# BerserkerMother/Video-Summarization

Hardware: AMD Instinct MI355X
Metric: frames/sec scored (whole node), synthetic [B,T=1024,D=1024] (higher is better)
Workload: dtype f32; 1 GPU; configs[2]: B=64 videos x T=1024 frames x D=1024 per GPU, scorer cfg M-A (heads 4, d_model 256, layers 4), logits + hidden state; global_batch=64, parallelism=videos sharded over 1 GPU(s), no all_gather of scores

## Files before the change

video-summarization_amd/_lib.py:

```python
from __future__ import annotations

import concurrent.futures
import ctypes as C
import os
import subprocess
import threading
from typing import NamedTuple

HERE = os.path.dirname(os.path.abspath(__file__))
ROOT = os.path.dirname(HERE)
CSRC = os.path.join(HERE, "csrc")
INCLUDE = os.path.join(ROOT, "include")
LIB_PATH = os.path.join(HERE, "libvsscore.so")
DIAG_LIB_PATH = os.path.join(HERE, "libvsscore_diag.so")
SOURCES = ("vs_kernels.hip", "vs_attention.hip", "vs_attention_w64.hip", "vs_mlp_fused.hip", "vs_gemm_ring.hip", "vs_scorer.cpp", "vs_eval.cpp",
           "vs_train_kernels.hip", "vs_train_attention.hip", "vs_train_attention_bf16.hip", "vs_train_gemm_rows.hip", "vs_pretrain_kernels.hip",
           "vs_train.cpp", "vs_segment.hip", "vs_segment_gram.hip", "vs_segment.cpp", "vs_optim.hip", "vs_attention_maps.hip",
           "vs_eval_device.hip", "vs_eval_device.cpp", "vs_summary.hip", "vs_summary.cpp", "vs_batch.hip", "vs_cnn.hip", "vs_cnn.cpp",
           "vs_resize.hip", "vs_resize.cpp", "vs_cnn3d.hip", "vs_cnn3d.cpp", "vs_weights.cpp", "vs_error.cpp")
EXTRA_FLAGS = {"vs_resize.cpp": ("-ffp-contract=off",)}
ABI_VERSION = 3

VS_OK, VS_ERR_INVALID, VS_ERR_WORKSPACE, VS_ERR_HIP = 0, 1, 2, 3
VS_FLAG_SIGMOID = 1
VS_FLAG_BF16_ATTENTION = 2
VS_FLAG_BF16_LINEAR = 4
VS_FLAG_F16X3_LINEAR = 8
VS_FLAG_F16X3_ATTENTION = 16
VS_FLAG_SPLITK = 32
VS_TRAIN_FLAG_BF16_LINEAR = 1
VS_TRAIN_FLAG_BF16_ATTENTION = 2
VS_TRAIN_FLAG_FP16 = 4
VS_TRAIN_FLAG_PACKED_LP_ATTENTION = 8

VS_ADAM_MAX_TENSORS = 64
VS_GRAD_NORM_L2, VS_GRAD_NORM_MAX = 0, 1
VS_KTS_FEATURES_F32, VS_KTS_KERNEL_F32, VS_KTS_KERNEL_F64 = 0, 1, 2
VS_KTS_SCORES, VS_KTS_BACKTRACK, VS_KTS_AUTO = 0, 1, 2
VS_KTS_GRAM_DOT, VS_KTS_GRAM_COSINE, VS_KTS_GRAM_RBF = 0, 1, 2
VS_CNN_INPUT_F32_NCHW, VS_CNN_INPUT_U8_NHWC, VS_CNN_INPUT_F32_NHWC = 0, 1, 2
VS_CNN_NUM_CONVS, VS_CNN_FEATURES = 57, 1024
VS_CNN3D_INPUT_F32_NCDHW, VS_CNN3D_INPUT_U8_NDHWC, VS_CNN3D_INPUT_F32_NDHWC = 0, 1, 2
VS_R3D_NUM_CONVS, VS_R3D_FEATURES = 20, 512
VS_RESIZE_SWAP_RB = 1
VS_RESIZE_PATH_FUSED, VS_RESIZE_PATH_SMALL_TILE = 0, 1
NUM_STAGES = 6


class ModelDesc(C.Structure):
    _fields_ = [("d_model", C.c_int32), ("num_heads", C.c_int32), ("num_layers", C.c_int32),
                ("in_features", C.c_int32), ("max_len", C.c_int32), ("num_classes", C.c_int32)]


_LAYER_FIELDS = ("wq", "bq", "wk", "bk", "wv", "bv", "wo", "bo", "ln1_g", "ln1_b",
                 "w1", "b1", "w2", "b2", "ln2_g", "ln2_b")


class LayerParams(C.Structure):
    _fields_ = [(n, C.c_void_p) for n in _LAYER_FIELDS]


class ModelParams(C.Structure):
    _fields_ = [("embed_w", C.c_void_p), ("embed_b", C.c_void_p), ("pos_embedding", C.c_void_p),
                ("layers", C.POINTER(LayerParams)), ("final_w", C.c_void_p), ("final_b", C.c_void_p)]


class DropoutCfg(C.Structure):
    _fields_ = [("p_embed", C.c_float), ("p", C.c_float), ("seed", C.c_uint64), ("flags", C.c_uint32), ("reserved", C.c_uint32)]


class EvalVideo(C.Structure):
    _fields_ = [("scores", C.c_void_p), ("positions", C.c_void_p), ("change_points", C.c_void_p), ("user_summary", C.c_void_p),
                ("user_scores", C.c_void_p)] + [(n, C.c_int32) for n in ("n_scores", "n_positions", "n_frames", "n_shots", "n_users",
                                                                        "user_len", "n_score_users", "use_max", "user_scores_f32")]


LayerGrads = LayerParams


class ModelGrads(C.Structure):
    _fields_ = [("embed_w", C.c_void_p), ("embed_b", C.c_void_p), ("layers", C.POINTER(LayerParams)),
                ("final_w", C.c_void_p), ("final_b", C.c_void_p)]


class AdamCfg(C.Structure):
    _fields_ = [("lr", C.c_double), ("beta1", C.c_double), ("beta2", C.c_double), ("eps", C.c_double),
                ("weight_decay", C.c_double), ("decoupled", C.c_int32), ("reserved", C.c_int32)]


class AdamTensor(C.Structure):
    _fields_ = [("p", C.c_void_p), ("g", C.c_void_p), ("m", C.c_void_p), ("v", C.c_void_p), ("mirror", C.c_void_p),
                ("step", C.c_void_p), ("n", C.c_size_t)]


class KtsKernel(C.Structure):
    _fields_ = [("kind", C.c_int32), ("reserved", C.c_int32), ("gamma", C.c_double)]


class GradTensor(C.Structure):
    _fields_ = [("g", C.c_void_p), ("n", C.c_size_t)]


class CnnConvParams(C.Structure):
    _fields_ = [(n, C.c_void_p) for n in ("weight", "gamma", "beta", "running_mean", "running_var")]


class CnnParams(C.Structure):
    _fields_ = [("conv", CnnConvParams * VS_CNN_NUM_CONVS)]


class Cnn3dConvParams(C.Structure):
    _fields_ = [(n, C.c_void_p) for n in ("weight", "gamma", "beta", "running_mean", "running_var")]


class R3dParams(C.Structure):
    _fields_ = [("conv", Cnn3dConvParams * VS_R3D_NUM_CONVS)]


_P, _I, _Z, _F, _D, _U32, _U64, _RC = C.c_void_p, C.c_int32, C.c_size_t, C.c_float, C.c_double, C.c_uint32, C.c_uint64, C.c_int
_ref = C.POINTER
_LINEAR = [_P] * 4 + [_I] * 4 + [_P, _I, _P]
_LINEAR_OPERANDS = [_P] * 4 + [_I] * 5 + [_P]
_LINEAR_LN = [_P] * 7 + [_I] * 3 + [_P] * 2 + [_I] * 2 + [_P] * 2
_ATTENTION = [_P] * 5 + [_I] * 4 + [_F, _P]
_BYTES_BT = (_Z, [_P, _I, _I])
_DROPOUT_MASK = [_P, _I, _I, _I, _U64, _U32, _F, _P]
_KTS_SIZES = [_P, _I, _I, _I, _P, _I]
_BINDINGS = {
    "vs_scorer.h": {
        "vs_abi_version": (_RC, []),
        "vs_last_error": (C.c_char_p, []),
        "vs_weights_pack": (_RC, [_ref(ModelDesc), _ref(ModelParams), _P, _ref(_P)]),
        "vs_weights_free": (None, [_P]),
        "vs_weights_update": (_RC, [_P, _ref(ModelParams), _P]),
        "vs_weights_set_norm_width": (_RC, [_P, _I]),
        "vs_set_option": (_RC, [C.c_char_p, _I]),
        "vs_scorer_workspace_bytes": _BYTES_BT,
        "vs_scorer_forward": (_RC, [_P, _P, _P, _I, _I, _U32, _P, _P, _P, _Z, _P]),
        "vs_scorer_workspace_bytes_packed": (_Z, [_P, _P, _I]),
        "vs_scorer_forward_packed": (_RC, [_P, _P, _P, _P, _I, _U32, _P, _P, _P, _Z, _P]),
        "vs_scorer_workspace_bytes_cls": _BYTES_BT,
        "vs_scorer_forward_cls": (_RC, [_P, _P, _P, _P, _I, _I, _U32, _P, _P, _P, _Z, _P]),
        "vs_linear_f32": (_RC, _LINEAR),
        "vs_qkv_proj_f32": (_RC, [_P] * 4 + [_I] * 4 + [_P]),
        "vs_attention_f32": (_RC, _ATTENTION),
        "vs_attention_bf16": (_RC, _ATTENTION),
        "vs_attention_bf16_stored": (_RC, [_P] * 5 + [_I] * 4 + [_P]),
        "vs_attention_qscale": (_F, [_F]),
        "vs_attention_f16x3": (_RC, _ATTENTION),
        "vs_linear_residual_layernorm_f32": (_RC, _LINEAR_LN),
        "vs_linear_bf16": (_RC, _LINEAR),
        "vs_linear_residual_layernorm_bf16": (_RC, _LINEAR_LN),
        "vs_linear_f16x3": (_RC, _LINEAR),
        "vs_linear_residual_layernorm_f16x3": (_RC, _LINEAR_LN),
        "vs_mlp_block_bf16": (_RC, [_P, _I, _P, _P, _I, _I, _I, _P, _P]),
        "vs_linear_bf16_operands": (_RC, _LINEAR_OPERANDS),
        "vs_qkv_proj_bf16_operands": (_RC, _LINEAR_OPERANDS),
        "vs_to_bf16": (_RC, [_P, _P, _Z, _P]),
        "vs_linear_bf16_a16": (_RC, [_P] * 4 + [_I] * 3 + [_P, _P]),
        "vs_profile_enable": (_RC, [_I]),
        "vs_profile_collect": (_RC, [_ref(_D), _ref(C.c_int64)]),
        "vs_stage_name": (C.c_char_p, [_I]),
    },
    "vs_eval.h": {
        "vs_eval_upsample": (_RC, [_P, _I, _P, _I, _I, _P]),
        "vs_eval_knapsack": (_RC, [_I, _P, _P, _I, _P, _ref(_I)]),
        "vs_eval_generate_summary": (_RC, [_P, _I, _P, _I, _I, _P, _I, _P, _I]),
        "vs_eval_fscore": (_RC, [_P, _I, _P, _I, _I, _I, _ref(_D)]),
        "vs_eval_rank_correlation": (_RC, [_P, _I, _P, _I, _ref(_D), _ref(_D)]),
        "vs_eval_corpus": (_RC, [_ref(EvalVideo), _I, _I, _P, _P, _P]),
    },
    "vs_eval_device.h": {
        "vs_eval_set_create": (_RC, [_ref(EvalVideo), _I, _P, _ref(_P)]),
        "vs_eval_set_free": (None, [_P]),
        "vs_eval_set_workspace_bytes": (_Z, [_P, _P, _I]),
        "vs_eval_set_run": (_RC, [_P, _P, _P, _I] + [_P] * 5 + [_Z, _P]),
    },
    "vs_summary.h": {
        "vs_summarize_workspace_bytes": (_Z, [_I] + [_P] * 4 + [_D]),
        "vs_summarize": (_RC, [_I] + [_P] * 6 + [_D] + [_P] * 7 + [_Z, _P]),
    },
    "vs_batch.h": {
        "vs_batch_gather_packed": (_RC, [_P] * 3 + [_I] + [_P] * 2 + [_I, C.c_int64, _I] + [_P] * 3),
        "vs_batch_gather_padded": (_RC, [_P] * 3 + [_I] + [_P] * 2 + [_I] * 3 + [_F, _I] + [_P] * 4),
        "vs_batch_gather_rows": (_RC, [_P, _I, _P, _I, _I, _P, _P]),
    },
    "vs_train.h": {
        "vs_train_prepare": (_RC, [_P, _P]),
        "vs_train_saved_bytes": _BYTES_BT,
        "vs_train_workspace_bytes": _BYTES_BT,
        "vs_train_forward": (_RC, [_P, _P, _P, _I, _I, _ref(DropoutCfg), _P, _P, _P, _Z, _P, _Z, _P]),
        "vs_train_backward": (_RC, [_P, _P, _P, _I, _I, _ref(DropoutCfg), _P, _P, _P, _Z, _ref(ModelGrads), _P, _P, _Z, _P]),
        "vs_mse_mask_loss_forward": (_RC, [_P, _P, _P, _I, _I, _P, _P, _P]),
        "vs_mse_mask_loss_backward": (_RC, [_P, _P, _P, _P, _I, _I, _P, _P]),
        "vs_train_attention_forward": (_RC, [_P] * 6 + [_I] * 4 + [_F, _U64, _U32, _F, _P]),
        "vs_train_attention_backward": (_RC, [_P] * 9 + [_I] * 4 + [_F, _U64, _U32, _F, _P]),
        "vs_train_attention_dropout_bits_bytes": (_Z, [_I] * 3),
        "vs_train_attention_dropout_bits": (_RC, _DROPOUT_MASK),
        "vs_train_attention_forward_bf16": (_RC, [_P] * 6 + [_I] * 4 + [_F, _F, _P, _I, _P]),
        "vs_train_attention_backward_bf16": (_RC, [_P] * 9 + [_I] * 4 + [_F, _F, _P, _I, _P]),
        "vs_train_wgrad_scratch_floats": (_Z, [_I] * 3),
        "vs_train_wgrad": (_RC, [_P, _P, _I, _I, _I, _P, _P, _P, _P]),
        "vs_train_wgrad_bf16": (_RC, [_P, _P, _I, _I, _I, _P, _P, _P, _P]),
        "vs_train_dropout_mask_attention": (_RC, _DROPOUT_MASK),
        "vs_train_dropout_mask_rows": (_RC, [_P, _I, _I, _U64, _U32, _F, _P]),
        "vs_train_dropout_site": (_U32, [_I, _I]),
        "vs_train_saved_field": (_RC, [_P, _I, _I, _I, _I, _ref(_Z), _ref(_Z)]),
        "vs_train_last_format": (_U32, []),
        "vs_pretrain_head_state_bytes": (_Z, [_I] * 3),
        "vs_pretrain_head_workspace_bytes": (_Z, [_I] * 4),
        "vs_pretrain_head_forward": (_RC, [_P] * 6 + [_I] * 4 + [_F, _I] + [_P] * 4),
        "vs_pretrain_head_backward": (_RC, [_P] * 8 + [_I] * 4 + [_F, _I] + [_P] * 5 + [_Z, _P]),
        "vs_train_check_packed": (_RC, [_ref(ModelDesc), _P, _I]),
        "vs_train_saved_bytes_desc": (_Z, [_ref(ModelDesc), _P, _I, _I]),
        "vs_train_saved_bytes_packed": (_Z, [_P, _P, _I]),
        "vs_train_workspace_bytes_packed": (_Z, [_P, _P, _I]),
        "vs_train_forward_packed": (_RC, [_P, _P, _P, _P, _I, _ref(DropoutCfg), _P, _P, _P, _Z, _P, _Z, _P]),
        "vs_train_backward_packed": (_RC, [_P, _P, _P, _P, _I, _ref(DropoutCfg), _P, _P, _P, _Z, _ref(ModelGrads), _P, _P, _Z, _P]),
        "vs_mse_packed_loss_forward": (_RC, [_P, _P, _I, _D, _P, _P, _P]),
        "vs_mse_packed_loss_backward": (_RC, [_P, _P, _P, _I, _D, _P, _P]),
        "vs_train_attention_packed_scratch_bytes": _BYTES_BT,
        "vs_train_attention_forward_packed": (_RC, [_P] * 7 + [_I] * 3 + [_F, _U64, _U32, _F, _P, _Z, _P]),
        "vs_train_attention_backward_packed": (_RC, [_P] * 9 + [_I] * 3 + [_F, _U64, _U32, _F, _P, _Z, _P]),
        "vs_train_dropout_mask_attention_packed": (_RC, [_P, _P, _I, _I, _U64, _U32, _F, _P]),
        "vs_train_saved_field_packed": (_RC, [_P, _P, _I, _I, _I, _ref(_Z), _ref(_Z)]),
        "vs_train_attention_packed_lp_scratch_bytes": _BYTES_BT,
        "vs_train_attention_forward_packed_lp": (_RC, [_P] * 7 + [_I] * 3 + [_F, _U64, _U32, _F, _I, _P, _Z, _P]),
        "vs_train_attention_backward_packed_lp": (_RC, [_P] * 9 + [_I] * 3 + [_F, _U64, _U32, _F, _I, _P, _Z, _P]),
        "vs_pretrain_head_state_bytes_packed": _BYTES_BT,
        "vs_pretrain_head_workspace_bytes_packed": (_Z, [_P, _I, _I, _I]),
        "vs_pretrain_head_forward_packed": (_RC, [_P] * 4 + [_I] * 2 + [_P] * 3 + [_I] * 2 + [_F, _I] + [_P] * 4),
        "vs_pretrain_head_backward_packed": (_RC, [_P] * 4 + [_I] * 2 + [_P] * 5 + [_I] * 2 + [_F, _I] + [_P] * 5 + [_Z, _P]),
    },
    "vs_segment.h": {
        "vs_kts_workspace_bytes": (_Z, _KTS_SIZES),
        "vs_kts_segment": (_RC, [_P, _I, _I, _P, _I] + [_P] * 5 + [_I] + [_P] * 4 + [_Z, _P]),
        "vs_kts_scatters": (_RC, [_P, _I, _I, _I, _P, _P, _Z, _P]),
        "vs_kts_gram_workspace_bytes": _BYTES_BT,
        "vs_kts_gram": (_RC, [_P, _I, _P, _I, _ref(KtsKernel), _P, _P, _Z, _P]),
        "vs_kts_workspace_bytes_k": (_Z, _KTS_SIZES + [_ref(KtsKernel)]),
        "vs_kts_segment_k": (_RC, [_P, _I, _I, _P, _I] + [_P] * 5 + [_I, _ref(KtsKernel)] + [_P] * 4 + [_Z, _P]),
        "vs_kts_eval_score": (_RC, [_P, _I, _I, _ref(KtsKernel), _P, _I] + [_P] * 4 + [_Z, _P]),
    },
    "vs_optim.h": {
        "vs_adam_step_tensors": (_RC, [_ref(AdamTensor), _I, _ref(AdamCfg), _P, _P, _P, _P]),
        "vs_adam_state_bytes": (_Z, [_P]),
        "vs_adam_state_init": (_RC, [_P, _P, _P]),
        "vs_adam_state_field": (_RC, [_P, _I, _I, _ref(_Z), _ref(_Z)]),
        "vs_adam_step": (_RC, [_P, _ref(ModelParams), _ref(ModelGrads), _P, _ref(AdamCfg), _P, _P, _P]),
        "vs_grad_norm_workspace_bytes": (_Z, [_ref(GradTensor), _I]),
        "vs_grad_norm_tensors": (_RC, [_ref(GradTensor), _I, _I, _D, _P, _P, _P, _Z, _P]),
        "vs_grad_norm": (_RC, [_P, _ref(ModelGrads), _I, _D, _P, _P, _P, _Z, _P]),
        "vs_grad_scale_tensors": (_RC, [_ref(GradTensor), _I, _P, _P]),
    },
    "vs_inspect.h": {
        "vs_inspect_workspace_bytes": (_Z, [_P, _I, _I, _I]),
        "vs_inspect_forward": (_RC, [_P] * 4 + [_I] * 2 + [_ref(_I), _I] + [_P] * 6 + [_Z, _P]),
        "vs_attention_probs_workspace_bytes": (_Z, [_I] * 3),
        "vs_attention_probs_f32": (_RC, [_P] * 6 + [_I] * 4 + [_F, _P, _Z, _P]),
    },
}
(EXPORTS, EVAL_EXPORTS, EVAL_DEVICE_EXPORTS, SUMMARY_EXPORTS, BATCH_EXPORTS, TRAIN_EXPORTS, SEGMENT_EXPORTS, OPTIM_EXPORTS,
 INSPECT_EXPORTS) = (tuple(_BINDINGS["vs_%s.h" % h]) for h in ("scorer", "eval", "eval_device", "summary", "batch", "train", "segment",
                                                                "optim", "inspect"))

PACKED_INSPECT_HEADER = os.path.join("packed", "vs_inspect_packed.h")
_PACKED_INSPECT_BINDINGS = {
    "vs_inspect_workspace_bytes_packed": (_Z, [_P, _P, _I]),
    "vs_inspect_forward_packed": (_RC, [_P] * 4 + [_I, _ref(_I), _I] + [_P] * 6 + [_Z, _P]),
    "vs_attention_probs_packed_workspace_bytes": (_Z, [_P, _I, _I]),
    "vs_attention_probs_packed_f32": (_RC, [_P] * 4 + [_I] * 3 + [_F] + [_P] * 4 + [_Z, _P]),
}
PACKED_INSPECT_EXPORTS = tuple(_PACKED_INSPECT_BINDINGS)

FEATURES_HEADER = os.path.join("features", "vs_features.h")
_FEATURES_BINDINGS = {
    "vs_cnn_pack": (_RC, [_ref(CnnParams), _P, _ref(_P)]),
    "vs_cnn_free": (None, [_P]),
    "vs_cnn_min_side": (_I, []),
    "vs_cnn_workspace_bytes": (_Z, [_I] * 3),
    "vs_cnn_forward": (_RC, [_P, _P] + [_I] * 4 + [_P, _P, _Z, _P]),
    "vs_cnn_packed_floats": (_Z, [_I] * 3),
    "vs_cnn_pack_conv": (_RC, [_ref(CnnConvParams)] + [_I] * 3 + [_P, _P]),
    "vs_cnn_conv": (_RC, [_P] + [_I] * 5 + [_P] + [_I] * 4 + [_P, _I, _I, _P]),
    "vs_cnn_maxpool": (_RC, [_P] + [_I] * 8 + [_P, _P]),
}
FEATURES_EXPORTS = tuple(_FEATURES_BINDINGS)

RESIZE_HEADER = os.path.join("features", "vs_resize.h")
_RESIZE_BINDINGS = {
    "vs_resize_output_size": (_RC, [_I] * 3 + [_ref(_I)] * 2),
    "vs_resize_plan_create": (_RC, [_I] * 4 + [_P, _ref(_P)]),
    "vs_resize_plan_free": (None, [_P]),
    "vs_resize_plan_describe": (_RC, [_P] + [_ref(_I)] * 3),
    "vs_resize_workspace_bytes": (_Z, [_P, _I]),
    "vs_resize_run": (_RC, [_P, _P, _I, _U32, _P, _P, _Z, _P]),
}
RESIZE_EXPORTS = tuple(_RESIZE_BINDINGS)

VIDEO_FEATURES_HEADER = os.path.join("features", "vs_video_features.h")
_VIDEO_FEATURES_BINDINGS = {
    "vs_r3d_pack": (_RC, [_ref(R3dParams), _P, _ref(_P)]),
    "vs_r3d_free": (None, [_P]),
    "vs_r3d_workspace_bytes": (_Z, [_I] * 4),
    "vs_r3d_flops": (_D, [_I] * 4),
    "vs_r3d_normalisation": (_RC, [_ref(_F)]),
    "vs_r3d_forward": (_RC, [_P, _P] + [_I] * 5 + [_P, _P, _Z, _P]),
    "vs_cnn3d_packed_floats": (_Z, [_I] * 4),
    "vs_cnn3d_pack_conv": (_RC, [_ref(Cnn3dConvParams)] + [_I] * 4 + [_P, _P]),
    "vs_cnn3d_conv": (_RC, [_P] + [_I] * 6 + [_P] + [_I] * 7 + [_P, _I, _P, _P]),
}
VIDEO_FEATURES_EXPORTS = tuple(_VIDEO_FEATURES_BINDINGS)


def hipcc_path() -> str:
    for p in (os.environ.get("HIPCC"), "/opt/rocm/bin/hipcc"):
        if p and os.path.exists(p):
            return p
# ... 152 lines not shown
```

video-summarization_amd/csrc/vs_forward_plan.h:

```cpp
#pragma once
#include <stddef.h>

#include <cstdio>
#include <string>

#include "vs_scorer.h"

struct VskOptions {
    int skinny_rows;
    int lp_min_rows;
    int train_lp_min_rows;
    int lp_min_rows_fused;
    int attn_w64;
    int lp_store32;
    int lp_mlp_unfused;
    int lp_tail_unfused;
    int lp_qkv_unfused;
    int lp_tile256;
    int lp_embed_unfused;
    int exact_unfused;
    int layer_tail_min_rows;
    int mlp_abl;
    int attn_w64_checked;
    int attn_w64_abl;
};

enum { VSK_STORE16 = 16, VSK_A16 = 32, VSK_F16 = 64 };

enum { VSW_FRAGMENTS = 1, VSW_F16X3 = 2, VSW_BF16 = 4, VSW_ROWS16 = 8,
       VSW_TRANSPOSED = 16, VSW_TRANSPOSED_FRAGMENTS = 32, VSW_TRANSPOSED_W2_16 = 64,
       VSW_NUM_FAMILIES = 7 };

inline bool vsk_mlp_bf16_supported(int d) { return d == 256; }
inline bool vsk_gemm16_supported(int M, int N, int K) { return M > 0 && N > 0 && N % 32 == 0 && K >= 32 && K % 32 == 0; }
inline bool vsk_layer_fused_supported(int M, int d, int skinny_rows) { return d == 256 && M > skinny_rows && M <= (1 << 20); }

enum VsArith { VS_ARITH_EXACT = 0, VS_ARITH_BF16 = 1, VS_ARITH_F16X3 = 2 };
enum VsEmbedForm {
    VS_EMBED_CLS,
    VS_EMBED_BF16_QKV,
    VS_EMBED_SPLITK,
    VS_EMBED_GEMM,
};
enum VsAttentionKernel {
    VS_ATT_PACKED,
    VS_ATT_DH256,
    VS_ATT_SPLITKV,
    VS_ATT_LOWPREC,
    VS_ATT_EXACT,
};
enum VsLayerForm {
    VS_LAYER_RING,
    VS_LAYER_BF16_TAIL,
    VS_LAYER_BF16_MLP,
    VS_LAYER_EXACT_PAIR,
    VS_LAYER_STAGES,
};
enum VsLnForm {
    VS_LN_NONE,
    VS_LN_SPLITK_ROWS,
    VS_LN_GEMM_ROWS,
    VS_LN_FUSED,
};

struct VsForwardIn {
    int d_model, num_heads, num_layers, in_features, max_len;
    int norm_width;
    bool has_pe, has_b_embed;
    int B, T;
    unsigned flags;
    bool cls, packed;
};

struct VsForwardPlan {
    int T, M;
    VsArith linear, attention_arith;
    unsigned families;
    VsEmbedForm embed;
    VsAttentionKernel attention;
    VsLayerForm layer;
    VsLnForm ln1, ln2;
    bool qkv16, ffn16;
    bool next_qkv;
    size_t kv_stride;
    int mode_linear;
    int mode_qkv;
    int mode_ffn;
    int mode_attention;

    bool tail_writes_qkv() const { return next_qkv || layer == VS_LAYER_EXACT_PAIR; }
};

inline int vs_attention_prec(unsigned flags) { return (flags & VS_FLAG_F16X3_ATTENTION) ? 2 : (flags & VS_FLAG_BF16_ATTENTION) ? 1 : 0; }

inline int vs_forward_plan(const VsForwardIn &in, const VskOptions &opt, VsForwardPlan *plan, std::string *err) {
    char msg[192];
    auto fail = [&](int code) { *err = msg; return code; };
    const int d = in.d_model, H = in.num_heads, dh = d / H;
    const unsigned flags = in.flags;
    if (!in.packed && in.has_pe && in.T > in.max_len) {
        snprintf(msg, sizeof msg, "T=%d exceeds the positional table (max_len=%d)", in.T, in.max_len);
        return fail(VS_ERR_INVALID);
    }
    if (in.cls && in.packed) { snprintf(msg, sizeof msg, "packed batches have no class-token form"); return fail(VS_ERR_INVALID); }
    const int T = in.T + (in.cls ? 1 : 0);
    if ((long long)in.B * T > (1ll << 30)) { snprintf(msg, sizeof msg, "B*T too large"); return fail(VS_ERR_INVALID); }
    if ((flags & VS_FLAG_BF16_LINEAR) && (flags & VS_FLAG_F16X3_LINEAR)) {
        snprintf(msg, sizeof msg, "VS_FLAG_BF16_LINEAR and VS_FLAG_F16X3_LINEAR are exclusive");
        return fail(VS_ERR_INVALID);
    }
    if ((flags & (VS_FLAG_BF16_ATTENTION | VS_FLAG_F16X3_ATTENTION)) && dh != 32 && dh != 64 && !((flags & VS_FLAG_BF16_ATTENTION) && dh == 128)) {
        snprintf(msg, sizeof msg, "VS_FLAG_BF16_ATTENTION needs head_dim 32, 64 or 128, VS_FLAG_F16X3_ATTENTION 32 or 64 (got %d)", dh);
        return fail(VS_ERR_INVALID);
    }
    if ((flags & VS_FLAG_BF16_ATTENTION) && (flags & VS_FLAG_F16X3_ATTENTION)) {
        snprintf(msg, sizeof msg, "VS_FLAG_BF16_ATTENTION and VS_FLAG_F16X3_ATTENTION are exclusive");
        return fail(VS_ERR_INVALID);
    }

    VsForwardPlan p{};
    p.T = T;
    p.M = in.B * T;
    const int M = p.M;
    const bool embedded = in.norm_width != d;
    const int aprec = vs_attention_prec(flags);
    p.attention_arith = (VsArith)aprec;
    const bool fused_ok = !embedded && vsk_mlp_bf16_supported(d) && aprec == 1 && !opt.lp_store32 && !opt.lp_mlp_unfused;
    const int lp_min_rows = fused_ok && opt.lp_min_rows_fused < opt.lp_min_rows ? opt.lp_min_rows_fused
                                                                               : opt.lp_min_rows;
    p.linear = (flags & VS_FLAG_F16X3_LINEAR) ? VS_ARITH_F16X3 : ((flags & VS_FLAG_BF16_LINEAR) && M > lp_min_rows) ? VS_ARITH_BF16 : VS_ARITH_EXACT;
    const bool bf16 = p.linear == VS_ARITH_BF16;
    const bool splitk = (flags & VS_FLAG_SPLITK) && !bf16 && !in.packed && !in.cls && M <= opt.skinny_rows && (d == 128 || d == 256 || d == 512);
    const int rows_min = in.cls ? in.B * in.T : M;
    p.families = 0;
    if (bf16) p.families = VSW_BF16;
    else if (rows_min <= opt.skinny_rows) p.families = p.linear == VS_ARITH_F16X3 ? VSW_F16X3 : VSW_FRAGMENTS;
    if (bf16 && d > 256) p.families |= VSW_ROWS16;
    p.ffn16 = bf16 && d <= 256 && !embedded && !opt.lp_store32;
    p.qkv16 = p.ffn16 && aprec == 1;
    const bool mlp16 = bf16 && !embedded && vsk_mlp_bf16_supported(d) && !opt.lp_mlp_unfused && !opt.lp_store32;
    const bool ring = bf16 && aprec == 1 && !in.packed && d > 256 && !opt.lp_store32 && vsk_gemm16_supported(M, d, d);
    p.kv_stride = (p.qkv16 || ring) ? (size_t)M * d / 2 : (size_t)M * d;
    p.next_qkv = mlp16 && p.qkv16 && !opt.lp_qkv_unfused;
    const bool exact_fused = p.linear == VS_ARITH_EXACT && aprec == 0 && !embedded && !splitk && !opt.exact_unfused &&
                             vsk_layer_fused_supported(M, d, opt.skinny_rows) && d % H == 0 && dh % 32 == 0;

    p.embed = in.cls ? VS_EMBED_CLS
            : bf16 && in.has_b_embed && p.next_qkv && in.num_layers > 0 && !opt.lp_embed_unfused ? VS_EMBED_BF16_QKV
            : splitk && in.in_features % 1024 == 0 ? VS_EMBED_SPLITK
            : VS_EMBED_GEMM;
    p.attention = in.packed ? VS_ATT_PACKED
                : dh == 256 ? VS_ATT_DH256
                : splitk && aprec != 1 && (dh == 32 || dh == 64 || dh == 128) ? VS_ATT_SPLITKV
                : aprec ? VS_ATT_LOWPREC
                : VS_ATT_EXACT;
    const VsLnForm ln = (d > 256 || embedded) ? VS_LN_GEMM_ROWS : VS_LN_FUSED;
    p.ln1 = p.ln2 = VS_LN_NONE;
    if (ring) p.layer = VS_LAYER_RING;
    else if (mlp16 && p.qkv16 && !opt.lp_tail_unfused) p.layer = VS_LAYER_BF16_TAIL;
    else if (exact_fused) p.layer = VS_LAYER_EXACT_PAIR;
    else {
        p.layer = mlp16 ? VS_LAYER_BF16_MLP : VS_LAYER_STAGES;
        p.ln1 = splitk && d >= 256 ? VS_LN_SPLITK_ROWS : ln;
        if (!mlp16) p.ln2 = splitk ? VS_LN_SPLITK_ROWS : ln;
    }
    p.mode_linear = p.linear;
    p.mode_qkv = p.qkv16 ? (1 | VSK_STORE16) : p.linear;
    p.mode_ffn = p.ffn16 ? (1 | VSK_STORE16) : p.linear;
    p.mode_attention = (p.qkv16 || ring) ? (1 | VSK_STORE16) : aprec;
    *plan = p;
    return VS_OK;
}

inline int vs_packed_waves(int dh, int aprec, long long r8, long long r4) {
    if (dh == 128) return aprec == 1 ? 8 : 4;
    return (!(aprec != 0 && dh == 32) && r8 * 100 <= r4 * 105) ? 8 : 4;
}
```

video-summarization_amd/csrc/vs_kernels.h:

```cpp
#pragma once
#include <hip/hip_runtime.h>
#include <stdint.h>

#include "vs_forward_plan.h"

int vsk_linear(const float *A, const float *W, const float *Wf, const float *bias, float *C, int M, int N, int K,
               int relu, const float *pe, int T, int mode, hipStream_t st);
int vsk_linear_gate(const float *A, const float *W, const float *Wf, const float *bias, const float *gate, float scale,
                    float *C, int M, int N, int K, hipStream_t st, int mode = 0);
int vsk_linear_relu_dropout(const float *A, const float *W, const float *Wf, const float *bias, float *C, int M, int N,
                            int K, unsigned long long seed, unsigned site, float p, hipStream_t st, int mode = 0);
int vsk_pack_fragments(const float *W, float *Wf, int N, int K, hipStream_t st);
int vsk_pack_fragments_f16x3(const float *W, float *Wh, int N, int K, hipStream_t st);
int vsk_qkv(const float *h, const float *Wqkv, const float *Wf, const float *bqkv, float *qkv, int B, int T, int d,
            int H, int mode, hipStream_t st, float qscale = 1.0f);
int vsk_attention(const float *q, const float *k, const float *v, const uint8_t *mask, float *out,
                  int B, int H, int T, int dh, float scale, hipStream_t st);
int vsk_attention_packed(const float *q, const float *k, const float *v, float *out, int H, int Mtot, int dh,
                         float scale, const int *cu, const int *work, int nwork, int nw, int prec, hipStream_t st);
float vsk_attention_qscale(float scale);
int vsk_attention_bf16(const float *q, const float *k, const float *v, const uint8_t *mask, float *out,
                       int B, int H, int T, int dh, float scale, int prec, hipStream_t st);
int vsk_attention_bf16_w64(const void *q, const void *k, const void *v, const uint8_t *mask, void *out, int B, int H, int T,
                           hipStream_t st);
int vsk_attention_bf16_w64_packed(const void *q, const void *k, const void *v, void *out, int H, int Mtot, const int *cu,
                                  const int *work, int nwork, hipStream_t st);
size_t vsk_attention_probs_workspace_bytes(int B, int H, int T);
int vsk_attention_probs(const float *q, const float *k, const uint8_t *mask, float *maps, float *received, float *entropy,
                        int B, int H, int T, int dh, float scale, void *workspace, hipStream_t st);
size_t vsk_attention_probs_packed_workspace_bytes(int B, int H, int M, int tiles);
int vsk_attention_probs_packed_plan(const int *lengths_dev, int B, int H, int M, int tiles, void *workspace, hipStream_t st);
int vsk_attention_probs_packed(const float *q, const float *k, const int *cu, float *maps, float *received, float *entropy, int B,
                               int H, int M, int tiles, int dh, float scale, void *workspace, hipStream_t st);
int vsk_linear_res_ln(const float *A, const float *W, const float *Wf, const float *bias, const float *res,
                      const float *gamma, const float *beta, float *out, int M, int N, int K,
                      const float *score_w, const float *score_b, int num_classes, int sigmoid,
                      float *scores, int mode, hipStream_t st);
int vsk_outproj_ln_fc1(const float *att, const float *Wo, const float *bo, const float *res, const float *gamma, const float *beta,
                       float *h1, const float *W1, const float *b1, float *hidden, int M, int d, hipStream_t st);
int vsk_fc2_ln_qkv(const float *hidden, const float *W2, const float *b2, const float *res, const float *gamma, const float *beta,
                   float *out, const float *Wqkv, const float *bqkv, float *qkv, int B, int T, int d, int H, hipStream_t st);
int vsk_layer_tail(const float *att, const float *Wo, const float *bo, const float *res, const float *g1, const float *be1,
                   const float *W1, const float *b1, float *hidden, const float *W2, const float *b2, const float *g2, const float *be2,
                   float *out, const float *Wqkv, const float *bqkv, float *qkv, const float *score_w, const float *score_b,
                   int num_classes, int sigmoid, float *scores, int B, int T, int d, int H, hipStream_t st);
int vsk_rows_res_ln(const float *a, const float *res, const float *gamma, const float *beta, float *out, int M, int d,
                    const float *score_w, const float *score_b, int num_classes, int sigmoid, float *scores,
                    hipStream_t st, void *out16 = nullptr, int dn = 0,
                    int nsplit = 0, const float *pbias = nullptr);
struct VskMatJobs {
    enum { MAX = 24 };
    const float *in[MAX];
    float *out[MAX];
    int rows[MAX], cols[MAX];
    int n;
};
int vsk_pack_fragments_batch(const VskMatJobs &jobs, hipStream_t st);
int vsk_attention_splitkv(const float *q, const float *k, const float *v, const uint8_t *mask, float *out,
                          int B, int H, int T, int dh, float scale, hipStream_t st);
int vsk_linear_parts(const float *A, const float *Wf, float *parts, int M, int N, int K, int nsplit, hipStream_t st,
                     int f16x3 = 0);
int vsk_sum_parts_pe(const float *parts, int nsplit, const float *bias, const float *pe, int T, float *out, int M, int N, hipStream_t st);
int vsk_diag_attention(const float *q, const float *k, const float *v, float *out, int B, int H, int T, float scale,
                       unsigned long long *diag, hipStream_t st);
int vsk_diag_attention_lp(const float *q, const float *k, const float *v, float *out, int B, int H, int T, float scale,
                          int prec, unsigned long long *diag, hipStream_t st);
int vsk_diag_gemm(const float *A, const float *W, const float *bias, float *C, int M, int N, int K,
                  int grid, unsigned long long *diag, hipStream_t st);
size_t vsk_mlp_bf16_image_bytes(int d);
int vsk_pack_mlp_bf16(const float *Wo, const float *W1, const float *W2, void *img, int d, hipStream_t st);
struct VskNextQkv {
    const void *img;
    const float *bqkv;
    void *qkv16;
    int T, H;
    float qscale;
};
size_t vsk_embed_bf16_image_bytes(int d, int K);
int vsk_pack_embed_bf16(const float *W, void *img, int d, int K, hipStream_t st);
int vsk_embed_bf16(const float *x, const void *img, const float *bias, const float *pe, int T, float *out, int M, int d, int K,
                   const VskNextQkv *next, hipStream_t st);
size_t vsk_qkv_bf16_image_bytes(int d);
int vsk_pack_qkv_bf16(const float *Wqkv, void *img, int d, hipStream_t st);
int vsk_mlp_bf16(const float *h, const void *att16, const float *bo, const float *gamma1, const float *beta1,
                 const void *img, const float *b1, const float *b2,
                 const float *gamma, const float *beta, float *out, int M, int d,
                 const float *score_w, const float *score_b, int num_classes, int sigmoid, float *scores,
                 const VskNextQkv *next, hipStream_t st);
int vsk_plan_packed(const int *lengths_dev, int B, int qb, int *cu, int *work, int work_cap, hipStream_t st);
int vsk_gather_rows(const float *pe, const int *cu, int B, int tmax, int d, float *rows, hipStream_t st);
enum { VSK_COPY_MAX_SEGS = 20 };
struct VskCopySegs {
    const float *src[VSK_COPY_MAX_SEGS];
    float *dst[VSK_COPY_MAX_SEGS];
    unsigned n[VSK_COPY_MAX_SEGS];
    int count;
};
int vsk_copy_segments(const VskCopySegs &segs, hipStream_t st);
int vsk_insert_cls(const float *e, const float *cls, const uint8_t *mask, float *h, uint8_t *mask1, int B, int T, int d,
                   hipStream_t st);
int vsk_skinny_max_rows();

VskOptions &vsk_options();
int vsk_device_cus();

int vsk_gemm16(const void *A16, const void *W16, const float *bias, void *C, int M, int N, int K, int epi, int c16,
               int T, int H, int dh, float qscale, hipStream_t st);
int vsk_to_bf16(const float *src, void *dst, size_t n, hipStream_t st);
```

video-summarization_amd/csrc/vs_kernels.hip:

```cpp
#include "vs_train_device.h"
#include "vs_kernels.h"
#include "vs_launch.h"
#include "vs_linear_pick.h"

namespace {

struct EpiArgs {
    unsigned long long seed;
    unsigned site;
    float p;
    float scale;
};

__device__ __forceinline__ unsigned long long stamp() { return vs_stamp(); }

template <int EPI, int NWM = 2, int DIAG = 0, int NJ = 2, int PREC = 0, int C16 = 0, int KW = 32, int A16 = 0>
__global__ __launch_bounds__(128 * NWM, 2) void gemm_nt_128(
    const float *__restrict__ A, const float *__restrict__ W, const float *__restrict__ bias,
    float *__restrict__ C, int M, int N, int K, const float *__restrict__ pe, int T, int H, int dh,
    unsigned long long *__restrict__ diag = nullptr, EpiArgs ea = EpiArgs{0ull, 0u, 0.f, 0.f}) {
    static_assert(KW == 32 || (KW == 64 && (PREC == 1 || PREC == 3)), "64-wide k-tiles exist for the 16-bit operands only");
    static_assert(A16 == 0 || PREC == 1 || PREC == 3, "16-bit-stored A belongs to the 16-bit operand modes");
    constexpr bool LP1 = PREC == 1 || PREC == 3;
    constexpr int F16 = PREC == 3 ? 1 : 0;
// ... 243 lines not shown
        } else
            __syncthreads();
        fpar ^= 1;
    };

    set_tile(0);
#pragma unroll
    for (int i = 0; i < LA; ++i) load_a(i, 0);
#pragma unroll
    for (int i = 0; i < LW; ++i) load_w(i, 0);
    stage(0);
    __syncthreads();
    if (DIAG != 0) ts0 = stamp();
    const unsigned long long tbegin = ts0;
    if (DIAG >= 2) dsum[3] = __builtin_amdgcn_s_memrealtime();

    for (int it = 0; it < my_tiles; ++it) {
        cu_m0 = nx_m0; cu_n0 = nx_n0;
#pragma unroll
        for (int jj = 0; jj < NJ; ++jj) cu_bias[jj] = nx_bias[jj];
        {
            const f32x16 zero = {0.f, 0.f, 0.f, 0.f, 0.f, 0.f, 0.f, 0.f, 0.f, 0.f, 0.f, 0.f, 0.f, 0.f, 0.f, 0.f};
#pragma unroll
            for (int i = 0; i < 2; ++i)
#pragma unroll
                for (int jj = 0; jj < NJ; ++jj) acc[i][jj] = MFMA32(cu_bias[jj], PREC == 2 ? F16X3_WS : 1.0f, zero);
        }
        for (int kt = 0; kt + 1 < nk; ++kt) ktile((kt + 1) * BK);
        if (it + 1 < my_tiles) set_tile(it + 1);
        ktile(0);

        if constexpr (DIAG == 2) {
            float keep = 0.f;
#pragma unroll
            for (int i = 0; i < 2; ++i)
#pragma unroll
                for (int jj = 0; jj < NJ; ++jj)
#pragma unroll
                    for (int t = 0; t < 16; ++t) keep += acc[i][jj][t];
            if (keep == 1.2345e-30f && diag != nullptr) diag[0] = 1;
            continue;
        }
        unsigned long long te = 0;
        if constexpr (DIAG != 0) te = stamp();
        const int m0 = cu_m0, n0 = cu_n0;
        float *tp = smem + (fpar ^ 1) * (BM + BN) * LD + wave * (32 * LD);
        const int trow = lane >> 3, tc4 = (lane & 7) * 4;
        int b0 = 0, t0 = 0;
        if (EPI == EPI_PE || EPI == EPI_QKV) { b0 = m0 / T; t0 = m0 - b0 * T; }
#pragma unroll
        for (int i = 0; i < 2; ++i) {
#pragma unroll
            for (int jj = 0; jj < NJ; ++jj) {
#pragma unroll
                for (int q = 0; q < 4; ++q) {
                    f32x4 v;
#pragma unroll
                    for (int e = 0; e < 4; ++e) {
                        v[e] = acc[i][jj][4 * q + e];
                        if (EPI == EPI_RELU || EPI == EPI_RELU_DROP) v[e] = relu1(v[e]);
                    }
                    *(f32x4 *)&tp[r * LD + 8 * q + 4 * h] = v;
                }
                const int c32 = n0 + 32 * NJ * wc + 32 * jj;
                int which = 0, head = 0, e0 = 0;
                if (EPI == EPI_QKV) { const int d = H * dh; which = c32 / d; const int c = c32 - which * d; head = c / dh; e0 = c - head * dh; }
#pragma unroll
                for (int p = 0; p < 4; ++p) {
                    const int ro = 64 * wr + 32 * i + trow + 8 * p;
                    f32x4 v = *(const f32x4 *)&tp[(trow + 8 * p) * LD + tc4];
                    if constexpr (PREC == 2) v *= 1.0f / F16X3_WS;
                    const int row = m0 + ro;
                    int bb = b0, tt = t0 + ro;
                    if (EPI == EPI_PE || EPI == EPI_QKV) { while (tt >= T) { tt -= T; ++bb; } }
                    if (row < M && c32 < N) {
                        if (EPI == EPI_PE) {
                            const f32x4 pv = *(const f32x4 *)(pe + (size_t)tt * N + c32 + tc4);
#pragma unroll
                            for (int e = 0; e < 4; ++e) v[e] += pv[e];
                        }
                        if (EPI == EPI_GATE) {
                            if constexpr (C16 != 0) {
                                const u32x2 g2 = *(const u32x2 *)((const a16_t *)pe + (size_t)row * N + c32 + tc4);
#pragma unroll
                                for (int e = 0; e < 4; ++e) v[e] = (short)(g2[e >> 1] >> (16 * (e & 1))) > 0 ? v[e] * ea.scale : 0.f;
                            } else {
                            const f32x4 gv = *(const f32x4 *)(pe + (size_t)row * N + c32 + tc4);
#pragma unroll
                            for (int e = 0; e < 4; ++e) v[e] = gv[e] > 0.f ? v[e] * ea.scale : 0.f;
                            }
                        }
                        if (EPI == EPI_RELU_DROP) {
                            const DropSite dsite = drop_site(ea.seed, ea.site, ea.p);
                            const unsigned rk = drop_rowkey(dsite, (unsigned)row);
#pragma unroll
                            for (int e = 0; e < 4; ++e) v[e] = drop_keep(dsite, rk, (unsigned)(c32 + tc4 + e)) ? v[e] * dsite.scale : 0.f;
                        }
                        if constexpr (C16 != 0) {
                            if (EPI == EPI_QKV && which == 0) v *= ea.scale;
                            u32x2 u; u[0] = pack_lp<F16>(v[0], v[1]); u[1] = pack_lp<F16>(v[2], v[3]);
                            unsigned short *C2 = (unsigned short *)C;
                            if (EPI == EPI_QKV)
                                *(u32x2 *)(C2 + (size_t)which * M * (H * dh) + (((size_t)bb * H + head) * T + tt) * dh + e0 + tc4) = u;
                            else
                                *(u32x2 *)(C2 + (size_t)row * N + c32 + tc4) = u;
                        } else if (EPI == EPI_QKV)
                            *(f32x4 *)(C + (size_t)which * M * (H * dh) + (((size_t)bb * H + head) * T + tt) * dh + e0 + tc4) = v;
                        else
                            *(f32x4 *)(C + (size_t)row * N + c32 + tc4) = v;
                    }
                }
            }
        }
        __syncthreads();
        if constexpr (DIAG != 0) dsum[1] += stamp() - te;
    }
    if (DIAG >= 2) { ts0 = stamp(); dsum[4] = __builtin_amdgcn_s_memrealtime(); }
    if (DIAG != 0 && diag != nullptr && lane == 0) {
        unsigned long long *o = diag + ((size_t)blockIdx.x * (2 * NWM) + wave) * 8;
#pragma unroll
        for (int i = 0; i < 5; ++i) o[i] = dsum[i];
        o[5] = ts0 - tbegin; o[6] = (unsigned long long)(my_tiles * nk); o[7] = tbegin;
    }
}

template <int NB, int PREC = 0>
__global__ __launch_bounds__(256) void gemm_res_ln(
    const float *__restrict__ A, const float *__restrict__ W, const float *__restrict__ bias,
    const float *__restrict__ res, const float *__restrict__ gamma, const float *__restrict__ beta,
    float *__restrict__ out, int M, int K,
    const float *__restrict__ score_w, const float *__restrict__ score_b, int num_classes,
    int sigmoid, float *__restrict__ scores) {
    constexpr int BM = 64, N = 64 * NB, BK = 16, LD = BK + 4;
    __shared__ __attribute__((aligned(16))) float smem[2 * (BM + N) * LD];

    const int m0 = blockIdx.x * BM;
    const int tid = threadIdx.x, lane = tid & 63, wave = tid >> 6;
    const int r = lane & 31, h = lane >> 5;
    const int wr = wave >> 1, wc = wave & 1;

    const int lrow = tid >> 2, lc4 = (tid & 3) * 4;
    int arow = m0 + lrow; arow = arow < M ? arow : M - 1;
    const float *ag = A + (size_t)arow * K + lc4;
    const float *wg = W + (size_t)lrow * K + lc4;
    f32x4 pa, pw[NB];
    pa = *(const f32x4 *)ag;
#pragma unroll
    for (int i = 0; i < NB; ++i) pw[i] = *(const f32x4 *)(wg + (size_t)64 * i * K);

    f32x16 acc[NB];
#pragma unroll
    for (int j = 0; j < NB; ++j)
#pragma unroll
        for (int t = 0; t < 16; ++t) acc[j][t] = 0.f;

    auto put = [&](float *rowp, f32x4 v, float scale) __attribute__((always_inline)) {
        if constexpr (PREC == 2) {
            v *= scale;
            u32x2 hi, lo;
            split_f16x4((const float *)&v, hi, lo);
            *(u32x2 *)&rowp[lc4 / 2] = hi;
            *(u32x2 *)&rowp[8 + lc4 / 2] = lo;
        } else {
            *(f32x4 *)&rowp[lc4] = v;
        }
    };
    {
        float *As = smem, *Ws = smem + BM * LD;
        put(&As[lrow * LD], pa, 1.0f);
#pragma unroll
        for (int i = 0; i < NB; ++i) put(&Ws[(lrow + 64 * i) * LD], pw[i], F16X3_WS);
    }
    __syncthreads();

    const int nk = K / BK;
    for (int kt = 0; kt < nk; ++kt) {
        const int cur = kt & 1;
        const float *As = smem + cur * (BM + N) * LD, *Ws = As + BM * LD;
        const bool more = kt + 1 < nk;
        if (more) {
            pa = *(const f32x4 *)(ag + (kt + 1) * BK);
#pragma unroll
            for (int i = 0; i < NB; ++i) pw[i] = *(const f32x4 *)(wg + (size_t)64 * i * K + (kt + 1) * BK);
        }
        const float *ap = As + (32 * wr + r) * LD + 4 * h;
        const float *wp = Ws + (32 * NB * wc + r) * LD + 4 * h;
        if constexpr (PREC == 2) {
            const f16x8 ah = __builtin_bit_cast(f16x8, *(const u32x4 *)ap), al = __builtin_bit_cast(f16x8, *(const u32x4 *)(ap + 8));
#pragma unroll
            for (int j = 0; j < NB; ++j) {
                const f16x8 bh = __builtin_bit_cast(f16x8, *(const u32x4 *)(wp + 32 * j * LD));
                const f16x8 bl = __builtin_bit_cast(f16x8, *(const u32x4 *)(wp + 32 * j * LD + 8));
                acc[j] = MFMA_F16(ah, bl, acc[j]);
                acc[j] = MFMA_F16(al, bh, acc[j]);
                acc[j] = MFMA_F16(ah, bh, acc[j]);
            }
        } else {
#pragma unroll
            for (int g = 0; g < BK / 8; ++g) {
                const f32x4 a = *(const f32x4 *)(ap + 8 * g);
                f32x4 b[NB];
#pragma unroll
                for (int j = 0; j < NB; ++j) b[j] = *(const f32x4 *)(wp + 32 * j * LD + 8 * g);
#pragma unroll
                for (int s = 0; s < 4; ++s)
#pragma unroll
                    for (int j = 0; j < NB; ++j) acc[j] = MFMA32(a[s], b[j][s], acc[j]);
            }
        }
        if (more) {
            float *An = smem + (cur ^ 1) * (BM + N) * LD, *Wn = An + BM * LD;
            put(&An[lrow * LD], pa, 1.0f);
#pragma unroll
            for (int i = 0; i < NB; ++i) put(&Wn[(lrow + 64 * i) * LD], pw[i], F16X3_WS);
        }
        __syncthreads();
    }

    float *red = smem;
    const int cbase = 32 * NB * wc + r;
    float bj[NB], gj[NB], bej[NB];
#pragma unroll
    for (int j = 0; j < NB; ++j) { bj[j] = bias[cbase + 32 * j]; gj[j] = gamma[cbase + 32 * j]; bej[j] = beta[cbase + 32 * j]; }

    float part[16];
#pragma unroll
    for (int t = 0; t < 16; ++t) {
        int row = m0 + 32 * wr + acc_row(t, h); row = row < M ? row : M - 1;
        float s = 0.f;
#pragma unroll
        for (int j = 0; j < NB; ++j) {
            const float v = (PREC == 2 ? acc[j][t] * (1.0f / F16X3_WS) : acc[j][t]) + bj[j] + res[(size_t)row * N + cbase + 32 * j];
            acc[j][t] = v;
            s += v;
        }
        part[t] = half_sum(s);
    }
    if (r == 0) {
#pragma unroll
        for (int t = 0; t < 16; ++t) red[wc * 64 + 32 * wr + acc_row(t, h)] = part[t];
    }
    __syncthreads();
    float mean[16];
#pragma unroll
    for (int t = 0; t < 16; ++t) {
        const int rl = 32 * wr + acc_row(t, h);
        mean[t] = (red[rl] + red[64 + rl]) * (1.0f / N);
    }
    __syncthreads();
#pragma unroll
    for (int t = 0; t < 16; ++t) {
        float s = 0.f;
#pragma unroll
        for (int j = 0; j < NB; ++j) { const float c = acc[j][t] - mean[t]; acc[j][t] = c; s += c * c; }
        part[t] = half_sum(s);
    }
    if (r == 0) {
#pragma unroll
        for (int t = 0; t < 16; ++t) red[wc * 64 + 32 * wr + acc_row(t, h)] = part[t];
    }
    __syncthreads();
#pragma unroll
    for (int t = 0; t < 16; ++t) {
        const int rl = 32 * wr + acc_row(t, h);
        const float rstd = 1.0f / sqrtf((red[rl] + red[64 + rl]) * (1.0f / N) + 1e-5f);
        const int row = m0 + rl;
#pragma unroll
        for (int j = 0; j < NB; ++j) {
            const float y = acc[j][t] * rstd * gj[j] + bej[j];
            acc[j][t] = y;
            if (row < M) out[(size_t)row * N + cbase + 32 * j] = y;
        }
    }
    if (score_w != nullptr) {
        for (int c = 0; c < num_classes; ++c) {
            __syncthreads();
            float wj[NB];
#pragma unroll
            for (int j = 0; j < NB; ++j) wj[j] = score_w[(size_t)c * N + cbase + 32 * j];
#pragma unroll
            for (int t = 0; t < 16; ++t) {
                float s = 0.f;
#pragma unroll
                for (int j = 0; j < NB; ++j) s += acc[j][t] * wj[j];
                part[t] = half_sum(s);
            }
            if (r == 0) {
#pragma unroll
                for (int t = 0; t < 16; ++t) red[wc * 64 + 32 * wr + acc_row(t, h)] = part[t];
            }
            __syncthreads();
            if (tid < 64) {
                const int row = m0 + tid;
                if (row < M) {
                    float s = red[tid] + red[64 + tid] + score_b[c];
                    if (sigmoid) s = 1.0f / (1.0f + expf(-s));
                    scores[(size_t)row * num_classes + c] = s;
                }
            }
        }
    }
}

struct LnTail {
    const float *W2, *b2;
    float *C2;
    int T, H, dhs;
};
struct LnPhase2 {
    const float *W, *bias, *gamma, *beta;
    float *out;
    LnTail tl;
};

template <int NT, int PREC, int A16, int DIAG, int TAIL>
__device__ __forceinline__ void ln_rows_tiles(
    const float *__restrict__ A, const float *__restrict__ W, const float *__restrict__ bias,
    const float *__restrict__ res, const float *__restrict__ gamma, const float *__restrict__ beta,
    float *__restrict__ out, int M, int K,
    const float *__restrict__ score_w, const float *__restrict__ score_b, int num_classes,
    int sigmoid, float *__restrict__ scores, unsigned long long *__restrict__ diag, const LnTail tl, const LnPhase2 p2) {
    static_assert(TAIL == 0 || (NT == 8 && PREC == 0 && DIAG == 0), "the register-fed tail exists for exact fp32 at d_model 256");
    constexpr int BM = 128, N = 32 * NT, BK = 16, LD = BK + 4;
    constexpr int WL = (N * BK / 4 + 255) / 256;
    constexpr bool TWO = TAIL >= 3;
    constexpr int NPH = TWO ? 2 : 1;
    constexpr int TN2 = TAIL == 2 ? 3 * N : 4 * N;
    constexpr int SMALL2 = TAIL == 3 ? 3 * N + 3 * N : TAIL == 4 ? 3 * N : 0;
    __shared__ __attribute__((aligned(16))) float smem[2 * (BM + N) * LD + 4 * N + (TAIL != 0 ? TN2 : 0) + SMALL2];
    float *gam_s = smem + 2 * (BM + N) * LD, *bet_s = gam_s + N, *sw_s = bet_s + N, *bias_s = sw_s + N;
    float *bias2_s = bias_s + N;
    float *small2_s = bias2_s + TN2;

    int tid = threadIdx.x, lane = tid & 63, wave = tid >> 6;
    int r = lane & 31, h = lane >> 5;
    const int ntiles = (M + BM - 1) / BM;
    const int nk = K / BK;

    constexpr float SC = PREC == 2 ? F16X3_WS : 1.0f;
    for (int i = tid; i < N; i += 256) { gam_s[i] = gamma[i]; bet_s[i] = beta[i]; bias_s[i] = bias[i] * SC; }
    if constexpr (TAIL != 0)
        for (int i = tid; i < TN2; i += 256) bias2_s[i] = tl.b2[i];
    if constexpr (TWO) {
        for (int i = tid; i < N; i += 256) { small2_s[i] = p2.gamma[i]; small2_s[N + i] = p2.beta[i]; small2_s[2 * N + i] = p2.bias[i]; }
        if constexpr (TAIL == 3)
            for (int i = tid; i < 3 * N; i += 256) small2_s[3 * N + i] = p2.tl.b2[i];
    }

    int lrow = tid >> 2, lc4 = (tid & 3) * 4;
    f32x4 pa[2], pw[WL];
    u32x2 pa16[2];
    const float *aptr[2], *wptr[WL];
    const unsigned short *aptr16[2];
#pragma unroll
    for (int i = 0; i < WL; ++i) {
        int wrow = lrow + 64 * i; wrow = wrow < N ? wrow : N - 1;
        wptr[i] = W + (size_t)wrow * K + lc4;
    }
    static_assert(PREC != 0 || N % 64 == 0, "the exact-fp32 staging map covers W without a guard");
    __amdgpu_buffer_rsrc_t ars = __builtin_amdgcn_make_buffer_rsrc(const_cast<float *>(A), 0, 0, 0x00020000);
    __amdgpu_buffer_rsrc_t wrs = __builtin_amdgcn_make_buffer_rsrc(const_cast<float *>(W), 0, N * K * 4, 0x00020000);
    int aoff[2], woff[WL];
#pragma unroll
    for (int i = 0; i < WL; ++i) woff[i] = ((lrow + 64 * i) * K + lc4) * 4;
    auto gload = [&](int i, int kb) __attribute__((always_inline)) {
        if (i < 2) pa[i] = __builtin_bit_cast(f32x4, __builtin_amdgcn_raw_buffer_load_b128(ars, aoff[i], kb, 0));
        else pw[i - 2] = __builtin_bit_cast(f32x4, __builtin_amdgcn_raw_buffer_load_b128(wrs, woff[i - 2], kb, 0));
    };
    constexpr int LDB = 12;
    auto stage = [&](int buf) __attribute__((always_inline)) {
        float *As = smem + buf * (BM + N) * LD, *Ws = As + BM * LD;
        if constexpr (PREC == 2) {
#pragma unroll
            for (int i = 0; i < 2; ++i) {
                u32x2 hi, lo;
                split_f16x4((const float *)&pa[i], hi, lo);
                *(u32x2 *)&As[(lrow + 64 * i) * LD + lc4 / 2] = hi;
                *(u32x2 *)&As[(lrow + 64 * i) * LD + 8 + lc4 / 2] = lo;
            }
#pragma unroll
            for (int i = 0; i < WL; ++i)
                if (lrow + 64 * i < N) {
                    u32x2 hi, lo;
                    const f32x4 ws = pw[i] * F16X3_WS;
                    split_f16x4((const float *)&ws, hi, lo);
                    *(u32x2 *)&Ws[(lrow + 64 * i) * LD + lc4 / 2] = hi;
                    *(u32x2 *)&Ws[(lrow + 64 * i) * LD + 8 + lc4 / 2] = lo;
                }
        } else if constexpr (PREC == 1) {
#pragma unroll
            for (int i = 0; i < 2; ++i) {
                u32x2 u;
                if constexpr (A16 != 0) u = pa16[i];
                else { u[0] = pack_bf16(pa[i][0], pa[i][1]); u[1] = pack_bf16(pa[i][2], pa[i][3]); }
                *(u32x2 *)&As[(lrow + 64 * i) * LDB + lc4 / 2] = u;
            }
#pragma unroll
            for (int i = 0; i < WL; ++i)
                if (lrow + 64 * i < N) {
                    u32x2 u; u[0] = pack_bf16(pw[i][0], pw[i][1]); u[1] = pack_bf16(pw[i][2], pw[i][3]);
                    *(u32x2 *)&Ws[(lrow + 64 * i) * LDB + lc4 / 2] = u;
                }
        } else {
#pragma unroll
            for (int i = 0; i < 2; ++i) *(f32x4 *)&As[(lrow + 64 * i) * LD + lc4] = pa[i];
#pragma unroll
            for (int i = 0; i < WL; ++i) *(f32x4 *)&Ws[(lrow + 64 * i) * LD + lc4] = pw[i];
        }
    };

    f32x16 acc[NT];

    constexpr int TCH = 128, TWB = 4 * 32 * 36, TBUF = TCH * 36;
    static_assert(TAIL == 0 || TWB + 2 * TBUF <= 2 * (BM + N) * LD, "corners and weight tiles fit the staging area");
    int r2 = tid >> 3, c2 = (tid & 7) * 4;
    __amdgpu_buffer_rsrc_t wrs2 = __builtin_amdgcn_make_buffer_rsrc(const_cast<float *>(tl.W2), 0, TN2 * N * 4, 0x00020000);
    const float *tbias_s = bias2_s;
    int woff2 = (r2 * N + c2) * 4;
    f32x4 pw2[4];
    f32x16 U[4];
    auto tail_soff = [&](int c, int kt) __attribute__((always_inline)) { return (TCH * c * N + 32 * kt) * 4; };
    auto tail_load = [&](int i, int soff) __attribute__((always_inline)) {
        pw2[i] = __builtin_bit_cast(f32x4, __builtin_amdgcn_raw_buffer_load_b128(wrs2, woff2, soff + 32 * i * N * 4, 0));
    };
    auto tail_stage = [&](int buf) __attribute__((always_inline)) {
#pragma unroll
        for (int i = 0; i < 4; ++i) *(f32x4 *)&smem[TWB + buf * TBUF + (r2 + 32 * i) * 36 + c2] = pw2[i];
    };
    auto bias_mfma = [&](int c) __attribute__((always_inline)) {
        const f32x16 zero = {0.f, 0.f, 0.f, 0.f, 0.f, 0.f, 0.f, 0.f, 0.f, 0.f, 0.f, 0.f, 0.f, 0.f, 0.f, 0.f};
#pragma unroll
        for (int jj = 0; jj < 4; ++jj) {
            const float bv = tbias_s[TCH * c + 32 * jj + r];
            U[jj] = MFMA32(h == 0 ? bv : 0.f, 1.0f, zero);
        }
    };
    auto tail_step = [&](auto ktc, int nsoff) __attribute__((always_inline)) {
        constexpr int kt = decltype(ktc)::value;
        const float *wp = smem + TWB + (kt & 1) * TBUF + r * 36 + 4 * h;
        float *wd = smem + TWB + ((kt + 1) & 1) * TBUF + r2 * 36 + c2;
        f32x4 fw[3];
        fw[0] = *(const f32x4 *)wp;
        fw[1] = *(const f32x4 *)(wp + 32 * 36);
        __builtin_amdgcn_sched_barrier(0);
#pragma unroll
        for (int t = 0; t < 16; ++t) {
            const int g = t / 4, jj = t % 4;
            if (t + 2 < 16) fw[(t + 2) % 3] = *(const f32x4 *)(wp + 32 * ((t + 2) % 4) * 36 + 8 * ((t + 2) / 4));
            if (t < 4) tail_load(t, nsoff);
            if (t >= 12) *(f32x4 *)(wd + 32 * (t - 12) * 36) = pw2[t - 12];
#pragma unroll
            for (int s2 = 0; s2 < 4; ++s2) U[jj] = MFMA32(fw[t % 3][s2], acc[kt][4 * g + s2], U[jj]);
            __builtin_amdgcn_sched_group_barrier(0x008, 1, 0);
            if (t + 2 < 16) __builtin_amdgcn_sched_group_barrier(0x100, 1, 0);
            if (t < 4) __builtin_amdgcn_sched_group_barrier(0x020, 1, 0);
            __builtin_amdgcn_sched_group_barrier(0x008, 3, 0);
            if (t >= 12) __builtin_amdgcn_sched_group_barrier(0x200, 1, 0);
            __builtin_amdgcn_sched_barrier(0);
        }
        __syncthreads();
    };

    unsigned long long dsum[3] = {0, 0, 0}, tbegin = 0, tq = 0, ktiles = 0;
    if constexpr (DIAG != 0) tbegin = stamp();
    for (int tile = blockIdx.x; tile < ntiles; tile += gridDim.x) {
        if constexpr (DIAG != 0) tq = stamp();
        const int m0 = tile * BM;
      static_for<NPH>([&](auto phc) __attribute__((always_inline)) {
        constexpr int PH = decltype(phc)::value;
        constexpr bool P1 = TWO && PH == 1;
        constexpr int PT = !TWO ? TAIL : PH == 0 ? 1 : TAIL == 3 ? 2 : 0;
        constexpr int PTN2 = PT == 2 ? 3 * N : 4 * N, TNC = PTN2 / TCH;
        const LnTail ptl = P1 ? p2.tl : tl;
        const float *pA = P1 ? tl.C2 : A;
        const int pK = P1 ? 4 * N : K, pnk = P1 ? 4 * N / BK : nk;
        const float *pgam_s = P1 ? small2_s : gam_s, *pbet_s = P1 ? small2_s + N : bet_s, *pbias_s = P1 ? small2_s + 2 * N : bias_s;
        float *pout = P1 ? p2.out : out;
        if constexpr (TWO) {
            asm volatile("" : "+v"(tid));
            lane = tid & 63; wave = tid >> 6; r = lane & 31; h = lane >> 5;
            lrow = tid >> 2; lc4 = (tid & 3) * 4; r2 = tid >> 3; c2 = (tid & 7) * 4; woff2 = (r2 * N + c2) * 4;
            wrs = __builtin_amdgcn_make_buffer_rsrc(const_cast<float *>(P1 ? p2.W : W), 0, N * pK * 4, 0x00020000);
#pragma unroll
            for (int i = 0; i < WL; ++i) woff[i] = ((lrow + 64 * i) * pK + lc4) * 4;
            if constexpr (PT != 0) {
                wrs2 = __builtin_amdgcn_make_buffer_rsrc(const_cast<float *>(ptl.W2), 0, PTN2 * N * 4, 0x00020000);
                tbias_s = P1 ? small2_s + 3 * N : bias2_s;
            }
        }
        int row = m0 + 32 * wave + r;
        const bool row_ok = row < M;
        row = row_ok ? row : M - 1;
#pragma unroll
        for (int i = 0; i < 2; ++i) {
            int ar = m0 + lrow + 64 * i; ar = ar < M ? ar : M - 1;
            if constexpr (A16 != 0) {
                aptr16[i] = (const unsigned short *)A + (size_t)ar * K + lc4;
                pa16[i] = *(const u32x2 *)aptr16[i];
            } else if constexpr (PREC == 0) {
                aoff[i] = ((ar - m0) * pK + lc4) * 4;
            } else {
                aptr[i] = A + (size_t)ar * K + lc4;
                pa[i] = *(const f32x4 *)aptr[i];
            }
        }
        if constexpr (PREC == 0) {
            ars = __builtin_amdgcn_make_buffer_rsrc(const_cast<float *>(pA + (size_t)m0 * pK), 0, (M - m0 < BM ? M - m0 : BM) * pK * 4, 0x00020000);
            if constexpr (P1) {
#pragma unroll
                for (int i = 2; i < 2 + WL; ++i) gload(i, 0);
                asm volatile("s_waitcnt vmcnt(0)" ::: "memory");
                __builtin_amdgcn_fence(__ATOMIC_RELEASE, "workgroup");
                __syncthreads();
                __builtin_amdgcn_fence(__ATOMIC_ACQUIRE, "workgroup");
#pragma unroll
                for (int i = 0; i < 2; ++i) gload(i, 0);
            } else {
#pragma unroll
                for (int i = 0; i < 2 + WL; ++i) gload(i, 0);
            }
        } else {
#pragma unroll
            for (int i = 0; i < WL; ++i) pw[i] = *(const f32x4 *)wptr[i];
        }
        if constexpr (!P1) {
            const float *rp = res + (size_t)row * N + 4 * h;
#pragma unroll
            for (int j = 0; j < NT; ++j)
#pragma unroll
                for (int q = 0; q < 4; ++q) {
                    f32x4 rv = *(const f32x4 *)(rp + 32 * j + 8 * q);
                    if constexpr (PREC == 2) rv *= SC;
#pragma unroll
                    for (int e = 0; e < 4; ++e) acc[j][4 * q + e] = rv[e];
                }
        }
        if constexpr (!P1) __syncthreads();
        stage(0);
        __syncthreads();
        if constexpr (DIAG != 0) { dsum[2] += stamp() - tq; ktiles += nk; }

        for (int kt = 0; kt < pnk; ++kt) {
            const int kn = kt + 1 < pnk ? kt + 1 : kt;
            const float *As = smem + (kt & 1) * (BM + N) * LD, *Ws = As + BM * LD;
            if constexpr (PREC == 2) {
                const float *arow = As + (32 * wave + r) * LD + 4 * h;
                const f16x8 ah = __builtin_bit_cast(f16x8, *(const u32x4 *)arow);
                const f16x8 al = __builtin_bit_cast(f16x8, *(const u32x4 *)(arow + 8));
#pragma unroll
                for (int i = 0; i < 2; ++i) pa[i] = *(const f32x4 *)(aptr[i] + kn * BK);
#pragma unroll
                for (int i = 0; i < WL; ++i) pw[i] = *(const f32x4 *)(wptr[i] + kn * BK);
#pragma unroll
                for (int j = 0; j < NT; ++j) {
                    const float *wrow = Ws + (32 * j + r) * LD + 4 * h;
                    const f16x8 wh = __builtin_bit_cast(f16x8, *(const u32x4 *)wrow);
                    const f16x8 wl = __builtin_bit_cast(f16x8, *(const u32x4 *)(wrow + 8));
                    acc[j] = MFMA_F16(wl, ah, acc[j]);
                    acc[j] = MFMA_F16(wh, al, acc[j]);
                    acc[j] = MFMA_F16(wh, ah, acc[j]);
                }
                stage((kt + 1) & 1);
                __syncthreads();
                continue;
            }
            if constexpr (PREC == 1) {
                const bf16x8 fa = __builtin_bit_cast(bf16x8, *(const u32x4 *)(As + (32 * wave + r) * LDB + 4 * h));
#pragma unroll
                for (int i = 0; i < 2; ++i) {
                    if constexpr (A16 != 0) pa16[i] = *(const u32x2 *)(aptr16[i] + kn * BK);
                    else pa[i] = *(const f32x4 *)(aptr[i] + kn * BK);
                }
#pragma unroll
                for (int i = 0; i < WL; ++i) pw[i] = *(const f32x4 *)(wptr[i] + kn * BK);
#pragma unroll
                for (int j = 0; j < NT; ++j) {
                    const bf16x8 fw = __builtin_bit_cast(bf16x8, *(const u32x4 *)(Ws + (32 * j + r) * LDB + 4 * h));
                    acc[j] = MFMA_BF16(fw, fa, acc[j]);
                }
                stage((kt + 1) & 1);
                __syncthreads();
                continue;
            }
            const float *ap = As + (32 * wave + r) * LD + 4 * h;
            const float *wp = Ws + r * LD + 4 * h;
            constexpr int NS = 2 * NT, NL = 2 + WL;
            constexpr int LPS = (NL + NT - 1) / NT;
            constexpr int WB = NS - (NL + LPS - 1) / LPS;
            static_assert(BK == 16 && (NL + LPS - 1) / LPS <= NT, "loads and LDS writes of a k-tile occupy distinct steps");
            f32x4 fa[2], fw[3];
            fa[0] = *(const f32x4 *)ap;
            fw[0] = *(const f32x4 *)wp;
            fw[1] = *(const f32x4 *)(wp + 32 * LD);
            fa[1] = *(const f32x4 *)(ap + 8);
            __builtin_amdgcn_sched_barrier(0);
#pragma unroll
            for (int t = 0; t < NS; ++t) {
                const int g = t / NT, j = t % NT;
                if (t + 2 < NS) fw[(t + 2) % 3] = *(const f32x4 *)(wp + 32 * ((t + 2) % NT) * LD + 8 * ((t + 2) / NT));
                int nld = 0, nwr = 0;
#pragma unroll
                for (int q = 0; q < LPS; ++q) {
                    const int il = t * LPS + q, iw = (t - WB) * LPS + q;
                    if (il < NL) { gload(il, kn * (BK * 4)); ++nld; }
                    if (t >= WB && iw < NL) {
                        float *Ad = smem + ((kt + 1) & 1) * (BM + N) * LD, *Wd = Ad + BM * LD;
                        if (iw < 2) *(f32x4 *)&Ad[(lrow + 64 * iw) * LD + lc4] = pa[iw];
                        else *(f32x4 *)&Wd[(lrow + 64 * (iw - 2)) * LD + lc4] = pw[iw - 2];
                        ++nwr;
                    }
                }
#pragma unroll
                for (int s2 = 0; s2 < 4; ++s2) acc[j] = MFMA32(fw[t % 3][s2], fa[g][s2], acc[j]);
                __builtin_amdgcn_sched_group_barrier(0x008, 1, 0);
                if (t + 2 < NS) __builtin_amdgcn_sched_group_barrier(0x100, 1, 0);
#pragma unroll
                for (int q = 0; q < LPS; ++q)
                    if (q < nld) __builtin_amdgcn_sched_group_barrier(0x020, 1, 0);
                __builtin_amdgcn_sched_group_barrier(0x008, 3, 0);
#pragma unroll
                for (int q = 0; q < LPS; ++q)
                    if (q < nwr) __builtin_amdgcn_sched_group_barrier(0x200, 1, 0);
                __builtin_amdgcn_sched_barrier(0);
            }
            if constexpr (DIAG != 0) {
                const unsigned long long tb = stamp();
                __syncthreads();
                dsum[0] += stamp() - tb;
            } else
                __syncthreads();
        }
        if constexpr (DIAG != 0) tq = stamp();
        if constexpr (PT != 0) {
#pragma unroll
            for (int i = 0; i < 4; ++i) tail_load(i, tail_soff(0, 0));
        }

        float sum = 0.f;
#pragma unroll
        for (int j = 0; j < NT; ++j) {
            float pj = 0.f;
#pragma unroll
            for (int q = 0; q < 4; ++q) {
                const f32x4 bv = *(const f32x4 *)&pbias_s[32 * j + 8 * q + 4 * h];
#pragma unroll
                for (int e = 0; e < 4; ++e) { acc[j][4 * q + e] += bv[e]; pj += acc[j][4 * q + e]; }
            }
            sum += pj;
        }
        sum = pair_sum(sum);
        const float mean = sum * (1.0f / N);
        float sq = 0.f;
#pragma unroll
        for (int j = 0; j < NT; ++j) {
            float pj = 0.f;
#pragma unroll
            for (int t = 0; t < 16; ++t) { const float c = acc[j][t] - mean; acc[j][t] = c; pj += c * c; }
            sq += pj;
        }
        sq = pair_sum(sq);
        const float rstd = 1.0f / sqrtf(sq * (1.0f / N) + 1e-5f * (SC * SC));
        float *tp = smem + wave * (32 * 36);
        const int trow = lane >> 3, tc4 = (lane & 7) * 4;
#pragma unroll
        for (int j = 0; j < NT; ++j) {
#pragma unroll
            for (int q = 0; q < 4; ++q) {
                const f32x4 gv = *(const f32x4 *)&pgam_s[32 * j + 8 * q + 4 * h];
                const f32x4 bv = *(const f32x4 *)&pbet_s[32 * j + 8 * q + 4 * h];
                f32x4 y;
#pragma unroll
                for (int e = 0; e < 4; ++e) { y[e] = acc[j][4 * q + e] * rstd * gv[e] + bv[e]; acc[j][4 * q + e] = y[e]; }
                if constexpr (!TWO || P1) *(f32x4 *)&tp[r * 36 + 8 * q + 4 * h] = y;
            }
            if constexpr (TWO && !P1) __builtin_amdgcn_sched_barrier(0);
            if constexpr (!TWO || P1) {
#pragma unroll
                for (int pq = 0; pq < 4; ++pq) {
                    const f32x4 v = *(const f32x4 *)&tp[(trow + 8 * pq) * 36 + tc4];
                    const int orow = m0 + 32 * wave + trow + 8 * pq;
                    if (orow < M) *(f32x4 *)(pout + (size_t)orow * N + 32 * j + tc4) = v;
                }
            }
        }
        if constexpr (!TWO || (P1 && TAIL == 4))
        if (score_w != nullptr) {
            for (int c = 0; c < num_classes; ++c) {
                __syncthreads();
                for (int i = tid; i < N; i += 256) sw_s[i] = score_w[(size_t)c * N + i];
                __syncthreads();
                float dot = 0.f;
#pragma unroll
                for (int j = 0; j < NT; ++j) {
                    float pj = 0.f;
#pragma unroll
                    for (int q = 0; q < 4; ++q) {
                        const f32x4 wv = *(const f32x4 *)&sw_s[32 * j + 8 * q + 4 * h];
#pragma unroll
                        for (int e = 0; e < 4; ++e) pj += acc[j][4 * q + e] * wv[e];
                    }
                    dot += pj;
                }
                dot = pair_sum(dot);
                if (h == 0 && row_ok) {
                    float sc = dot + score_b[c];
                    if (sigmoid) sc = 1.0f / (1.0f + expf(-sc));
                    scores[(size_t)row * num_classes + c] = sc;
                }
            }
        }
        if constexpr (DIAG != 0) dsum[1] += stamp() - tq;
        if constexpr (PT != 0) {
            tail_stage(0);
            int rowoff[4];
            __amdgpu_buffer_rsrc_t crs;
            if constexpr (PT == 1) {
                crs = __builtin_amdgcn_make_buffer_rsrc(ptl.C2 + (size_t)m0 * PTN2, 0, (M - m0 < BM ? M - m0 : BM) * PTN2 * 4, 0x00020000);
#pragma unroll
                for (int p = 0; p < 4; ++p) rowoff[p] = ((32 * wave + trow + 8 * p) * PTN2 + tc4) * 4;
            } else {
                crs = __builtin_amdgcn_make_buffer_rsrc(ptl.C2, 0, 0, 0x00020000);
#pragma unroll
                for (int p = 0; p < 4; ++p) {
                    const int orow = m0 + 32 * wave + trow + 8 * p;
                    const int bb = orow / ptl.T, tt = orow - bb * ptl.T;
                    rowoff[p] = orow < M ? (((bb * ptl.H * ptl.T + tt) << ptl.dhs) + tc4) * 4 : (int)0x80000000;
                }
            }
            bias_mfma(0);
            __syncthreads();
            for (int c = 0; c < TNC; ++c) {
                const int cn = c + 1 < TNC ? c + 1 : c;
                static_for<8>([&](auto ktc) __attribute__((always_inline)) {
                    constexpr int kt = decltype(ktc)::value;
                    tail_step(ktc, kt < 7 ? tail_soff(c, kt + 1) : tail_soff(cn, 0));
                });
                if constexpr (PT == 2) {
                    const int which = c >> 1;
                    crs = __builtin_amdgcn_make_buffer_rsrc(ptl.C2 + (size_t)which * M * N, 0, M * N * 4, 0x00020000);
                }
#pragma unroll
                for (int jj = 0; jj < 4; ++jj) {
                    __builtin_amdgcn_sched_barrier(0);
#pragma unroll
                    for (int q = 0; q < 4; ++q) {
                        f32x4 v;
#pragma unroll
                        for (int e = 0; e < 4; ++e) v[e] = PT == 1 ? relu1(U[jj][4 * q + e]) : U[jj][4 * q + e];
                        *(f32x4 *)&tp[r * 36 + 8 * q + 4 * h] = v;
                    }
                    int soff;
                    if constexpr (PT == 1) soff = (TCH * c + 32 * jj) * 4;
                    else {
                        const int cc = (TCH * c + 32 * jj) & (N - 1), head = cc >> ptl.dhs, e0 = cc - (head << ptl.dhs);
                        soff = (((head * ptl.T) << ptl.dhs) + e0) * 4;
                    }
#pragma unroll
                    for (int p = 0; p < 4; ++p) {
                        const f32x4 v = *(const f32x4 *)&tp[(trow + 8 * p) * 36 + tc4];
                        __builtin_amdgcn_raw_buffer_store_b128(__builtin_bit_cast(u32x4, v), crs, rowoff[p], soff, 0);
                    }
                }
                __builtin_amdgcn_sched_barrier(0);
                bias_mfma(cn);
            }
        }
      });
    }
    if constexpr (DIAG != 0) {
        if (diag != nullptr && lane == 0) {
            unsigned long long *o = diag + ((size_t)blockIdx.x * 4 + wave) * 8;
            o[0] = dsum[0]; o[1] = dsum[1]; o[2] = dsum[2]; o[3] = 0; o[4] = 0;
            o[5] = stamp() - tbegin; o[6] = ktiles; o[7] = tbegin;
        }
    }
}

template <int NT, int PREC = 0, int A16 = 0, int DIAG = 0>
__global__ __launch_bounds__(256, 2) void gemm_ln_rows(
    const float *__restrict__ A, const float *__restrict__ W, const float *__restrict__ bias,
    const float *__restrict__ res, const float *__restrict__ gamma, const float *__restrict__ beta,
    float *__restrict__ out, int M, int K,
    const float *__restrict__ score_w, const float *__restrict__ score_b, int num_classes,
    int sigmoid, float *__restrict__ scores, unsigned long long *__restrict__ diag = nullptr) {
    ln_rows_tiles<NT, PREC, A16, DIAG, 0>(A, W, bias, res, gamma, beta, out, M, K, score_w, score_b, num_classes, sigmoid, scores, diag,
                                          LnTail{nullptr, nullptr, nullptr, 0, 0, 0}, LnPhase2{});
}

__global__ __launch_bounds__(256, 2) void layer_outproj_ln_fc1(
    const float *__restrict__ A, const float *__restrict__ W, const float *__restrict__ bias,
    const float *__restrict__ res, const float *__restrict__ gamma, const float *__restrict__ beta,
    float *__restrict__ out, int M, int K, const float *__restrict__ W1, const float *__restrict__ b1, float *__restrict__ hidden) {
    ln_rows_tiles<8, 0, 0, 0, 1>(A, W, bias, res, gamma, beta, out, M, K, nullptr, nullptr, 0, 0, nullptr, nullptr,
                                 LnTail{W1, b1, hidden, 0, 0, 0}, LnPhase2{});
}
__global__ __launch_bounds__(256, 2) void layer_fc2_ln_qkv(
    const float *__restrict__ A, const float *__restrict__ W, const float *__restrict__ bias,
    const float *__restrict__ res, const float *__restrict__ gamma, const float *__restrict__ beta,
    float *__restrict__ out, int M, int K, const float *__restrict__ Wqkv, const float *__restrict__ bqkv, float *__restrict__ qkv,
    int T, int H, int dhs) {
    ln_rows_tiles<8, 0, 0, 0, 2>(A, W, bias, res, gamma, beta, out, M, K, nullptr, nullptr, 0, 0, nullptr, nullptr,
                                 LnTail{Wqkv, bqkv, qkv, T, H, dhs}, LnPhase2{});
}
struct LayerTailArgs {
    const float *att, *Wo, *bo, *res, *g1, *be1;
    const float *W1, *b1;
    float *hidden;
    const float *W2, *b2, *g2, *be2;
    float *out;
    int M;
};
__global__ __launch_bounds__(256, 2) void gemm_ln_rows_tail_qkv(const LayerTailArgs a, const float *__restrict__ Wqkv,
                                                         const float *__restrict__ bqkv, float *__restrict__ qkv, int T, int H, int dhs) {
    ln_rows_tiles<8, 0, 0, 0, 3>(a.att, a.Wo, a.bo, a.res, a.g1, a.be1, nullptr, a.M, 256, nullptr, nullptr, 0, 0, nullptr, nullptr,
                                 LnTail{a.W1, a.b1, a.hidden, 0, 0, 0}, LnPhase2{a.W2, a.b2, a.g2, a.be2, a.out, LnTail{Wqkv, bqkv, qkv, T, H, dhs}});
}
__global__ __launch_bounds__(256, 2) void gemm_ln_rows_tail_score(const LayerTailArgs a, const float *__restrict__ score_w,
                                                           const float *__restrict__ score_b, int num_classes, int sigmoid,
                                                           float *__restrict__ scores) {
    ln_rows_tiles<8, 0, 0, 0, 4>(a.att, a.Wo, a.bo, a.res, a.g1, a.be1, nullptr, a.M, 256, score_w, score_b, num_classes, sigmoid, scores, nullptr,
                                 LnTail{a.W1, a.b1, a.hidden, 0, 0, 0}, LnPhase2{a.W2, a.b2, a.g2, a.be2, a.out, LnTail{nullptr, nullptr, nullptr, 0, 0, 0}});
}

__device__ __forceinline__ void skinny_mainloop(f32x16 &acc, const float *__restrict__ ap,
                                                const float *__restrict__ wp, int K) {
    f32x4 a[4][4], w[4][4];
    auto load = [&](int set, int off) __attribute__((always_inline)) {
#pragma unroll
        for (int g = 0; g < 4; ++g) {
            a[set][g] = *(const f32x4 *)(ap + off + 8 * g);
            w[set][g] = *(const f32x4 *)(wp + off + 8 * g);
        }
    };
    auto mma = [&](int set) __attribute__((always_inline)) {
#pragma unroll
        for (int g = 0; g < 4; ++g)
#pragma unroll
            for (int st = 0; st < 4; ++st) acc = MFMA32(w[set][g][st], a[set][g][st], acc);
    };
    const int nc = K / 32;
    load(0, 0); load(1, 32); load(2, 64);
    for (int c = 0; c < nc - 4; c += 4) {
        load(3, 96);  mma(0);
        load(0, 128); mma(1);
        load(1, 160); mma(2);
        load(2, 192); mma(3);
        ap += 128; wp += 128;
    }
    load(3, 96);
    mma(0); mma(1); mma(2); mma(3);
}

template <int EPI>
__global__ __launch_bounds__(256) void skinny_gemm(
    const float *__restrict__ A, const float *__restrict__ W, const float *__restrict__ bias,
    float *__restrict__ C, int M, int N, int K, const float *__restrict__ pe, int T, int H, int dh, EpiArgs ea) {
    const int lane = threadIdx.x & 63, wave = threadIdx.x >> 6, r = lane & 31, h = lane >> 5;
    const int m0 = blockIdx.x * 32, n0 = blockIdx.y * 128 + 32 * wave;
    if (n0 >= N) return;
    const int row = m0 + r;
    const int arow = row < M ? row : M - 1;
    const float *ap = A + (size_t)arow * K + 4 * h, *wp = W + (size_t)(n0 + r) * K + 4 * h;
    const f32x16 zero = {0.f, 0.f, 0.f, 0.f, 0.f, 0.f, 0.f, 0.f, 0.f, 0.f, 0.f, 0.f, 0.f, 0.f, 0.f, 0.f};
    f32x16 acc = MFMA32(h == 0 ? bias[n0 + r] : 0.f, 1.0f, zero);
    skinny_mainloop(acc, ap, wp, K);
    if (row >= M) return;
    int bb = 0, tt = 0;
    if (EPI == EPI_PE || EPI == EPI_QKV) { bb = row / T; tt = row - bb * T; }
    int which = 0, head = 0, e0 = 0;
    if (EPI == EPI_QKV) { const int d = H * dh; which = n0 / d; const int c = n0 - which * d; head = c / dh; e0 = c - head * dh; }
#pragma unroll
    for (int q = 0; q < 4; ++q) {
        const int co = 8 * q + 4 * h;
        f32x4 v;
#pragma unroll
        for (int e = 0; e < 4; ++e) v[e] = acc[4 * q + e];
        if (EPI == EPI_RELU || EPI == EPI_RELU_DROP) {
#pragma unroll
            for (int e = 0; e < 4; ++e) v[e] = relu1(v[e]);
        }
        if (EPI == EPI_PE) {
            const f32x4 pv = *(const f32x4 *)(pe + (size_t)tt * N + n0 + co);
#pragma unroll
            for (int e = 0; e < 4; ++e) v[e] += pv[e];
        }
        if (EPI == EPI_GATE) {
            const f32x4 gv = *(const f32x4 *)(pe + (size_t)row * N + n0 + co);
#pragma unroll
            for (int e = 0; e < 4; ++e) v[e] = gv[e] > 0.f ? v[e] * ea.scale : 0.f;
        }
        if (EPI == EPI_RELU_DROP) {
            const DropSite dsite = drop_site(ea.seed, ea.site, ea.p);
            const unsigned rk = drop_rowkey(dsite, (unsigned)row);
#pragma unroll
            for (int e = 0; e < 4; ++e) v[e] = drop_keep(dsite, rk, (unsigned)(n0 + co + e)) ? v[e] * dsite.scale : 0.f;
        }
        if (EPI == EPI_QKV)
            *(f32x4 *)(C + (size_t)which * M * (H * dh) + (((size_t)bb * H + head) * T + tt) * dh + e0 + co) = v;
        else
            *(f32x4 *)(C + (size_t)row * N + n0 + co) = v;
    }
}

template <int NW>
__global__ __launch_bounds__(64 * NW) void skinny_ln(
    const float *__restrict__ A, const float *__restrict__ W, const float *__restrict__ bias,
    const float *__restrict__ res, const float *__restrict__ gamma, const float *__restrict__ beta,
    float *__restrict__ out, int M, int K,
    const float *__restrict__ score_w, const float *__restrict__ score_b, int num_classes,
    int sigmoid, float *__restrict__ scores) {
    constexpr int N = 32 * NW;
    __shared__ float red[NW * 64];
    const int lane = threadIdx.x & 63, wave = threadIdx.x >> 6, r = lane & 31, h = lane >> 5;
    const int m0 = blockIdx.x * 32, n0 = 32 * wave;
    const int row = m0 + r;
    const bool row_ok = row < M;
    const int arow = row_ok ? row : M - 1;
    const float *ap = A + (size_t)arow * K + 4 * h, *wp = W + (size_t)(n0 + r) * K + 4 * h;
    f32x16 acc;
#pragma unroll
    for (int q = 0; q < 4; ++q) {
        const f32x4 rv = *(const f32x4 *)(res + (size_t)arow * N + n0 + 8 * q + 4 * h);
#pragma unroll
        for (int e = 0; e < 4; ++e) acc[4 * q + e] = rv[e];
    }
    skinny_mainloop(acc, ap, wp, K);

    auto row_total = [&](float v) __attribute__((always_inline)) {
        __syncthreads();
        red[wave * 64 + lane] = v;
        __syncthreads();
        float t = 0.f;
#pragma unroll
        for (int w = 0; w < NW; ++w) t += red[w * 64 + lane];
        return pair_sum(t);
    };
    float s1 = 0.f;
#pragma unroll
    for (int q = 0; q < 4; ++q) {
        const f32x4 bv = *(const f32x4 *)(bias + n0 + 8 * q + 4 * h);
#pragma unroll
        for (int e = 0; e < 4; ++e) { acc[4 * q + e] += bv[e]; s1 += acc[4 * q + e]; }
    }
    const float mean = row_total(s1) * (1.0f / N);
    float s2 = 0.f;
#pragma unroll
    for (int t = 0; t < 16; ++t) { const float c = acc[t] - mean; acc[t] = c; s2 += c * c; }
    const float rstd = 1.0f / sqrtf(row_total(s2) * (1.0f / N) + 1e-5f);
#pragma unroll
    for (int q = 0; q < 4; ++q) {
        const int co = n0 + 8 * q + 4 * h;
        const f32x4 gv = *(const f32x4 *)(gamma + co), bv = *(const f32x4 *)(beta + co);
        f32x4 y;
#pragma unroll
        for (int e = 0; e < 4; ++e) { y[e] = acc[4 * q + e] * rstd * gv[e] + bv[e]; acc[4 * q + e] = y[e]; }
        if (row_ok) *(f32x4 *)(out + (size_t)row * N + co) = y;
    }
    if (score_w != nullptr) {
        for (int c = 0; c < num_classes; ++c) {
            float dot = 0.f;
#pragma unroll
            for (int q = 0; q < 4; ++q) {
                const f32x4 wv = *(const f32x4 *)(score_w + (size_t)c * N + n0 + 8 * q + 4 * h);
#pragma unroll
                for (int e = 0; e < 4; ++e) dot += acc[4 * q + e] * wv[e];
            }
            const float tot = row_total(dot);
            if (wave == 0 && h == 0 && row_ok) {
                float sc = tot + score_b[c];
                if (sigmoid) sc = 1.0f / (1.0f + expf(-sc));
                scores[(size_t)row * num_classes + c] = sc;
            }
        }
    }
}

__global__ void pack_fragments(const float *__restrict__ W, float *__restrict__ Wf, int N, int K) {
    const size_t total = (size_t)N * K / 4;
    for (size_t idx = (size_t)blockIdx.x * blockDim.x + threadIdx.x; idx < total; idx += (size_t)gridDim.x * blockDim.x) {
        const int lane = (int)(idx & 63);
        const size_t gi = idx >> 6;
        const int g = (int)(gi % (K / 8)), nb = (int)(gi / (K / 8));
        const int row = 32 * nb + (lane & 31), col = 8 * g + 4 * (lane >> 5);
        *(f32x4 *)(Wf + idx * 4) = *(const f32x4 *)(W + (size_t)row * K + col);
    }
}

__device__ __forceinline__ void skinny2_phase(f32x16 &acc, const float *__restrict__ As_row,
                                              const float *__restrict__ wf, int kp) {
    f32x4 w[4][4];
    auto load = [&](int set, int chunk) __attribute__((always_inline)) {
#pragma unroll
        for (int g = 0; g < 4; ++g) w[set][g] = *(const f32x4 *)(wf + (size_t)(4 * chunk + g) * 256);
    };
    auto mma = [&](int set, int chunk) __attribute__((always_inline)) {
#pragma unroll
        for (int g = 0; g < 4; ++g) {
            const f32x4 a = *(const f32x4 *)(As_row + 32 * chunk + 8 * g);
#pragma unroll
            for (int st = 0; st < 4; ++st) acc = MFMA32(w[set][g][st], a[st], acc);
        }
    };
    const int nc = kp / 32;
    load(0, 0); load(1, 1); load(2, 2);
    int c = 0;
    for (; c < nc - 4; c += 4) {
        load(3, c + 3); mma(0, c);
        load(0, c + 4); mma(1, c + 1);
        load(1, c + 5); mma(2, c + 2);
        load(2, c + 6); mma(3, c + 3);
    }
    load(3, c + 3);
    mma(0, c); mma(1, c + 1); mma(2, c + 2); mma(3, c + 3);
}

template <int NT>
__device__ __forceinline__ void skinny2_stage(float *As, const float *__restrict__ A, int M, int K, int m0, int k0, int kp) {
    const int f4row = kp / 4, total = 32 * f4row;
    for (int idx = threadIdx.x; idx < total; idx += NT) {
        const int row = idx / f4row, c4 = idx - row * f4row;
        int ar = m0 + row; ar = ar < M ? ar : M - 1;
        *(f32x4 *)&As[row * (kp + 4) + 4 * c4] = *(const f32x4 *)(A + (size_t)ar * K + k0 + 4 * c4);
    }
}

__global__ void pack_fragments_f16x3(const float *__restrict__ W, unsigned *__restrict__ Wh, int N, int K) {
    const size_t total = (size_t)N * K / 8;
    for (size_t idx = (size_t)blockIdx.x * blockDim.x + threadIdx.x; idx < total; idx += (size_t)gridDim.x * blockDim.x) {
        const int lane = (int)(idx & 63);
        const size_t gi = idx >> 6;
        const int g = (int)(gi % (K / 16)), nb = (int)(gi / (K / 16));
        const int row = 32 * nb + (lane & 31), col = 16 * g + 8 * (lane >> 5);
        const f32x4 v0 = *(const f32x4 *)(W + (size_t)row * K + col) * F16X3_WS;
        const f32x4 v1 = *(const f32x4 *)(W + (size_t)row * K + col + 4) * F16X3_WS;
        u32x2 h0, l0, h1, l1;
        split_f16x4((const float *)&v0, h0, l0);
        split_f16x4((const float *)&v1, h1, l1);
        u32x4 hi, lo;
        hi[0] = h0[0]; hi[1] = h0[1]; hi[2] = h1[0]; hi[3] = h1[1];
        lo[0] = l0[0]; lo[1] = l0[1]; lo[2] = l1[0]; lo[3] = l1[1];
        *(u32x4 *)(Wh + idx * 8) = hi;
        *(u32x4 *)(Wh + idx * 8 + 4) = lo;
    }
}

__device__ __forceinline__ void skinny3_phase(f32x16 &acc, const unsigned char *__restrict__ as_row,
                                              const unsigned *__restrict__ wh, int kp) {
    u32x4 w[4][2][2];
    auto load = [&](int set, int chunk) __attribute__((always_inline)) {
#pragma unroll
        for (int g = 0; g < 2; ++g) {
            w[set][g][0] = *(const u32x4 *)(wh + (size_t)(2 * chunk + g) * 512);
            w[set][g][1] = *(const u32x4 *)(wh + (size_t)(2 * chunk + g) * 512 + 4);
        }
    };
    auto mma = [&](int set, int chunk) __attribute__((always_inline)) {
#pragma unroll
        for (int g = 0; g < 2; ++g) {
            const f16x8 ah = __builtin_bit_cast(f16x8, *(const u32x4 *)(as_row + 64 * chunk + 32 * g));
            const f16x8 al = __builtin_bit_cast(f16x8, *(const u32x4 *)(as_row + 2 * kp + 64 * chunk + 32 * g));
            const f16x8 wh8 = __builtin_bit_cast(f16x8, w[set][g][0]), wl8 = __builtin_bit_cast(f16x8, w[set][g][1]);
            acc = MFMA_F16(wl8, ah, acc);
            acc = MFMA_F16(wh8, al, acc);
            acc = MFMA_F16(wh8, ah, acc);
        }
    };
    const int nc = kp / 32;
    load(0, 0); load(1, 1); load(2, 2);
    int c = 0;
    for (; c < nc - 4; c += 4) {
        load(3, c + 3); mma(0, c);
        load(0, c + 4); mma(1, c + 1);
        load(1, c + 5); mma(2, c + 2);
        load(2, c + 6); mma(3, c + 3);
    }
    load(3, c + 3);
    mma(0, c); mma(1, c + 1); mma(2, c + 2); mma(3, c + 3);
}

// ... 731 lines not shown
```

video-summarization_amd/csrc/vs_scorer.cpp:

```cpp
#include "vs_scorer.h"
#include "vs_inspect.h"

#include <hip/hip_runtime.h>

#include <atomic>
#include <cmath>
#include <cstdio>
#include <cstdlib>
#include <cstring>
#include <mutex>
#include <string>
#include <vector>

#include "vs_error.h"
#include "vs_kernels.h"
#include "vs_train_kernels.h"
#include "vs_weights_impl.h"

namespace {

size_t align_up(size_t v, size_t a) { return (v + a - 1) / a * a; }

const char *const kStageNames[VS_NUM_STAGES] = {"embed_pe", "qkv_proj", "attention", "outproj_ln", "fc1_relu", "fc2_ln_score"};
struct StageRec { int stage; hipEvent_t a, b; };
std::mutex g_prof_mu;
std::atomic<bool> g_prof_on{false};
std::vector<StageRec> g_prof;
std::vector<hipEvent_t> g_event_pool;

hipEvent_t take_event() {
    {
        std::lock_guard<std::mutex> lk(g_prof_mu);
        if (!g_event_pool.empty()) { hipEvent_t e = g_event_pool.back(); g_event_pool.pop_back(); return e; }
    }
    hipEvent_t e = nullptr;
    return hipEventCreate(&e) == hipSuccess ? e : nullptr;
}

struct StageScope {
    hipStream_t st; int stage; hipEvent_t a = nullptr, b = nullptr; bool on;
    StageScope(int stage_, hipStream_t st_) : st(st_), stage(stage_), on(g_prof_on.load(std::memory_order_relaxed)) {
        if (!on) return;
        a = take_event(); b = take_event();
        if (!a || !b) { on = false; return; }
        (void)hipEventRecord(a, st);
    }
    ~StageScope() {
        if (!on) return;
        (void)hipEventRecord(b, st);
        std::lock_guard<std::mutex> lk(g_prof_mu);
        g_prof.push_back({stage, a, b});
    }
};

}

namespace {
struct OptionName { const char *name; int VskOptions::*field; int dflt; };
const OptionName kOptions[] = {
    {"VS_SKINNY_ROWS", &VskOptions::skinny_rows, 16384}, {"VS_LP_MIN_ROWS", &VskOptions::lp_min_rows, 8192},
    {"VS_MLP_ABL", &VskOptions::mlp_abl, 0},             {"VS_EXACT_UNFUSED", &VskOptions::exact_unfused, 0},
    {"VS_LP_STORE32", &VskOptions::lp_store32, 0},
    {"VS_LP_MLP_UNFUSED", &VskOptions::lp_mlp_unfused, 0}, {"VS_LP_TAIL_UNFUSED", &VskOptions::lp_tail_unfused, 0},
    {"VS_LP_QKV_UNFUSED", &VskOptions::lp_qkv_unfused, 0}, {"VS_LP_EMBED_UNFUSED", &VskOptions::lp_embed_unfused, 0},
    {"VS_LP_MIN_ROWS_FUSED", &VskOptions::lp_min_rows_fused, 256}, {"VS_LP_TILE256", &VskOptions::lp_tile256, 0},
    {"VS_ATTN_W64_CHECKED", &VskOptions::attn_w64_checked, 0}, {"VS_TRAIN_LP_MIN_ROWS", &VskOptions::train_lp_min_rows, 1024},
    {"VS_ATTN_W64", &VskOptions::attn_w64, 1},           {"VS_ATTN_W64_ABL", &VskOptions::attn_w64_abl, 0},
    {"VS_LAYER_TAIL_MIN_ROWS", &VskOptions::layer_tail_min_rows, 1024},
};
int option_from_env(const OptionName &o) {
    const char *e = getenv(o.name);
    if (!e) return o.dflt;
    return *e ? atoi(e) : 1;
}
}

VskOptions &vsk_options() {
    static VskOptions opts = [] {
        VskOptions o{};
        for (const auto &k : kOptions) o.*(k.field) = option_from_env(k);
        return o;
    }();
    return opts;
}

int vsk_device_cus() {
    static std::atomic<int> cus[64];
    int dev = 0;
    if (hipGetDevice(&dev) != hipSuccess) return -1;
    if (dev >= 0 && dev < 64) { const int c = cus[dev].load(std::memory_order_relaxed); if (c > 0) return c; }
    int n = 0;
    if (hipDeviceGetAttribute(&n, hipDeviceAttributeMultiprocessorCount, dev) != hipSuccess || n <= 0) return -1;
    if (dev >= 0 && dev < 64) cus[dev].store(n, std::memory_order_relaxed);
    return n;
}

extern "C" {

int vs_abi_version(void) { return VS_ABI_VERSION; }

size_t vs_scorer_workspace_bytes(const vs_weights *w, int32_t B, int32_t T) {
    if (!w || B <= 0 || T <= 0) return 0;
    const size_t md = align_up((size_t)B * T * w->desc.d_model * sizeof(float), 256);
    return 10 * md;
}

}

namespace {
struct PackedInfo {
    const float *pe_rows;
    const int *cu;
    const int *work;
    int nwork, nw;
};

struct InspectHook {
    const int32_t *layers;
    int n_layers;
    float *maps, *received, *entropy;
    void *workspace;
    int videos = 0, tiles = 0;
    size_t map_stride = 0;
};

int forward_core(const vs_weights *w, const float *x, const uint8_t *key_pad_mask, int32_t B,
                 int32_t T, uint32_t flags, float *scores, float *hidden, void *workspace,
                 size_t workspace_bytes, void *stream, const PackedInfo *pk, const float *cls = nullptr,
                 const InspectHook *ins = nullptr) {
    if (!w || !x || !scores) return vs_failf(VS_ERR_INVALID, "weights/x/scores is NULL");
    if (B <= 0 || T <= 0) return vs_failf(VS_ERR_INVALID, "B=%d T=%d", B, T);
    const vs_model_desc &D = w->desc;
    const int Tf = T;
    const int sig = (flags & VS_FLAG_SIGMOID) ? 1 : 0;
    const VsForwardIn in{D.d_model, D.num_heads, D.num_layers, D.in_features, D.max_len, w->dn(), w->has_pe, w->has_b_embed,
                         B, Tf, flags, cls != nullptr, pk != nullptr};
    VsForwardPlan plan;
    std::string err;
    if (int rc = vs_forward_plan(in, vsk_options(), &plan, &err)) return vs_fail_msg(rc, err.c_str());
    T = plan.T;
    const size_t need_core = vs_scorer_workspace_bytes(w, B, T);
    const size_t need = need_core + (cls ? align_up((size_t)B * T, 256) : 0);
    if (!workspace || workspace_bytes < need)
        return vs_failf(VS_ERR_WORKSPACE, "workspace %zu bytes < %zu needed", workspace_bytes, need);
    if (((uintptr_t)workspace & 255) || ((uintptr_t)x & 15) || (hidden && ((uintptr_t)hidden & 15)) || (cls && ((uintptr_t)cls & 15)))
        return vs_failf(VS_ERR_INVALID, "workspace must be 256-byte, x/hidden/cls_token 16-byte aligned");
    vsw_order(w, stream);
    if (plan.families) if (int rc = vsw_ensure(w, plan.families, stream)) return rc;

    hipStream_t st = (hipStream_t)stream;
    const int d = D.d_model, H = D.num_heads, L = D.num_layers, M = plan.M;
    const size_t md = align_up((size_t)M * d * sizeof(float), 256) / sizeof(float);
    float *ws = (float *)workspace;
    float *h0 = ws, *h1 = ws + md, *qkv = ws + 2 * md, *att = ws + 5 * md, *ffn = ws + 6 * md;
    void *h16 = ffn + 2 * md;
    const size_t kv = plan.kv_stride;
    const int dn = w->dn();
    const float scale = 1.0f / sqrtf((float)dn);
    const float qs = vsk_attention_qscale(scale);
    const bool f16x3 = plan.linear == VS_ARITH_F16X3;
    auto frag = [&](size_t f, size_t h) { return w->p(f16x3 ? h : f); };
    const float *pe_rows = pk ? pk->pe_rows : (w->has_pe ? w->p(w->pe) : nullptr);
    {
        StageScope ps(VS_STAGE_EMBED, st);
        switch (plan.embed) {
        case VS_EMBED_CLS: {
            VS_LAUNCH(vsk_linear(x, w->p(w->embed_w), frag(w->f_embed_w, w->h_embed_w), w->p(w->embed_b), h1, B * Tf, d,
                                 D.in_features, 0, pe_rows, Tf, plan.mode_linear, st));
            uint8_t *mask1 = key_pad_mask ? (uint8_t *)workspace + need_core : nullptr;
            VS_LAUNCH(vsk_insert_cls(h1, cls, key_pad_mask, h0, mask1, B, Tf, d, st));
            key_pad_mask = mask1;
        } break;
        case VS_EMBED_BF16_QKV: {
            const LayerOff &N = w->layers[0];
            const VskNextQkv nq{w->p(N.b_qkv), w->p(N.bqkv), qkv, T, H, qs};
            VS_LAUNCH(vsk_embed_bf16(x, w->p(w->b_embed), w->p(w->embed_b), pe_rows, T, h0, M, d, D.in_features, &nq, st));
        } break;
        case VS_EMBED_SPLITK:
            VS_LAUNCH(vsk_linear_parts(x, frag(w->f_embed_w, w->h_embed_w), qkv, M, d, D.in_features, 8, st, f16x3));
            VS_LAUNCH(vsk_sum_parts_pe(qkv, 8, w->p(w->embed_b), pe_rows, T, h0, M, d, st));
            break;
        case VS_EMBED_GEMM:
            VS_LAUNCH(vsk_linear(x, w->p(w->embed_w), frag(w->f_embed_w, w->h_embed_w), w->p(w->embed_b), h0, M, d, D.in_features, 0,
                                 pe_rows, T, plan.mode_linear, st));
            break;
        }
    }
    if (plan.layer == VS_LAYER_RING) VS_LAUNCH(vsk_to_bf16(h0, h16, (size_t)M * d, st));
    for (int l = 0; l < L; ++l) {
        const LayerOff &P = w->layers[l];
        const bool last = l == L - 1;
        float *dst = (last && hidden) ? hidden : h0;
        const float *head_w = last ? w->p(w->final_w) : nullptr, *head_b = last ? w->p(w->final_b) : nullptr;
        float *head_out = last ? scores : nullptr;
        VskNextQkv nq{}, *next = nullptr;
        if (plan.next_qkv && !last) {
            const LayerOff &N = w->layers[l + 1];
            nq = VskNextQkv{w->p(N.b_qkv), w->p(N.bqkv), qkv, T, H, qs};
            next = &nq;
        }
        if (plan.layer == VS_LAYER_RING) {
            StageScope ps(VS_STAGE_QKV, st);
            VS_LAUNCH(vsk_gemm16(h16, w->p(P.r_wqkv), w->p(P.bqkv), qkv, M, 3 * d, d, 3, 1, T, H, d / H, qs, st));
        } else if (l == 0 ? plan.embed != VS_EMBED_BF16_QKV : !plan.tail_writes_qkv()) {
            StageScope ps(VS_STAGE_QKV, st);
            VS_LAUNCH(vsk_qkv(h0, w->p(P.wqkv), frag(P.f_wqkv, P.h_wqkv), w->p(P.bqkv), qkv, B, T, d, H, plan.mode_qkv, st,
                              plan.qkv16 ? qs : 1.0f));
        }
        if (ins) {
            for (int i = 0; i < ins->n_layers; ++i) {
                if (ins->layers[i] != l) continue;
                const size_t rows = (size_t)B * H * T;
                if (pk) {
                    VS_LAUNCH(vsk_attention_probs_packed(qkv, qkv + kv, pk->cu, ins->maps ? ins->maps + i * ins->map_stride : nullptr,
                                                         ins->received ? ins->received + i * rows : nullptr,
                                                         ins->entropy ? ins->entropy + i * rows : nullptr, ins->videos, H, M, ins->tiles,
                                                         d / H, scale, ins->workspace, st));
                    continue;
                }
                VS_LAUNCH(vsk_attention_probs(qkv, qkv + kv, key_pad_mask, ins->maps ? ins->maps + i * rows * T : nullptr,
                                              ins->received ? ins->received + i * rows : nullptr,
                                              ins->entropy ? ins->entropy + i * rows : nullptr, B, H, T, d / H, scale, ins->workspace, st));
            }
        }
        {
            StageScope ps(VS_STAGE_ATTENTION, st);
            switch (plan.attention) {
            case VS_ATT_PACKED:
                VS_LAUNCH(vsk_attention_packed(qkv, qkv + kv, qkv + 2 * kv, att, H, M, d / H, scale, pk->cu, pk->work, pk->nwork, pk->nw,
                                               plan.mode_attention, st));
                break;
            case VS_ATT_DH256:
                VS_LAUNCH(vst_attention_fwd(qkv, qkv + kv, qkv + 2 * kv, key_pad_mask, att, ffn, B, H, T, 256, scale, 0ull, 0u, 0.f, st, nullptr));
                break;
            case VS_ATT_SPLITKV:
                VS_LAUNCH(vsk_attention_splitkv(qkv, qkv + kv, qkv + 2 * kv, key_pad_mask, att, B, H, T, d / H, scale, st));
                break;
            case VS_ATT_LOWPREC:
                VS_LAUNCH(vsk_attention_bf16(qkv, qkv + kv, qkv + 2 * kv, key_pad_mask, att, B, H, T, d / H, scale, plan.mode_attention, st));
                break;
            case VS_ATT_EXACT:
                VS_LAUNCH(vsk_attention(qkv, qkv + kv, qkv + 2 * kv, key_pad_mask, att, B, H, T, d / H, scale, st));
                break;
            }
        }
        if (plan.ln1 != VS_LN_NONE) {
            StageScope ps(VS_STAGE_OUTPROJ_LN, st);
            switch (plan.ln1) {
            case VS_LN_SPLITK_ROWS:
                VS_LAUNCH(vsk_linear_parts(att, frag(P.f_wo, P.h_wo), qkv, M, d, d, 2, st, f16x3));
                VS_LAUNCH(vsk_rows_res_ln(qkv, h0, w->p(P.ln1g), w->p(P.ln1b), h1, M, d, nullptr, nullptr, 0, 0, nullptr, st, nullptr, dn,
                                          2, w->p(P.bo)));
                break;
            case VS_LN_GEMM_ROWS:
                VS_LAUNCH(vsk_linear(att, w->p(P.wo), frag(P.f_wo, P.h_wo), w->p(P.bo), qkv, M, d, d, 0, nullptr, 1, plan.mode_linear, st));
                VS_LAUNCH(vsk_rows_res_ln(qkv, h0, w->p(P.ln1g), w->p(P.ln1b), h1, M, d, nullptr, nullptr, 0, 0, nullptr, st, nullptr, dn));
                break;
            default:
                VS_LAUNCH(vsk_linear_res_ln(att, w->p(P.wo), frag(P.f_wo, P.h_wo), w->p(P.bo), h0, w->p(P.ln1g), w->p(P.ln1b), h1, M, d, d,
                                            nullptr, nullptr, 0, 0, nullptr, plan.mode_qkv, st));
            }
        }
        switch (plan.layer) {
        case VS_LAYER_RING: {
            {
                StageScope ps(VS_STAGE_OUTPROJ_LN, st);
                VS_LAUNCH(vsk_gemm16(att, w->p(P.r_wo), w->p(P.bo), qkv, M, d, d, 0, 0, 1, 0, 0, 1.0f, st));
                VS_LAUNCH(vsk_rows_res_ln(qkv, h0, w->p(P.ln1g), w->p(P.ln1b), h1, M, d, nullptr, nullptr, 0, 0, nullptr, st, h16, dn));
            }
            {
                StageScope ps(VS_STAGE_FC1, st);
                VS_LAUNCH(vsk_gemm16(h16, w->p(P.r_w1), w->p(P.b1), ffn, M, 4 * d, d, 1, 1, 1, 0, 0, 1.0f, st));
            }
            StageScope ps(VS_STAGE_FC2_LN, st);
            VS_LAUNCH(vsk_gemm16(ffn, w->p(P.r_w2), w->p(P.b2), att, M, d, 4 * d, 0, 0, 1, 0, 0, 1.0f, st));
            VS_LAUNCH(vsk_rows_res_ln(att, h1, w->p(P.ln2g), w->p(P.ln2b), dst, M, d, head_w, head_b, D.num_classes, sig, head_out, st,
                                      last ? nullptr : h16, dn));
        } break;
        case VS_LAYER_BF16_TAIL: {
            StageScope ps(VS_STAGE_FC2_LN, st);
            VS_LAUNCH(vsk_mlp_bf16(h0, att, w->p(P.bo), w->p(P.ln1g), w->p(P.ln1b), w->p(P.b_mlp), w->p(P.b1), w->p(P.b2),
                                   w->p(P.ln2g), w->p(P.ln2b), dst, M, d, head_w, head_b, D.num_classes, sig, head_out, next, st));
        } break;
        case VS_LAYER_BF16_MLP: {
            StageScope ps(VS_STAGE_FC2_LN, st);
            VS_LAUNCH(vsk_mlp_bf16(h1, nullptr, nullptr, nullptr, nullptr, w->p(P.b_mlp), w->p(P.b1), w->p(P.b2), w->p(P.ln2g), w->p(P.ln2b), dst, M, d,
                                   head_w, head_b, D.num_classes, sig, head_out, next, st));
        } break;
        case VS_LAYER_EXACT_PAIR: {
            if (M >= vsk_options().layer_tail_min_rows) {
                StageScope ps(VS_STAGE_FC2_LN, st);
                const LayerOff *N = last ? nullptr : &w->layers[l + 1];
                VS_LAUNCH(vsk_layer_tail(att, w->p(P.wo), w->p(P.bo), h0, w->p(P.ln1g), w->p(P.ln1b), w->p(P.w1), w->p(P.b1), ffn, w->p(P.w2),
                                         w->p(P.b2), w->p(P.ln2g), w->p(P.ln2b), dst, N ? w->p(N->wqkv) : nullptr, N ? w->p(N->bqkv) : nullptr,
                                         qkv, head_w, head_b, D.num_classes, sig, head_out, B, T, d, H, st));
                break;
            }
            {
                StageScope ps(VS_STAGE_FC1, st);
                VS_LAUNCH(vsk_outproj_ln_fc1(att, w->p(P.wo), w->p(P.bo), h0, w->p(P.ln1g), w->p(P.ln1b), h1, w->p(P.w1), w->p(P.b1), ffn, M, d, st));
            }
            StageScope ps(VS_STAGE_FC2_LN, st);
            if (last) {
                VS_LAUNCH(vsk_linear_res_ln(ffn, w->p(P.w2), w->p(P.f_w2), w->p(P.b2), h1, w->p(P.ln2g), w->p(P.ln2b), dst, M, d, 4 * d,
                                            head_w, head_b, D.num_classes, sig, head_out, 0, st));
            } else {
                const LayerOff &N = w->layers[l + 1];
                VS_LAUNCH(vsk_fc2_ln_qkv(ffn, w->p(P.w2), w->p(P.b2), h1, w->p(P.ln2g), w->p(P.ln2b), dst, w->p(N.wqkv), w->p(N.bqkv), qkv,
                                         B, T, d, H, st));
            }
        } break;
        case VS_LAYER_STAGES: {
            {
                StageScope ps(VS_STAGE_FC1, st);
                VS_LAUNCH(vsk_linear(h1, w->p(P.w1), frag(P.f_w1, P.h_w1), w->p(P.b1), ffn, M, 4 * d, d, 1, nullptr, 1, plan.mode_ffn, st));
            }
            StageScope ps(VS_STAGE_FC2_LN, st);
            switch (plan.ln2) {
            case VS_LN_SPLITK_ROWS:
                VS_LAUNCH(vsk_linear_parts(ffn, frag(P.f_w2, P.h_w2), qkv, M, d, 4 * d, 4, st, f16x3));
                VS_LAUNCH(vsk_rows_res_ln(qkv, h1, w->p(P.ln2g), w->p(P.ln2b), dst, M, d, head_w, head_b, D.num_classes, sig, head_out, st, nullptr, dn,
                                          4, w->p(P.b2)));
                break;
            case VS_LN_GEMM_ROWS:
                VS_LAUNCH(vsk_linear(ffn, w->p(P.w2), frag(P.f_w2, P.h_w2), w->p(P.b2), att, M, d, 4 * d, 0, nullptr, 1, plan.mode_linear, st));
                VS_LAUNCH(vsk_rows_res_ln(att, h1, w->p(P.ln2g), w->p(P.ln2b), dst, M, d, head_w, head_b, D.num_classes, sig, head_out, st, nullptr, dn));
                break;
            default:
                VS_LAUNCH(vsk_linear_res_ln(ffn, w->p(P.w2), frag(P.f_w2, P.h_w2), w->p(P.b2), h1, w->p(P.ln2g), w->p(P.ln2b), dst, M, d,
                                            4 * d, head_w, head_b, D.num_classes, sig, head_out, plan.mode_ffn, st));
            }
        } break;
        }
    }
    return VS_OK;
}
}

extern "C" {

int vs_scorer_forward(const vs_weights *w, const float *x, const uint8_t *key_pad_mask, int32_t B,
                      int32_t T, uint32_t flags, float *scores, float *hidden, void *workspace,
                      size_t workspace_bytes, void *stream) {
    return forward_core(w, x, key_pad_mask, B, T, flags, scores, hidden, workspace, workspace_bytes, stream, nullptr);
}

size_t vs_scorer_workspace_bytes_cls(const vs_weights *w, int32_t B, int32_t T) {
    if (!w || B <= 0 || T <= 0) return 0;
    return vs_scorer_workspace_bytes(w, B, T + 1) + align_up((size_t)B * (T + 1), 256);
}

int vs_scorer_forward_cls(const vs_weights *w, const float *x, const uint8_t *key_pad_mask, const float *cls_token,
                          int32_t B, int32_t T, uint32_t flags, float *scores, float *hidden, void *workspace,
                          size_t workspace_bytes, void *stream) {
    if (!cls_token) return vs_failf(VS_ERR_INVALID, "cls_token is NULL");
    return forward_core(w, x, key_pad_mask, B, T, flags, scores, hidden, workspace, workspace_bytes, stream, nullptr, cls_token);
}

size_t vs_inspect_workspace_bytes(const vs_weights *w, int32_t B, int32_t T, int32_t with_cls) {
    if (!w || B <= 0 || T <= 0) return 0;
    const size_t core = with_cls ? vs_scorer_workspace_bytes_cls(w, B, T) : vs_scorer_workspace_bytes(w, B, T);
    return align_up(core, 256) + vsk_attention_probs_workspace_bytes(B, w->desc.num_heads, T + (with_cls ? 1 : 0));
}

int vs_inspect_forward(const vs_weights *w, const float *x, const uint8_t *key_pad_mask, const float *cls_token,
                       int32_t B, int32_t T, const int32_t *layers, int32_t n_layers,
                       float *scores, float *hidden, float *maps, float *received, float *entropy,
                       void *workspace, size_t workspace_bytes, void *stream) {
    if (!w) return vs_failf(VS_ERR_INVALID, "weights is NULL");
    if (!layers || n_layers <= 0) return vs_failf(VS_ERR_INVALID, "layers is NULL or n_layers=%d", n_layers);
    for (int i = 0; i < n_layers; ++i) {
        if (layers[i] < 0 || layers[i] >= w->desc.num_layers)
            return vs_failf(VS_ERR_INVALID, "layers[%d]=%d out of range (num_layers=%d)", i, layers[i], w->desc.num_layers);
        if (i && layers[i] <= layers[i - 1]) return vs_failf(VS_ERR_INVALID, "layers must be strictly ascending (layers[%d]=%d after %d)", i, layers[i], layers[i - 1]);
    }
    if (!maps && !received && !entropy) return vs_failf(VS_ERR_INVALID, "maps, received and entropy are all NULL");
    if (((uintptr_t)maps | (uintptr_t)received | (uintptr_t)entropy) & 15)
        return vs_failf(VS_ERR_INVALID, "maps / received / entropy must be 16-byte aligned");
    if (B <= 0 || T <= 0) return vs_failf(VS_ERR_INVALID, "B=%d T=%d", B, T);
    const size_t core = align_up(cls_token ? vs_scorer_workspace_bytes_cls(w, B, T) : vs_scorer_workspace_bytes(w, B, T), 256);
    const size_t need = vs_inspect_workspace_bytes(w, B, T, cls_token != nullptr);
    if (!workspace || workspace_bytes < need)
        return vs_failf(VS_ERR_WORKSPACE, "workspace %zu bytes < %zu needed", workspace_bytes, need);
    const InspectHook ins{layers, n_layers, maps, received, entropy, (char *)workspace + core};
    return forward_core(w, x, key_pad_mask, B, T, 0u, scores, hidden, workspace, core, stream, nullptr, cls_token, &ins);
}

size_t vs_attention_probs_workspace_bytes(int32_t B, int32_t H, int32_t T) {
    if (B <= 0 || H <= 0 || T <= 0) return 0;
    return vsk_attention_probs_workspace_bytes(B, H, T);
}

int vs_attention_probs_f32(const float *q, const float *k, const uint8_t *key_pad_mask, float *maps, float *received,
                           float *entropy, int32_t B, int32_t H, int32_t T, int32_t dh, float scale, void *workspace,
                           size_t workspace_bytes, void *stream) {
    if (!q || !k) return vs_failf(VS_ERR_INVALID, "q / k is NULL");
    if (!maps && !received && !entropy) return vs_failf(VS_ERR_INVALID, "maps, received and entropy are all NULL");
    if (B <= 0 || H <= 0 || T <= 0) return vs_failf(VS_ERR_INVALID, "B=%d H=%d T=%d", B, H, T);
    if (dh != 32 && dh != 64 && dh != 128 && dh != 256) return vs_failf(VS_ERR_INVALID, "head_dim=%d unsupported (32, 64, 128 or 256)", dh);
    if (((uintptr_t)q | (uintptr_t)k | (uintptr_t)maps | (uintptr_t)received | (uintptr_t)entropy) & 15)
        return vs_failf(VS_ERR_INVALID, "q / k / maps / received / entropy must be 16-byte aligned");
    const size_t need = vsk_attention_probs_workspace_bytes(B, H, T);
    if (!workspace || workspace_bytes < need)
        return vs_failf(VS_ERR_WORKSPACE, "workspace %zu bytes < %zu needed", workspace_bytes, need);
    if ((uintptr_t)workspace & 255) return vs_failf(VS_ERR_INVALID, "workspace must be 256-byte aligned");
    VS_LAUNCH(vsk_attention_probs(q, k, key_pad_mask, maps, received, entropy, B, H, T, dh, scale, workspace, (hipStream_t)stream));
    return VS_OK;
}

static int packed_plan(const vs_weights *w, const int32_t *lengths, int32_t B, std::vector<int> &cu,
                       std::vector<int> &work, int &nw, int aprec = 0) {
    if (!w || !lengths || B <= 0) return vs_failf(VS_ERR_INVALID, "weights/lengths is NULL or B=%d", B);
    const vs_model_desc &D = w->desc;
    const int dh = D.d_model / D.num_heads;
    if (dh != 32 && dh != 64 && dh != 128) return vs_failf(VS_ERR_INVALID, "packed batches need head_dim 32, 64 or 128 (got %d)", dh);
    cu.assign(B + 1, 0);
    long long r8 = 0, r4 = 0;
    for (int b = 0; b < B; ++b) {
        const int t = lengths[b];
        if (t <= 0) return vs_failf(VS_ERR_INVALID, "lengths[%d]=%d", b, t);
        if (w->has_pe && t > D.max_len)
            return vs_failf(VS_ERR_INVALID, "T=%d exceeds the positional table (max_len=%d)", t, D.max_len);
        if ((long long)cu[b] + t > (1ll << 30)) return vs_failf(VS_ERR_INVALID, "too many frames");
        cu[b + 1] = cu[b] + t;
        r8 += (t + 255) / 256 * 256;
        r4 += (t + 127) / 128 * 128;
    }
    nw = vs_packed_waves(dh, aprec, r8, r4);
    const int qb = 32 * nw;
    work.clear();
    for (int b = 0; b < B; ++b)
        for (int q = 0; q < (lengths[b] + qb - 1) / qb; ++q) { work.push_back(b); work.push_back(q); }
    return VS_OK;
}

static size_t packed_plan_capacity(const int32_t *lengths, int32_t B) {
    size_t n = 0;
    for (int b = 0; b < B; ++b) n += (size_t)(lengths[b] + 127) / 128;
    return n;
}

size_t vs_scorer_workspace_bytes_packed(const vs_weights *w, const int32_t *lengths, int32_t B) {
    std::vector<int> cu, work;
    int nw = 0;
    if (packed_plan(w, lengths, B, cu, work, nw) != VS_OK) return 0;
    const size_t md = align_up((size_t)cu[B] * w->desc.d_model * sizeof(float), 256);
    return 11 * md + align_up((cu.size() + 2 * packed_plan_capacity(lengths, B)) * sizeof(int), 256);
}

static int forward_packed(const vs_weights *w, const float *x, const int32_t *lengths, const int32_t *lengths_dev,
                          int32_t B, uint32_t flags, float *scores, float *hidden, void *workspace,
                          size_t workspace_bytes, void *stream, const InspectHook *ins) {
    if (!lengths_dev) return vs_failf(VS_ERR_INVALID, "lengths_dev is NULL");
    if (!w) return vs_failf(VS_ERR_INVALID, "weights is NULL");
    if ((flags & VS_FLAG_BF16_ATTENTION) && (flags & VS_FLAG_F16X3_ATTENTION))
        return vs_failf(VS_ERR_INVALID, "VS_FLAG_BF16_ATTENTION and VS_FLAG_F16X3_ATTENTION are exclusive");
    const int aprec = vs_attention_prec(flags);
    std::vector<int> cu, work;
    int nw = 0;
    if (aprec == 2 && w->desc.d_model / w->desc.num_heads == 128)
        return vs_failf(VS_ERR_INVALID, "VS_FLAG_F16X3_ATTENTION needs head_dim 32 or 64 (got 128)");
    if (int rc = packed_plan(w, lengths, B, cu, work, nw, aprec)) return rc;
    const size_t need = vs_scorer_workspace_bytes_packed(w, lengths, B);
    if (!workspace || workspace_bytes < need)
        return vs_failf(VS_ERR_WORKSPACE, "workspace %zu bytes < %zu needed", workspace_bytes, need);
    if ((uintptr_t)workspace & 255) return vs_failf(VS_ERR_INVALID, "workspace must be 256-byte aligned");
    const int M = cu[B], d = w->desc.d_model;
    const size_t md = align_up((size_t)M * d * sizeof(float), 256);
    hipStream_t st = (hipStream_t)stream;
    float *pe_rows = (float *)((char *)workspace + 10 * md);
    int *plan = (int *)((char *)workspace + 11 * md);
    const size_t cap = packed_plan_capacity(lengths, B);
    if (work.size() / 2 > cap) return vs_failf(VS_ERR_INVALID, "internal: packed plan %zu > capacity %zu", work.size() / 2, cap);
    VS_LAUNCH(vsk_plan_packed(lengths_dev, B, 32 * nw, plan, plan + cu.size(), (int)cap, st));
    PackedInfo pk{nullptr, plan, plan + cu.size(), (int)(work.size() / 2), nw};
    if (w->has_pe) {
        int tmax = 0;
        for (int b = 0; b < B; ++b) tmax = lengths[b] > tmax ? lengths[b] : tmax;
        VS_LAUNCH(vsk_gather_rows(w->p(w->pe), pk.cu, B, tmax, d, pe_rows, st));
        pk.pe_rows = pe_rows;
    }
    return forward_core(w, x, nullptr, 1, M, flags, scores, hidden, workspace, 10 * md, stream, &pk, nullptr, ins);
}

int vs_scorer_forward_packed(const vs_weights *w, const float *x, const int32_t *lengths, const int32_t *lengths_dev,
                             int32_t B, uint32_t flags, float *scores, float *hidden, void *workspace,
                             size_t workspace_bytes, void *stream) {
    return forward_packed(w, x, lengths, lengths_dev, B, flags, scores, hidden, workspace, workspace_bytes, stream, nullptr);
}

static int probs_packed_sizes(const int32_t *lengths, int32_t B, int &M, int &tiles, size_t &sumsq) {
    if (!lengths || B <= 0) return vs_failf(VS_ERR_INVALID, "lengths is NULL or B=%d", B);
    long long m = 0, n = 0;
    sumsq = 0;
    for (int b = 0; b < B; ++b) {
        const int t = lengths[b];
        if (t <= 0) return vs_failf(VS_ERR_INVALID, "lengths[%d]=%d", b, t);
        m += t;
        n += (t + 31) / 32;
        sumsq += (size_t)t * (size_t)t;
        if (m > (1ll << 30)) return vs_failf(VS_ERR_INVALID, "too many frames");
    }
    M = (int)m;
    tiles = (int)n;
    return VS_OK;
}

// ... 302 lines not shown
```

Before: 12.35 million frames/s.

## Fuse embedding GEMM with first-layer QKV projection in exact fp32 path

Adds a kernel that computes the input embedding (with bias and positional rows) and then, from the register-resident result, produces layer 0's QKV projection in head-split layout. This replaces separate embed and QKV launches for large exact-fp32 batches. It saves one launch and a full re-read of the embedded activations from memory. The shared row-tile device routine moves into an include file with a new tail mode. It is gated by a row-count threshold and shape checks.

Result: no change. 12.40 million frames/s (median of 6 runs) (+0.4%).

```diff
diff --git a/video-summarization_amd/_lib.py b/video-summarization_amd/_lib.py
--- a/video-summarization_amd/_lib.py
+++ b/video-summarization_amd/_lib.py
@@ -13,7 +13,7 @@
 INCLUDE = os.path.join(ROOT, "include")
 LIB_PATH = os.path.join(HERE, "libvsscore.so")
 DIAG_LIB_PATH = os.path.join(HERE, "libvsscore_diag.so")
-SOURCES = ("vs_kernels.hip", "vs_attention.hip", "vs_attention_w64.hip", "vs_mlp_fused.hip", "vs_gemm_ring.hip", "vs_scorer.cpp", "vs_eval.cpp",
+SOURCES = ("vs_kernels.hip", "vs_embed_qkv.hip", "vs_attention.hip", "vs_attention_w64.hip", "vs_mlp_fused.hip", "vs_gemm_ring.hip", "vs_scorer.cpp", "vs_eval.cpp",
            "vs_train_kernels.hip", "vs_train_attention.hip", "vs_train_attention_bf16.hip", "vs_train_gemm_rows.hip", "vs_pretrain_kernels.hip",
            "vs_train.cpp", "vs_segment.hip", "vs_segment_gram.hip", "vs_segment.cpp", "vs_optim.hip", "vs_attention_maps.hip",
            "vs_eval_device.hip", "vs_eval_device.cpp", "vs_summary.hip", "vs_summary.cpp", "vs_batch.hip", "vs_cnn.hip", "vs_cnn.cpp",
diff --git a/video-summarization_amd/csrc/vs_embed_qkv.hip b/video-summarization_amd/csrc/vs_embed_qkv.hip
--- /dev/null
+++ b/video-summarization_amd/csrc/vs_embed_qkv.hip
@@ -0,0 +1,36 @@
+#include "vs_device.h"
+#include "vs_kernels.h"
+#include "vs_linear_pick.h"
+
+namespace {
+
+__device__ __forceinline__ unsigned long long stamp() { return vs_stamp(); }
+
+#include "vs_ln_rows_tiles.inc"
+
+template <bool PE>
+__global__ __launch_bounds__(256, 2) void gemm_rows_embed_qkv(
+    const float *__restrict__ x, const float *__restrict__ We, const float *__restrict__ be, const float *__restrict__ pe,
+    float *__restrict__ h0, int M, int K, const float *__restrict__ Wqkv, const float *__restrict__ bqkv, float *__restrict__ qkv,
+    int T, int H, int dhs) {
+    ln_rows_tiles<8, 0, 0, 0, PE ? 5 : 6>(x, We, be, pe, nullptr, nullptr, h0, M, K, nullptr, nullptr, 0, 0, nullptr, nullptr,
+                                          LnTail{Wqkv, bqkv, qkv, T, H, dhs}, LnPhase2{});
+}
+
+}
+
+int vsk_embed_qkv(const float *x, const float *We, const float *be, const float *pe_rows, float *h0, const float *Wqkv,
+                  const float *bqkv, float *qkv, int B, int T, int d, int H, int in_features, hipStream_t st) {
+    const int M = B * T;
+    if (!vsk_embed_qkv_shape_ok(M, d, H, in_features)) return -1;
+    const int cus = vsk_device_cus();
+    if (cus <= 0) return (int)hipErrorInvalidDevice;
+    const int blocks = vsk_row_tile_grid(M, cus);
+    const int dhs = vsk_head_dim_shift(d / H);
+    if (pe_rows != nullptr)
+        hipLaunchKernelGGL(gemm_rows_embed_qkv<true>, dim3(blocks), dim3(256), 0, st, x, We, be, pe_rows, h0, M, in_features, Wqkv, bqkv, qkv, T, H, dhs);
+    else
+        hipLaunchKernelGGL(gemm_rows_embed_qkv<false>, dim3(blocks), dim3(256), 0, st, x, We, be, pe_rows, h0, M, in_features, Wqkv, bqkv, qkv, T, H, dhs);
+    VSK_CHECK_LAUNCH();
+    return 0;
+}
diff --git a/video-summarization_amd/csrc/vs_forward_plan.h b/video-summarization_amd/csrc/vs_forward_plan.h
--- a/video-summarization_amd/csrc/vs_forward_plan.h
+++ b/video-summarization_amd/csrc/vs_forward_plan.h
@@ -20,6 +20,7 @@
     int lp_embed_unfused;
     int exact_unfused;
     int layer_tail_min_rows;
+    int embed_qkv_min_rows;
     int mlp_abl;
     int attn_w64_checked;
     int attn_w64_abl;
@@ -34,6 +35,10 @@
 inline bool vsk_mlp_bf16_supported(int d) { return d == 256; }
 inline bool vsk_gemm16_supported(int M, int N, int K) { return M > 0 && N > 0 && N % 32 == 0 && K >= 32 && K % 32 == 0; }
 inline bool vsk_layer_fused_supported(int M, int d, int skinny_rows) { return d == 256 && M > skinny_rows && M <= (1 << 20); }
+inline bool vsk_embed_qkv_shape_ok(int M, int d, int H, int in_features) {
+    if (d != 256 || M <= 0 || M > (1 << 20) || in_features < 16 || in_features % 16 || H <= 0 || d % H) return false;
+    return d / H == 32 || d / H == 64 || d / H == 128;
+}
 
 enum VsArith { VS_ARITH_EXACT = 0, VS_ARITH_BF16 = 1, VS_ARITH_F16X3 = 2 };
 enum VsEmbedForm {
@@ -172,6 +177,12 @@
     return VS_OK;
 }
 
+inline bool vsk_embed_qkv_applies(const VsForwardIn &in, const VsForwardPlan &p, const VskOptions &opt) {
+    return p.embed == VS_EMBED_GEMM && p.linear == VS_ARITH_EXACT && p.attention_arith == VS_ARITH_EXACT &&
+           in.norm_width == in.d_model && !in.cls && !(in.flags & VS_FLAG_SPLITK) && in.num_layers > 0 &&
+           vsk_embed_qkv_shape_ok(p.M, in.d_model, in.num_heads, in.in_features) && p.M >= opt.embed_qkv_min_rows;
+}
+
 inline int vs_packed_waves(int dh, int aprec, long long r8, long long r4) {
     if (dh == 128) return aprec == 1 ? 8 : 4;
     return (!(aprec != 0 && dh == 32) && r8 * 100 <= r4 * 105) ? 8 : 4;
diff --git a/video-summarization_amd/csrc/vs_kernels.h b/video-summarization_amd/csrc/vs_kernels.h
--- a/video-summarization_amd/csrc/vs_kernels.h
+++ b/video-summarization_amd/csrc/vs_kernels.h
@@ -44,6 +44,8 @@
                    const float *W1, const float *b1, float *hidden, const float *W2, const float *b2, const float *g2, const float *be2,
                    float *out, const float *Wqkv, const float *bqkv, float *qkv, const float *score_w, const float *score_b,
                    int num_classes, int sigmoid, float *scores, int B, int T, int d, int H, hipStream_t st);
+int vsk_embed_qkv(const float *x, const float *We, const float *be, const float *pe_rows, float *h0, const float *Wqkv,
+                  const float *bqkv, float *qkv, int B, int T, int d, int H, int in_features, hipStream_t st);
 int vsk_rows_res_ln(const float *a, const float *res, const float *gamma, const float *beta, float *out, int M, int d,
                     const float *score_w, const float *score_b, int num_classes, int sigmoid, float *scores,
                     hipStream_t st, void *out16 = nullptr, int dn = 0,
diff --git a/video-summarization_amd/csrc/vs_kernels.hip b/video-summarization_amd/csrc/vs_kernels.hip
--- a/video-summarization_amd/csrc/vs_kernels.hip
+++ b/video-summarization_amd/csrc/vs_kernels.hip
@@ -569,479 +569,7 @@
     }
 }
 
-struct LnTail {
-    const float *W2, *b2;
-    float *C2;
-    int T, H, dhs;
-};
-struct LnPhase2 {
-    const float *W, *bias, *gamma, *beta;
-    float *out;
-    LnTail tl;
-};
-
-template <int NT, int PREC, int A16, int DIAG, int TAIL>
-__device__ __forceinline__ void ln_rows_tiles(
-    const float *__restrict__ A, const float *__restrict__ W, const float *__restrict__ bias,
-    const float *__restrict__ res, const float *__restrict__ gamma, const float *__restrict__ beta,
-    float *__restrict__ out, int M, int K,
-    const float *__restrict__ score_w, const float *__restrict__ score_b, int num_classes,
-    int sigmoid, float *__restrict__ scores, unsigned long long *__restrict__ diag, const LnTail tl, const LnPhase2 p2) {
-    static_assert(TAIL == 0 || (NT == 8 && PREC == 0 && DIAG == 0), "the register-fed tail exists for exact fp32 at d_model 256");
-    constexpr int BM = 128, N = 32 * NT, BK = 16, LD = BK + 4;
-    constexpr int WL = (N * BK / 4 + 255) / 256;
-    constexpr bool TWO = TAIL >= 3;
-    constexpr int NPH = TWO ? 2 : 1;
-    constexpr int TN2 = TAIL == 2 ? 3 * N : 4 * N;
-    constexpr int SMALL2 = TAIL == 3 ? 3 * N + 3 * N : TAIL == 4 ? 3 * N : 0;
-    __shared__ __attribute__((aligned(16))) float smem[2 * (BM + N) * LD + 4 * N + (TAIL != 0 ? TN2 : 0) + SMALL2];
-    float *gam_s = smem + 2 * (BM + N) * LD, *bet_s = gam_s + N, *sw_s = bet_s + N, *bias_s = sw_s + N;
-    float *bias2_s = bias_s + N;
-    float *small2_s = bias2_s + TN2;
-
-    int tid = threadIdx.x, lane = tid & 63, wave = tid >> 6;
-    int r = lane & 31, h = lane >> 5;
-    const int ntiles = (M + BM - 1) / BM;
-    const int nk = K / BK;
-
-    constexpr float SC = PREC == 2 ? F16X3_WS : 1.0f;
-    for (int i = tid; i < N; i += 256) { gam_s[i] = gamma[i]; bet_s[i] = beta[i]; bias_s[i] = bias[i] * SC; }
-    if constexpr (TAIL != 0)
-        for (int i = tid; i < TN2; i += 256) bias2_s[i] = tl.b2[i];
-    if constexpr (TWO) {
-        for (int i = tid; i < N; i += 256) { small2_s[i] = p2.gamma[i]; small2_s[N + i] = p2.beta[i]; small2_s[2 * N + i] = p2.bias[i]; }
-        if constexpr (TAIL == 3)
-            for (int i = tid; i < 3 * N; i += 256) small2_s[3 * N + i] = p2.tl.b2[i];
-    }
-
-    int lrow = tid >> 2, lc4 = (tid & 3) * 4;
-    f32x4 pa[2], pw[WL];
-    u32x2 pa16[2];
-    const float *aptr[2], *wptr[WL];
-    const unsigned short *aptr16[2];
-#pragma unroll
-    for (int i = 0; i < WL; ++i) {
-        int wrow = lrow + 64 * i; wrow = wrow < N ? wrow : N - 1;
-        wptr[i] = W + (size_t)wrow * K + lc4;
-    }
-    static_assert(PREC != 0 || N % 64 == 0, "the exact-fp32 staging map covers W without a guard");
-    __amdgpu_buffer_rsrc_t ars = __builtin_amdgcn_make_buffer_rsrc(const_cast<float *>(A), 0, 0, 0x00020000);
-    __amdgpu_buffer_rsrc_t wrs = __builtin_amdgcn_make_buffer_rsrc(const_cast<float *>(W), 0, N * K * 4, 0x00020000);
-    int aoff[2], woff[WL];
-#pragma unroll
-    for (int i = 0; i < WL; ++i) woff[i] = ((lrow + 64 * i) * K + lc4) * 4;
-    auto gload = [&](int i, int kb) __attribute__((always_inline)) {
-        if (i < 2) pa[i] = __builtin_bit_cast(f32x4, __builtin_amdgcn_raw_buffer_load_b128(ars, aoff[i], kb, 0));
-        else pw[i - 2] = __builtin_bit_cast(f32x4, __builtin_amdgcn_raw_buffer_load_b128(wrs, woff[i - 2], kb, 0));
-    };
-    constexpr int LDB = 12;
-    auto stage = [&](int buf) __attribute__((always_inline)) {
-        float *As = smem + buf * (BM + N) * LD, *Ws = As + BM * LD;
-        if constexpr (PREC == 2) {
-#pragma unroll
-            for (int i = 0; i < 2; ++i) {
-                u32x2 hi, lo;
-                split_f16x4((const float *)&pa[i], hi, lo);
-                *(u32x2 *)&As[(lrow + 64 * i) * LD + lc4 / 2] = hi;
-                *(u32x2 *)&As[(lrow + 64 * i) * LD + 8 + lc4 / 2] = lo;
-            }
-#pragma unroll
-            for (int i = 0; i < WL; ++i)
-                if (lrow + 64 * i < N) {
-                    u32x2 hi, lo;
-                    const f32x4 ws = pw[i] * F16X3_WS;
-                    split_f16x4((const float *)&ws, hi, lo);
-                    *(u32x2 *)&Ws[(lrow + 64 * i) * LD + lc4 / 2] = hi;
-                    *(u32x2 *)&Ws[(lrow + 64 * i) * LD + 8 + lc4 / 2] = lo;
-                }
-        } else if constexpr (PREC == 1) {
-#pragma unroll
-            for (int i = 0; i < 2; ++i) {
-                u32x2 u;
-                if constexpr (A16 != 0) u = pa16[i];
-                else { u[0] = pack_bf16(pa[i][0], pa[i][1]); u[1] = pack_bf16(pa[i][2], pa[i][3]); }
-                *(u32x2 *)&As[(lrow + 64 * i) * LDB + lc4 / 2] = u;
-            }
-#pragma unroll
-            for (int i = 0; i < WL; ++i)
-                if (lrow + 64 * i < N) {
-                    u32x2 u; u[0] = pack_bf16(pw[i][0], pw[i][1]); u[1] = pack_bf16(pw[i][2], pw[i][3]);
-                    *(u32x2 *)&Ws[(lrow + 64 * i) * LDB + lc4 / 2] = u;
-                }
-        } else {
-#pragma unroll
-            for (int i = 0; i < 2; ++i) *(f32x4 *)&As[(lrow + 64 * i) * LD + lc4] = pa[i];
-#pragma unroll
-            for (int i = 0; i < WL; ++i) *(f32x4 *)&Ws[(lrow + 64 * i) * LD + lc4] = pw[i];
-        }
-    };
-
-    f32x16 acc[NT];
-
-    constexpr int TCH = 128, TWB = 4 * 32 * 36, TBUF = TCH * 36;
-    static_assert(TAIL == 0 || TWB + 2 * TBUF <= 2 * (BM + N) * LD, "corners and weight tiles fit the staging area");
-    int r2 = tid >> 3, c2 = (tid & 7) * 4;
-    __amdgpu_buffer_rsrc_t wrs2 = __builtin_amdgcn_make_buffer_rsrc(const_cast<float *>(tl.W2), 0, TN2 * N * 4, 0x00020000);
-    const float *tbias_s = bias2_s;
-    int woff2 = (r2 * N + c2) * 4;
-    f32x4 pw2[4];
-    f32x16 U[4];
-    auto tail_soff = [&](int c, int kt) __attribute__((always_inline)) { return (TCH * c * N + 32 * kt) * 4; };
-    auto tail_load = [&](int i, int soff) __attribute__((always_inline)) {
-        pw2[i] = __builtin_bit_cast(f32x4, __builtin_amdgcn_raw_buffer_load_b128(wrs2, woff2, soff + 32 * i * N * 4, 0));
-    };
-    auto tail_stage = [&](int buf) __attribute__((always_inline)) {
-#pragma unroll
-        for (int i = 0; i < 4; ++i) *(f32x4 *)&smem[TWB + buf * TBUF + (r2 + 32 * i) * 36 + c2] = pw2[i];
-    };
-    auto bias_mfma = [&](int c) __attribute__((always_inline)) {
-        const f32x16 zero = {0.f, 0.f, 0.f, 0.f, 0.f, 0.f, 0.f, 0.f, 0.f, 0.f, 0.f, 0.f, 0.f, 0.f, 0.f, 0.f};
-#pragma unroll
-        for (int jj = 0; jj < 4; ++jj) {
-            const float bv = tbias_s[TCH * c + 32 * jj + r];
-            U[jj] = MFMA32(h == 0 ? bv : 0.f, 1.0f, zero);
-        }
-    };
-    auto tail_step = [&](auto ktc, int nsoff) __attribute__((always_inline)) {
-        constexpr int kt = decltype(ktc)::value;
-        const float *wp = smem + TWB + (kt & 1) * TBUF + r * 36 + 4 * h;
-        float *wd = smem + TWB + ((kt + 1) & 1) * TBUF + r2 * 36 + c2;
-        f32x4 fw[3];
-        fw[0] = *(const f32x4 *)wp;
-        fw[1] = *(const f32x4 *)(wp + 32 * 36);
-        __builtin_amdgcn_sched_barrier(0);
-#pragma unroll
-        for (int t = 0; t < 16; ++t) {
-            const int g = t / 4, jj = t % 4;
-            if (t + 2 < 16) fw[(t + 2) % 3] = *(const f32x4 *)(wp + 32 * ((t + 2) % 4) * 36 + 8 * ((t + 2) / 4));
-            if (t < 4) tail_load(t, nsoff);
-            if (t >= 12) *(f32x4 *)(wd + 32 * (t - 12) * 36) = pw2[t - 12];
-#pragma unroll
-            for (int s2 = 0; s2 < 4; ++s2) U[jj] = MFMA32(fw[t % 3][s2], acc[kt][4 * g + s2], U[jj]);
-            __builtin_amdgcn_sched_group_barrier(0x008, 1, 0);
-            if (t + 2 < 16) __builtin_amdgcn_sched_group_barrier(0x100, 1, 0);
-            if (t < 4) __builtin_amdgcn_sched_group_barrier(0x020, 1, 0);
-            __builtin_amdgcn_sched_group_barrier(0x008, 3, 0);
-            if (t >= 12) __builtin_amdgcn_sched_group_barrier(0x200, 1, 0);
-            __builtin_amdgcn_sched_barrier(0);
-        }
-        __syncthreads();
-    };
-
-    unsigned long long dsum[3] = {0, 0, 0}, tbegin = 0, tq = 0, ktiles = 0;
-    if constexpr (DIAG != 0) tbegin = stamp();
-    for (int tile = blockIdx.x; tile < ntiles; tile += gridDim.x) {
-        if constexpr (DIAG != 0) tq = stamp();
-        const int m0 = tile * BM;
-      static_for<NPH>([&](auto phc) __attribute__((always_inline)) {
-        constexpr int PH = decltype(phc)::value;
-        constexpr bool P1 = TWO && PH == 1;
-        constexpr int PT = !TWO ? TAIL : PH == 0 ? 1 : TAIL == 3 ? 2 : 0;
-        constexpr int PTN2 = PT == 2 ? 3 * N : 4 * N, TNC = PTN2 / TCH;
-        const LnTail ptl = P1 ? p2.tl : tl;
-        const float *pA = P1 ? tl.C2 : A;
-        const int pK = P1 ? 4 * N : K, pnk = P1 ? 4 * N / BK : nk;
-        const float *pgam_s = P1 ? small2_s : gam_s, *pbet_s = P1 ? small2_s + N : bet_s, *pbias_s = P1 ? small2_s + 2 * N : bias_s;
-        float *pout = P1 ? p2.out : out;
-        if constexpr (TWO) {
-            asm volatile("" : "+v"(tid));
-            lane = tid & 63; wave = tid >> 6; r = lane & 31; h = lane >> 5;
-            lrow = tid >> 2; lc4 = (tid & 3) * 4; r2 = tid >> 3; c2 = (tid & 7) * 4; woff2 = (r2 * N + c2) * 4;
-            wrs = __builtin_amdgcn_make_buffer_rsrc(const_cast<float *>(P1 ? p2.W : W), 0, N * pK * 4, 0x00020000);
-#pragma unroll
-            for (int i = 0; i < WL; ++i) woff[i] = ((lrow + 64 * i) * pK + lc4) * 4;
-            if constexpr (PT != 0) {
-                wrs2 = __builtin_amdgcn_make_buffer_rsrc(const_cast<float *>(ptl.W2), 0, PTN2 * N * 4, 0x00020000);
-                tbias_s = P1 ? small2_s + 3 * N : bias2_s;
-            }
-        }
-        int row = m0 + 32 * wave + r;
-        const bool row_ok = row < M;
-        row = row_ok ? row : M - 1;
-#pragma unroll
-        for (int i = 0; i < 2; ++i) {
-            int ar = m0 + lrow + 64 * i; ar = ar < M ? ar : M - 1;
-            if constexpr (A16 != 0) {
-                aptr16[i] = (const unsigned short *)A + (size_t)ar * K + lc4;
-                pa16[i] = *(const u32x2 *)aptr16[i];
-            } else if constexpr (PREC == 0) {
-                aoff[i] = ((ar - m0) * pK + lc4) * 4;
-            } else {
-                aptr[i] = A + (size_t)ar * K + lc4;
-                pa[i] = *(const f32x4 *)aptr[i];
-            }
-        }
-        if constexpr (PREC == 0) {
-            ars = __builtin_amdgcn_make_buffer_rsrc(const_cast<float *>(pA + (size_t)m0 * pK), 0, (M - m0 < BM ? M - m0 : BM) * pK * 4, 0x00020000);
-            if constexpr (P1) {
-#pragma unroll
-                for (int i = 2; i < 2 + WL; ++i) gload(i, 0);
-                asm volatile("s_waitcnt vmcnt(0)" ::: "memory");
-                __builtin_amdgcn_fence(__ATOMIC_RELEASE, "workgroup");
-                __syncthreads();
-                __builtin_amdgcn_fence(__ATOMIC_ACQUIRE, "workgroup");
-#pragma unroll
-                for (int i = 0; i < 2; ++i) gload(i, 0);
-            } else {
-#pragma unroll
-                for (int i = 0; i < 2 + WL; ++i) gload(i, 0);
-            }
-        } else {
-#pragma unroll
-            for (int i = 0; i < WL; ++i) pw[i] = *(const f32x4 *)wptr[i];
-        }
-        if constexpr (!P1) {
-            const float *rp = res + (size_t)row * N + 4 * h;
-#pragma unroll
-            for (int j = 0; j < NT; ++j)
-#pragma unroll
-                for (int q = 0; q < 4; ++q) {
-                    f32x4 rv = *(const f32x4 *)(rp + 32 * j + 8 * q);
-                    if constexpr (PREC == 2) rv *= SC;
-#pragma unroll
-                    for (int e = 0; e < 4; ++e) acc[j][4 * q + e] = rv[e];
-                }
-        }
-        if constexpr (!P1) __syncthreads();
-        stage(0);
-        __syncthreads();
-        if constexpr (DIAG != 0) { dsum[2] += stamp() - tq; ktiles += nk; }
-
-        for (int kt = 0; kt < pnk; ++kt) {
-            const int kn = kt + 1 < pnk ? kt + 1 : kt;
-            const float *As = smem + (kt & 1) * (BM + N) * LD, *Ws = As + BM * LD;
-            if constexpr (PREC == 2) {
-                const float *arow = As + (32 * wave + r) * LD + 4 * h;
-                const f16x8 ah = __builtin_bit_cast(f16x8, *(const u32x4 *)arow);
-                const f16x8 al = __builtin_bit_cast(f16x8, *(const u32x4 *)(arow + 8));
-#pragma unroll
-                for (int i = 0; i < 2; ++i) pa[i] = *(const f32x4 *)(aptr[i] + kn * BK);
-#pragma unroll
-                for (int i = 0; i < WL; ++i) pw[i] = *(const f32x4 *)(wptr[i] + kn * BK);
-#pragma unroll
-                for (int j = 0; j < NT; ++j) {
-                    const float *wrow = Ws + (32 * j + r) * LD + 4 * h;
-                    const f16x8 wh = __builtin_bit_cast(f16x8, *(const u32x4 *)wrow);
-                    const f16x8 wl = __builtin_bit_cast(f16x8, *(const u32x4 *)(wrow + 8));
-                    acc[j] = MFMA_F16(wl, ah, acc[j]);
-                    acc[j] = MFMA_F16(wh, al, acc[j]);
-                    acc[j] = MFMA_F16(wh, ah, acc[j]);
-                }
-                stage((kt + 1) & 1);
-                __syncthreads();
-                continue;
-            }
-            if constexpr (PREC == 1) {
-                const bf16x8 fa = __builtin_bit_cast(bf16x8, *(const u32x4 *)(As + (32 * wave + r) * LDB + 4 * h));
-#pragma unroll
-                for (int i = 0; i < 2; ++i) {
-                    if constexpr (A16 != 0) pa16[i] = *(const u32x2 *)(aptr16[i] + kn * BK);
-                    else pa[i] = *(const f32x4 *)(aptr[i] + kn * BK);
-                }
-#pragma unroll
-                for (int i = 0; i < WL; ++i) pw[i] = *(const f32x4 *)(wptr[i] + kn * BK);
-#pragma unroll
-                for (int j = 0; j < NT; ++j) {
-                    const bf16x8 fw = __builtin_bit_cast(bf16x8, *(const u32x4 *)(Ws + (32 * j + r) * LDB + 4 * h));
-                    acc[j] = MFMA_BF16(fw, fa, acc[j]);
-                }
-                stage((kt + 1) & 1);
-                __syncthreads();
-                continue;
-            }
-            const float *ap = As + (32 * wave + r) * LD + 4 * h;
-            const float *wp = Ws + r * LD + 4 * h;
-            constexpr int NS = 2 * NT, NL = 2 + WL;
-            constexpr int LPS = (NL + NT - 1) / NT;
-            constexpr int WB = NS - (NL + LPS - 1) / LPS;
-            static_assert(BK == 16 && (NL + LPS - 1) / LPS <= NT, "loads and LDS writes of a k-tile occupy distinct steps");
-            f32x4 fa[2], fw[3];
-            fa[0] = *(const f32x4 *)ap;
-            fw[0] = *(const f32x4 *)wp;
-            fw[1] = *(const f32x4 *)(wp + 32 * LD);
-            fa[1] = *(const f32x4 *)(ap + 8);
-            __builtin_amdgcn_sched_barrier(0);
-#pragma unroll
-            for (int t = 0; t < NS; ++t) {
-                const int g = t / NT, j = t % NT;
-                if (t + 2 < NS) fw[(t + 2) % 3] = *(const f32x4 *)(wp + 32 * ((t + 2) % NT) * LD + 8 * ((t + 2) / NT));
-                int nld = 0, nwr = 0;
-#pragma unroll
-                for (int q = 0; q < LPS; ++q) {
-                    const int il = t * LPS + q, iw = (t - WB) * LPS + q;
-                    if (il < NL) { gload(il, kn * (BK * 4)); ++nld; }
-                    if (t >= WB && iw < NL) {
-                        float *Ad = smem + ((kt + 1) & 1) * (BM + N) * LD, *Wd = Ad + BM * LD;
-                        if (iw < 2) *(f32x4 *)&Ad[(lrow + 64 * iw) * LD + lc4] = pa[iw];
-                        else *(f32x4 *)&Wd[(lrow + 64 * (iw - 2)) * LD + lc4] = pw[iw - 2];
-                        ++nwr;
-                    }
-                }
-#pragma unroll
-                for (int s2 = 0; s2 < 4; ++s2) acc[j] = MFMA32(fw[t % 3][s2], fa[g][s2], acc[j]);
-                __builtin_amdgcn_sched_group_barrier(0x008, 1, 0);
-                if (t + 2 < NS) __builtin_amdgcn_sched_group_barrier(0x100, 1, 0);
-#pragma unroll
-                for (int q = 0; q < LPS; ++q)
-                    if (q < nld) __builtin_amdgcn_sched_group_barrier(0x020, 1, 0);
-                __builtin_amdgcn_sched_group_barrier(0x008, 3, 0);
-#pragma unroll
-                for (int q = 0; q < LPS; ++q)
-                    if (q < nwr) __builtin_amdgcn_sched_group_barrier(0x200, 1, 0);
-                __builtin_amdgcn_sched_barrier(0);
-            }
-            if constexpr (DIAG != 0) {
-                const unsigned long long tb = stamp();
-                __syncthreads();
-                dsum[0] += stamp() - tb;
-            } else
-                __syncthreads();
-        }
-        if constexpr (DIAG != 0) tq = stamp();
-        if constexpr (PT != 0) {
-#pragma unroll
-            for (int i = 0; i < 4; ++i) tail_load(i, tail_soff(0, 0));
-        }
-
-        float sum = 0.f;
-#pragma unroll
-        for (int j = 0; j < NT; ++j) {
-            float pj = 0.f;
-#pragma unroll
-            for (int q = 0; q < 4; ++q) {
-                const f32x4 bv = *(const f32x4 *)&pbias_s[32 * j + 8 * q + 4 * h];
-#pragma unroll
-                for (int e = 0; e < 4; ++e) { acc[j][4 * q + e] += bv[e]; pj += acc[j][4 * q + e]; }
-            }
-            sum += pj;
-        }
-        sum = pair_sum(sum);
-        const float mean = sum * (1.0f / N);
-        float sq = 0.f;
-#pragma unroll
-        for (int j = 0; j < NT; ++j) {
-            float pj = 0.f;
-#pragma unroll
-            for (int t = 0; t < 16; ++t) { const float c = acc[j][t] - mean; acc[j][t] = c; pj += c * c; }
-            sq += pj;
-        }
-        sq = pair_sum(sq);
-        const float rstd = 1.0f / sqrtf(sq * (1.0f / N) + 1e-5f * (SC * SC));
-        float *tp = smem + wave * (32 * 36);
-        const int trow = lane >> 3, tc4 = (lane & 7) * 4;
-#pragma unroll
-        for (int j = 0; j < NT; ++j) {
-#pragma unroll
-            for (int q = 0; q < 4; ++q) {
-                const f32x4 gv = *(const f32x4 *)&pgam_s[32 * j + 8 * q + 4 * h];
-                const f32x4 bv = *(const f32x4 *)&pbet_s[32 * j + 8 * q + 4 * h];
-                f32x4 y;
-#pragma unroll
-                for (int e = 0; e < 4; ++e) { y[e] = acc[j][4 * q + e] * rstd * gv[e] + bv[e]; acc[j][4 * q + e] = y[e]; }
-                if constexpr (!TWO || P1) *(f32x4 *)&tp[r * 36 + 8 * q + 4 * h] = y;
-            }
-            if constexpr (TWO && !P1) __builtin_amdgcn_sched_barrier(0);
-            if constexpr (!TWO || P1) {
-#pragma unroll
-                for (int pq = 0; pq < 4; ++pq) {
-                    const f32x4 v = *(const f32x4 *)&tp[(trow + 8 * pq) * 36 + tc4];
-                    const int orow = m0 + 32 * wave + trow + 8 * pq;
-                    if (orow < M) *(f32x4 *)(pout + (size_t)orow * N + 32 * j + tc4) = v;
-                }
-            }
-        }
-        if constexpr (!TWO || (P1 && TAIL == 4))
-        if (score_w != nullptr) {
-            for (int c = 0; c < num_classes; ++c) {
-                __syncthreads();
-                for (int i = tid; i < N; i += 256) sw_s[i] = score_w[(size_t)c * N + i];
-                __syncthreads();
-                float dot = 0.f;
-#pragma unroll
-                for (int j = 0; j < NT; ++j) {
-                    float pj = 0.f;
-#pragma unroll
-                    for (int q = 0; q < 4; ++q) {
-                        const f32x4 wv = *(const f32x4 *)&sw_s[32 * j + 8 * q + 4 * h];
-#pragma unroll
-                        for (int e = 0; e < 4; ++e) pj += acc[j][4 * q + e] * wv[e];
-                    }
-                    dot += pj;
-                }
-                dot = pair_sum(dot);
-                if (h == 0 && row_ok) {
-                    float sc = dot + score_b[c];
-                    if (sigmoid) sc = 1.0f / (1.0f + expf(-sc));
-                    scores[(size_t)row * num_classes + c] = sc;
-                }
-            }
-        }
-        if constexpr (DIAG != 0) dsum[1] += stamp() - tq;
-        if constexpr (PT != 0) {
-            tail_stage(0);
-            int rowoff[4];
-            __amdgpu_buffer_rsrc_t crs;
-            if constexpr (PT == 1) {
-                crs = __builtin_amdgcn_make_buffer_rsrc(ptl.C2 + (size_t)m0 * PTN2, 0, (M - m0 < BM ? M - m0 : BM) * PTN2 * 4, 0x00020000);
-#pragma unroll
-                for (int p = 0; p < 4; ++p) rowoff[p] = ((32 * wave + trow + 8 * p) * PTN2 + tc4) * 4;
-            } else {
-                crs = __builtin_amdgcn_make_buffer_rsrc(ptl.C2, 0, 0, 0x00020000);
-#pragma unroll
-                for (int p = 0; p < 4; ++p) {
-                    const int orow = m0 + 32 * wave + trow + 8 * p;
-                    const int bb = orow / ptl.T, tt = orow - bb * ptl.T;
-                    rowoff[p] = orow < M ? (((bb * ptl.H * ptl.T + tt) << ptl.dhs) + tc4) * 4 : (int)0x80000000;
-                }
-            }
-            bias_mfma(0);
-            __syncthreads();
-            for (int c = 0; c < TNC; ++c) {
-                const int cn = c + 1 < TNC ? c + 1 : c;
-                static_for<8>([&](auto ktc) __attribute__((always_inline)) {
-                    constexpr int kt = decltype(ktc)::value;
-                    tail_step(ktc, kt < 7 ? tail_soff(c, kt + 1) : tail_soff(cn, 0));
-                });
-                if constexpr (PT == 2) {
-                    const int which = c >> 1;
-                    crs = __builtin_amdgcn_make_buffer_rsrc(ptl.C2 + (size_t)which * M * N, 0, M * N * 4, 0x00020000);
-                }
-#pragma unroll
-                for (int jj = 0; jj < 4; ++jj) {
-                    __builtin_amdgcn_sched_barrier(0);
-#pragma unroll
-                    for (int q = 0; q < 4; ++q) {
-                        f32x4 v;
-#pragma unroll
-                        for (int e = 0; e < 4; ++e) v[e] = PT == 1 ? relu1(U[jj][4 * q + e]) : U[jj][4 * q + e];
-                        *(f32x4 *)&tp[r * 36 + 8 * q + 4 * h] = v;
-                    }
-                    int soff;
-                    if constexpr (PT == 1) soff = (TCH * c + 32 * jj) * 4;
-                    else {
-                        const int cc = (TCH * c + 32 * jj) & (N - 1), head = cc >> ptl.dhs, e0 = cc - (head << ptl.dhs);
-                        soff = (((head * ptl.T) << ptl.dhs) + e0) * 4;
-                    }
-#pragma unroll
-                    for (int p = 0; p < 4; ++p) {
-                        const f32x4 v = *(const f32x4 *)&tp[(trow + 8 * p) * 36 + tc4];
-                        __builtin_amdgcn_raw_buffer_store_b128(__builtin_bit_cast(u32x4, v), crs, rowoff[p], soff, 0);
-                    }
-                }
-                __builtin_amdgcn_sched_barrier(0);
-                bias_mfma(cn);
-            }
-        }
-      });
-    }
-    if constexpr (DIAG != 0) {
-        if (diag != nullptr && lane == 0) {
-            unsigned long long *o = diag + ((size_t)blockIdx.x * 4 + wave) * 8;
-            o[0] = dsum[0]; o[1] = dsum[1]; o[2] = dsum[2]; o[3] = 0; o[4] = 0;
-            o[5] = stamp() - tbegin; o[6] = ktiles; o[7] = tbegin;
-        }
-    }
-}
+#include "vs_ln_rows_tiles.inc"
 
 template <int NT, int PREC = 0, int A16 = 0, int DIAG = 0>
 __global__ __launch_bounds__(256, 2) void gemm_ln_rows(
diff --git a/video-summarization_amd/csrc/vs_ln_rows_tiles.inc b/video-summarization_amd/csrc/vs_ln_rows_tiles.inc
--- /dev/null
+++ b/video-summarization_amd/csrc/vs_ln_rows_tiles.inc
@@ -0,0 +1,534 @@
+struct LnTail {
+    const float *W2, *b2;
+    float *C2;
+    int T, H, dhs;
+};
+struct LnPhase2 {
+    const float *W, *bias, *gamma, *beta;
+    float *out;
+    LnTail tl;
+};
+
+template <int NT, int PREC, int A16, int DIAG, int TAIL>
+__device__ __forceinline__ void ln_rows_tiles(
+    const float *__restrict__ A, const float *__restrict__ W, const float *__restrict__ bias,
+    const float *__restrict__ res, const float *__restrict__ gamma, const float *__restrict__ beta,
+    float *__restrict__ out, int M, int K,
+    const float *__restrict__ score_w, const float *__restrict__ score_b, int num_classes,
+    int sigmoid, float *__restrict__ scores, unsigned long long *__restrict__ diag, const LnTail tl, const LnPhase2 p2) {
+    static_assert(TAIL == 0 || (NT == 8 && PREC == 0 && DIAG == 0), "the register-fed tail exists for exact fp32 at d_model 256");
+    static_assert(TAIL >= 0 && TAIL <= 6, "TAIL 0 .. 6");
+    constexpr int BM = 128, N = 32 * NT, BK = 16, LD = BK + 4;
+    constexpr int WL = (N * BK / 4 + 255) / 256;
+    constexpr bool TWO = TAIL == 3 || TAIL == 4;
+    constexpr bool EMB = TAIL == 5 || TAIL == 6;
+    constexpr int NPH = TWO ? 2 : 1;
+    constexpr int TN2 = TAIL == 2 || EMB ? 3 * N : 4 * N;
+    constexpr int SMALL2 = TAIL == 3 ? 3 * N + 3 * N : TAIL == 4 ? 3 * N : 0;
+    __shared__ __attribute__((aligned(16))) float smem[2 * (BM + N) * LD + 4 * N + (TAIL != 0 ? TN2 : 0) + SMALL2];
+    float *gam_s = smem + 2 * (BM + N) * LD, *bet_s = gam_s + N, *sw_s = bet_s + N, *bias_s = sw_s + N;
+    float *bias2_s = bias_s + N;
+    float *small2_s = bias2_s + TN2;
+
+    int tid = threadIdx.x, lane = tid & 63, wave = tid >> 6;
+    int r = lane & 31, h = lane >> 5;
+    const int ntiles = (M + BM - 1) / BM;
+    const int nk = K / BK;
+
+    constexpr float SC = PREC == 2 ? F16X3_WS : 1.0f;
+    for (int i = tid; i < N; i += 256) {
+        if constexpr (!EMB) { gam_s[i] = gamma[i]; bet_s[i] = beta[i]; }
+        bias_s[i] = bias[i] * SC;
+    }
+    if constexpr (TAIL != 0)
+        for (int i = tid; i < TN2; i += 256) bias2_s[i] = tl.b2[i];
+    if constexpr (TWO) {
+        for (int i = tid; i < N; i += 256) { small2_s[i] = p2.gamma[i]; small2_s[N + i] = p2.beta[i]; small2_s[2 * N + i] = p2.bias[i]; }
+        if constexpr (TAIL == 3)
+            for (int i = tid; i < 3 * N; i += 256) small2_s[3 * N + i] = p2.tl.b2[i];
+    }
+
+    int lrow = tid >> 2, lc4 = (tid & 3) * 4;
+    f32x4 pa[2], pw[WL];
+    u32x2 pa16[2];
+    const float *aptr[2], *wptr[WL];
+    const unsigned short *aptr16[2];
+#pragma unroll
+    for (int i = 0; i < WL; ++i) {
+        int wrow = lrow + 64 * i; wrow = wrow < N ? wrow : N - 1;
+        wptr[i] = W + (size_t)wrow * K + lc4;
+    }
+    static_assert(PREC != 0 || N % 64 == 0, "the exact-fp32 staging map covers W without a guard");
+    __amdgpu_buffer_rsrc_t ars = __builtin_amdgcn_make_buffer_rsrc(const_cast<float *>(A), 0, 0, 0x00020000);
+    __amdgpu_buffer_rsrc_t wrs = __builtin_amdgcn_make_buffer_rsrc(const_cast<float *>(W), 0, N * K * 4, 0x00020000);
+    int aoff[2], woff[WL];
+#pragma unroll
+    for (int i = 0; i < WL; ++i) woff[i] = ((lrow + 64 * i) * K + lc4) * 4;
+    auto gload = [&](int i, int kb) __attribute__((always_inline)) {
+        if (i < 2) pa[i] = __builtin_bit_cast(f32x4, __builtin_amdgcn_raw_buffer_load_b128(ars, aoff[i], kb, 0));
+        else pw[i - 2] = __builtin_bit_cast(f32x4, __builtin_amdgcn_raw_buffer_load_b128(wrs, woff[i - 2], kb, 0));
+    };
+    constexpr int LDB = 12;
+    auto stage = [&](int buf) __attribute__((always_inline)) {
+        float *As = smem + buf * (BM + N) * LD, *Ws = As + BM * LD;
+        if constexpr (PREC == 2) {
+#pragma unroll
+            for (int i = 0; i < 2; ++i) {
+                u32x2 hi, lo;
+                split_f16x4((const float *)&pa[i], hi, lo);
+                *(u32x2 *)&As[(lrow + 64 * i) * LD + lc4 / 2] = hi;
+                *(u32x2 *)&As[(lrow + 64 * i) * LD + 8 + lc4 / 2] = lo;
+            }
+#pragma unroll
+            for (int i = 0; i < WL; ++i)
+                if (lrow + 64 * i < N) {
+                    u32x2 hi, lo;
+                    const f32x4 ws = pw[i] * F16X3_WS;
+                    split_f16x4((const float *)&ws, hi, lo);
+                    *(u32x2 *)&Ws[(lrow + 64 * i) * LD + lc4 / 2] = hi;
+                    *(u32x2 *)&Ws[(lrow + 64 * i) * LD + 8 + lc4 / 2] = lo;
+                }
+        } else if constexpr (PREC == 1) {
+#pragma unroll
+            for (int i = 0; i < 2; ++i) {
+                u32x2 u;
+                if constexpr (A16 != 0) u = pa16[i];
+                else { u[0] = pack_bf16(pa[i][0], pa[i][1]); u[1] = pack_bf16(pa[i][2], pa[i][3]); }
+                *(u32x2 *)&As[(lrow + 64 * i) * LDB + lc4 / 2] = u;
+            }
+#pragma unroll
+            for (int i = 0; i < WL; ++i)
+                if (lrow + 64 * i < N) {
+                    u32x2 u; u[0] = pack_bf16(pw[i][0], pw[i][1]); u[1] = pack_bf16(pw[i][2], pw[i][3]);
+                    *(u32x2 *)&Ws[(lrow + 64 * i) * LDB + lc4 / 2] = u;
+                }
+        } else {
+#pragma unroll
+            for (int i = 0; i < 2; ++i) *(f32x4 *)&As[(lrow + 64 * i) * LD + lc4] = pa[i];
+#pragma unroll
+            for (int i = 0; i < WL; ++i) *(f32x4 *)&Ws[(lrow + 64 * i) * LD + lc4] = pw[i];
+        }
+    };
+
+    f32x16 acc[NT];
+
+    constexpr int TCH = 128, TWB = 4 * 32 * 36, TBUF = TCH * 36;
+    static_assert(TAIL == 0 || TWB + 2 * TBUF <= 2 * (BM + N) * LD, "corners and weight tiles fit the staging area");
+    int r2 = tid >> 3, c2 = (tid & 7) * 4;
+    __amdgpu_buffer_rsrc_t wrs2 = __builtin_amdgcn_make_buffer_rsrc(const_cast<float *>(tl.W2), 0, TN2 * N * 4, 0x00020000);
+    const float *tbias_s = bias2_s;
+    int woff2 = (r2 * N + c2) * 4;
+    f32x4 pw2[4];
+    f32x16 U[4];
+    auto tail_soff = [&](int c, int kt) __attribute__((always_inline)) { return (TCH * c * N + 32 * kt) * 4; };
+    auto tail_load = [&](int i, int soff) __attribute__((always_inline)) {
+        pw2[i] = __builtin_bit_cast(f32x4, __builtin_amdgcn_raw_buffer_load_b128(wrs2, woff2, soff + 32 * i * N * 4, 0));
+    };
+    auto tail_stage = [&](int buf) __attribute__((always_inline)) {
+#pragma unroll
+        for (int i = 0; i < 4; ++i) *(f32x4 *)&smem[TWB + buf * TBUF + (r2 + 32 * i) * 36 + c2] = pw2[i];
+    };
+    auto bias_mfma = [&](int c) __attribute__((always_inline)) {
+        const f32x16 zero = {0.f, 0.f, 0.f, 0.f, 0.f, 0.f, 0.f, 0.f, 0.f, 0.f, 0.f, 0.f, 0.f, 0.f, 0.f, 0.f};
+#pragma unroll
+        for (int jj = 0; jj < 4; ++jj) {
+            const float bv = tbias_s[TCH * c + 32 * jj + r];
+            U[jj] = MFMA32(h == 0 ? bv : 0.f, 1.0f, zero);
+        }
+    };
+    auto tail_step = [&](auto ktc, int nsoff) __attribute__((always_inline)) {
+        constexpr int kt = decltype(ktc)::value;
+        const float *wp = smem + TWB + (kt & 1) * TBUF + r * 36 + 4 * h;
+        float *wd = smem + TWB + ((kt + 1) & 1) * TBUF + r2 * 36 + c2;
+        f32x4 fw[3];
+        fw[0] = *(const f32x4 *)wp;
+        fw[1] = *(const f32x4 *)(wp + 32 * 36);
+        __builtin_amdgcn_sched_barrier(0);
+#pragma unroll
+        for (int t = 0; t < 16; ++t) {
+            const int g = t / 4, jj = t % 4;
+            if (t + 2 < 16) fw[(t + 2) % 3] = *(const f32x4 *)(wp + 32 * ((t + 2) % 4) * 36 + 8 * ((t + 2) / 4));
+            if (t < 4) tail_load(t, nsoff);
+            if (t >= 12) *(f32x4 *)(wd + 32 * (t - 12) * 36) = pw2[t - 12];
+#pragma unroll
+            for (int s2 = 0; s2 < 4; ++s2) U[jj] = MFMA32(fw[t % 3][s2], acc[kt][4 * g + s2], U[jj]);
+            __builtin_amdgcn_sched_group_barrier(0x008, 1, 0);
+            if (t + 2 < 16) __builtin_amdgcn_sched_group_barrier(0x100, 1, 0);
+            if (t < 4) __builtin_amdgcn_sched_group_barrier(0x020, 1, 0);
+            __builtin_amdgcn_sched_group_barrier(0x008, 3, 0);
+            if (t >= 12) __builtin_amdgcn_sched_group_barrier(0x200, 1, 0);
+            __builtin_amdgcn_sched_barrier(0);
+        }
+        __syncthreads();
+    };
+
+    unsigned long long dsum[3] = {0, 0, 0}, tbegin = 0, tq = 0, ktiles = 0;
+    if constexpr (DIAG != 0) tbegin = stamp();
+    for (int tile = blockIdx.x; tile < ntiles; tile += gridDim.x) {
+        if constexpr (DIAG != 0) tq = stamp();
+        const int m0 = tile * BM;
+      static_for<NPH>([&](auto phc) __attribute__((always_inline)) {
+        constexpr int PH = decltype(phc)::value;
+        constexpr bool P1 = TWO && PH == 1;
+        constexpr int PT = EMB ? 2 : !TWO ? TAIL : PH == 0 ? 1 : TAIL == 3 ? 2 : 0;
+        constexpr int PTN2 = PT == 2 ? 3 * N : 4 * N, TNC = PTN2 / TCH;
+        const LnTail ptl = P1 ? p2.tl : tl;
+        const float *pA = P1 ? tl.C2 : A;
+        const int pK = P1 ? 4 * N : K, pnk = P1 ? 4 * N / BK : nk;
+        const float *pgam_s = P1 ? small2_s : gam_s, *pbet_s = P1 ? small2_s + N : bet_s, *pbias_s = P1 ? small2_s + 2 * N : bias_s;
+        float *pout = P1 ? p2.out : out;
+        if constexpr (TWO || EMB) {
+            asm volatile("" : "+v"(tid));
+            lane = tid & 63; wave = tid >> 6; r = lane & 31; h = lane >> 5;
+            lrow = tid >> 2; lc4 = (tid & 3) * 4; r2 = tid >> 3; c2 = (tid & 7) * 4; woff2 = (r2 * N + c2) * 4;
+            if constexpr (TWO) wrs = __builtin_amdgcn_make_buffer_rsrc(const_cast<float *>(P1 ? p2.W : W), 0, N * pK * 4, 0x00020000);
+#pragma unroll
+            for (int i = 0; i < WL; ++i) woff[i] = ((lrow + 64 * i) * pK + lc4) * 4;
+            if constexpr (TWO && PT != 0) {
+                wrs2 = __builtin_amdgcn_make_buffer_rsrc(const_cast<float *>(ptl.W2), 0, PTN2 * N * 4, 0x00020000);
+                tbias_s = P1 ? small2_s + 3 * N : bias2_s;
+            }
+        }
+        int row = m0 + 32 * wave + r;
+        const bool row_ok = row < M;
+        row = row_ok ? row : M - 1;
+#pragma unroll
+        for (int i = 0; i < 2; ++i) {
+            int ar = m0 + lrow + 64 * i; ar = ar < M ? ar : M - 1;
+            if constexpr (A16 != 0) {
+                aptr16[i] = (const unsigned short *)A + (size_t)ar * K + lc4;
+                pa16[i] = *(const u32x2 *)aptr16[i];
+            } else if constexpr (PREC == 0) {
+                aoff[i] = ((ar - m0) * pK + lc4) * 4;
+            } else {
+                aptr[i] = A + (size_t)ar * K + lc4;
+                pa[i] = *(const f32x4 *)aptr[i];
+            }
+        }
+        if constexpr (PREC == 0) {
+            ars = __builtin_amdgcn_make_buffer_rsrc(const_cast<float *>(pA + (size_t)m0 * pK), 0, (M - m0 < BM ? M - m0 : BM) * pK * 4, 0x00020000);
+            if constexpr (P1) {
+#pragma unroll
+                for (int i = 2; i < 2 + WL; ++i) gload(i, 0);
+                asm volatile("s_waitcnt vmcnt(0)" ::: "memory");
+                __builtin_amdgcn_fence(__ATOMIC_RELEASE, "workgroup");
+                __syncthreads();
+                __builtin_amdgcn_fence(__ATOMIC_ACQUIRE, "workgroup");
+#pragma unroll
+                for (int i = 0; i < 2; ++i) gload(i, 0);
+            } else {
+#pragma unroll
+                for (int i = 0; i < 2 + WL; ++i) gload(i, 0);
+            }
+        } else {
+#pragma unroll
+            for (int i = 0; i < WL; ++i) pw[i] = *(const f32x4 *)wptr[i];
+        }
+        if constexpr (!P1 && !EMB) {
+            const float *rp = res + (size_t)row * N + 4 * h;
+#pragma unroll
+            for (int j = 0; j < NT; ++j)
+#pragma unroll
+                for (int q = 0; q < 4; ++q) {
+                    f32x4 rv = *(const f32x4 *)(rp + 32 * j + 8 * q);
+                    if constexpr (PREC == 2) rv *= SC;
+#pragma unroll
+                    for (int e = 0; e < 4; ++e) acc[j][4 * q + e] = rv[e];
+                }
+        }
+        if constexpr (!P1) __syncthreads();
+        stage(0);
+        __syncthreads();
+        if constexpr (DIAG != 0) { dsum[2] += stamp() - tq; ktiles += nk; }
+        if constexpr (EMB) {
+            const f32x16 zero = {0.f, 0.f, 0.f, 0.f, 0.f, 0.f, 0.f, 0.f, 0.f, 0.f, 0.f, 0.f, 0.f, 0.f, 0.f, 0.f};
+#pragma unroll
+            for (int j = 0; j < NT; ++j) {
+                const float bv = bias_s[32 * j + r];
+                acc[j] = MFMA32(h == 0 ? bv : 0.f, 1.0f, zero);
+            }
+        }
+
+        for (int kt = 0; kt < pnk; ++kt) {
+            const int kn = kt + 1 < pnk ? kt + 1 : kt;
+            const float *As = smem + (kt & 1) * (BM + N) * LD, *Ws = As + BM * LD;
+            if constexpr (PREC == 2) {
+                const float *arow = As + (32 * wave + r) * LD + 4 * h;
+                const f16x8 ah = __builtin_bit_cast(f16x8, *(const u32x4 *)arow);
+                const f16x8 al = __builtin_bit_cast(f16x8, *(const u32x4 *)(arow + 8));
+#pragma unroll
+                for (int i = 0; i < 2; ++i) pa[i] = *(const f32x4 *)(aptr[i] + kn * BK);
+#pragma unroll
+                for (int i = 0; i < WL; ++i) pw[i] = *(const f32x4 *)(wptr[i] + kn * BK);
+#pragma unroll
+                for (int j = 0; j < NT; ++j) {
+                    const float *wrow = Ws + (32 * j + r) * LD + 4 * h;
+                    const f16x8 wh = __builtin_bit_cast(f16x8, *(const u32x4 *)wrow);
+                    const f16x8 wl = __builtin_bit_cast(f16x8, *(const u32x4 *)(wrow + 8));
+                    acc[j] = MFMA_F16(wl, ah, acc[j]);
+                    acc[j] = MFMA_F16(wh, al, acc[j]);
+                    acc[j] = MFMA_F16(wh, ah, acc[j]);
+                }
+                stage((kt + 1) & 1);
+                __syncthreads();
+                continue;
+            }
+            if constexpr (PREC == 1) {
+                const bf16x8 fa = __builtin_bit_cast(bf16x8, *(const u32x4 *)(As + (32 * wave + r) * LDB + 4 * h));
+#pragma unroll
+                for (int i = 0; i < 2; ++i) {
+                    if constexpr (A16 != 0) pa16[i] = *(const u32x2 *)(aptr16[i] + kn * BK);
+                    else pa[i] = *(const f32x4 *)(aptr[i] + kn * BK);
+                }
+#pragma unroll
+                for (int i = 0; i < WL; ++i) pw[i] = *(const f32x4 *)(wptr[i] + kn * BK);
+#pragma unroll
+                for (int j = 0; j < NT; ++j) {
+                    const bf16x8 fw = __builtin_bit_cast(bf16x8, *(const u32x4 *)(Ws + (32 * j + r) * LDB + 4 * h));
+                    acc[j] = MFMA_BF16(fw, fa, acc[j]);
+                }
+                stage((kt + 1) & 1);
+                __syncthreads();
+                continue;
+            }
+            const float *ap = As + (32 * wave + r) * LD + 4 * h;
+            const float *wp = Ws + r * LD + 4 * h;
+            constexpr int NS = 2 * NT, NL = 2 + WL;
+            constexpr int LPS = (NL + NT - 1) / NT;
+            constexpr int WB = NS - (NL + LPS - 1) / LPS;
+            static_assert(BK == 16 && (NL + LPS - 1) / LPS <= NT, "loads and LDS writes of a k-tile occupy distinct steps");
+            f32x4 fa[2], fw[3];
+            fa[0] = *(const f32x4 *)ap;
+            fw[0] = *(const f32x4 *)wp;
+            fw[1] = *(const f32x4 *)(wp + 32 * LD);
+            fa[1] = *(const f32x4 *)(ap + 8);
+            __builtin_amdgcn_sched_barrier(0);
+#pragma unroll
+            for (int t = 0; t < NS; ++t) {
+                const int g = t / NT, j = t % NT;
+                if (t + 2 < NS) fw[(t + 2) % 3] = *(const f32x4 *)(wp + 32 * ((t + 2) % NT) * LD + 8 * ((t + 2) / NT));
+                int nld = 0, nwr = 0;
+#pragma unroll
+                for (int q = 0; q < LPS; ++q) {
+                    const int il = t * LPS + q, iw = (t - WB) * LPS + q;
+                    if (il < NL) { gload(il, kn * (BK * 4)); ++nld; }
+                    if (t >= WB && iw < NL) {
+                        float *Ad = smem + ((kt + 1) & 1) * (BM + N) * LD, *Wd = Ad + BM * LD;
+                        if (iw < 2) *(f32x4 *)&Ad[(lrow + 64 * iw) * LD + lc4] = pa[iw];
+                        else *(f32x4 *)&Wd[(lrow + 64 * (iw - 2)) * LD + lc4] = pw[iw - 2];
+                        ++nwr;
+                    }
+                }
+#pragma unroll
+                for (int s2 = 0; s2 < 4; ++s2) acc[j] = MFMA32(fw[t % 3][s2], fa[g][s2], acc[j]);
+                __builtin_amdgcn_sched_group_barrier(0x008, 1, 0);
+                if (t + 2 < NS) __builtin_amdgcn_sched_group_barrier(0x100, 1, 0);
+#pragma unroll
+                for (int q = 0; q < LPS; ++q)
+                    if (q < nld) __builtin_amdgcn_sched_group_barrier(0x020, 1, 0);
+                __builtin_amdgcn_sched_group_barrier(0x008, 3, 0);
+#pragma unroll
+                for (int q = 0; q < LPS; ++q)
+                    if (q < nwr) __builtin_amdgcn_sched_group_barrier(0x200, 1, 0);
+                __builtin_amdgcn_sched_barrier(0);
+            }
+            if constexpr (DIAG != 0) {
+                const unsigned long long tb = stamp();
+                __syncthreads();
+                dsum[0] += stamp() - tb;
+            } else
+                __syncthreads();
+        }
+        if constexpr (DIAG != 0) tq = stamp();
+        if constexpr (PT != 0 && !EMB) {
+#pragma unroll
+            for (int i = 0; i < 4; ++i) tail_load(i, tail_soff(0, 0));
+        }
+
+        float *tp;
+        int trow, tc4;
+        if constexpr (EMB) {
+            tp = smem + wave * (32 * 36);
+            trow = lane >> 3; tc4 = (lane & 7) * 4;
+            constexpr bool PE = TAIL == 5;
+            __amdgpu_buffer_rsrc_t prs = __builtin_amdgcn_make_buffer_rsrc(const_cast<float *>(res), 0, 0, 0x00020000);
+            if constexpr (PE) prs = __builtin_amdgcn_make_buffer_rsrc(const_cast<float *>(res), 0, tl.T * N * 4, 0x00020000);
+            const __amdgpu_buffer_rsrc_t hrs =
+                __builtin_amdgcn_make_buffer_rsrc(pout + (size_t)m0 * N, 0, (M - m0 < BM ? M - m0 : BM) * N * 4, 0x00020000);
+            const int poff = ((row % tl.T) * N + 4 * h) * 4;
+            int hoff[4];
+#pragma unroll
+            for (int p = 0; p < 4; ++p) hoff[p] = ((32 * wave + trow + 8 * p) * N + tc4) * 4;
+            f32x4 pv[4];
+            auto pe_load = [&](int j) __attribute__((always_inline)) {
+#pragma unroll
+                for (int q = 0; q < 4; ++q)
+                    pv[q] = __builtin_bit_cast(f32x4, __builtin_amdgcn_raw_buffer_load_b128(prs, poff, (32 * j + 8 * q) * 4, 0));
+            };
+            if constexpr (PE) pe_load(0);
+#pragma unroll
+            for (int j = 0; j < NT; ++j) {
+                __builtin_amdgcn_sched_barrier(0);
+                if constexpr (PE) {
+#pragma unroll
+                    for (int t = 0; t < 16; ++t) acc[j][t] += pv[t / 4][t % 4];
+                    if (j + 1 < NT) pe_load(j + 1);
+                }
+                if (j == NT - 1) {
+#pragma unroll
+                    for (int i = 0; i < 4; ++i) tail_load(i, tail_soff(0, 0));
+                }
+#pragma unroll
+                for (int q = 0; q < 4; ++q) {
+                    f32x4 y;
+#pragma unroll
+                    for (int e = 0; e < 4; ++e) y[e] = acc[j][4 * q + e];
+                    *(f32x4 *)&tp[r * 36 + 8 * q + 4 * h] = y;
+                }
+#pragma unroll
+                for (int pq = 0; pq < 4; ++pq) {
+                    const f32x4 v = *(const f32x4 *)&tp[(trow + 8 * pq) * 36 + tc4];
+                    __builtin_amdgcn_raw_buffer_store_b128(__builtin_bit_cast(u32x4, v), hrs, hoff[pq], 32 * j * 4, 0);
+                }
+            }
+        } else {
+            float sum = 0.f;
+#pragma unroll
+            for (int j = 0; j < NT; ++j) {
+                float pj = 0.f;
+#pragma unroll
+                for (int q = 0; q < 4; ++q) {
+                    const f32x4 bv = *(const f32x4 *)&pbias_s[32 * j + 8 * q + 4 * h];
+#pragma unroll
+                    for (int e = 0; e < 4; ++e) { acc[j][4 * q + e] += bv[e]; pj += acc[j][4 * q + e]; }
+                }
+                sum += pj;
+            }
+            sum = pair_sum(sum);
+            const float mean = sum * (1.0f / N);
+            float sq = 0.f;
+#pragma unroll
+            for (int j = 0; j < NT; ++j) {
+                float pj = 0.f;
+#pragma unroll
+                for (int t = 0; t < 16; ++t) { const float c = acc[j][t] - mean; acc[j][t] = c; pj += c * c; }
+                sq += pj;
+            }
+            sq = pair_sum(sq);
+            const float rstd = 1.0f / sqrtf(sq * (1.0f / N) + 1e-5f * (SC * SC));
+            tp = smem + wave * (32 * 36);
+            trow = lane >> 3; tc4 = (lane & 7) * 4;
+#pragma unroll
+            for (int j = 0; j < NT; ++j) {
+#pragma unroll
+                for (int q = 0; q < 4; ++q) {
+                    const f32x4 gv = *(const f32x4 *)&pgam_s[32 * j + 8 * q + 4 * h];
+                    const f32x4 bv = *(const f32x4 *)&pbet_s[32 * j + 8 * q + 4 * h];
+                    f32x4 y;
+#pragma unroll
+                    for (int e = 0; e < 4; ++e) { y[e] = acc[j][4 * q + e] * rstd * gv[e] + bv[e]; acc[j][4 * q + e] = y[e]; }
+                    if constexpr (!TWO || P1) *(f32x4 *)&tp[r * 36 + 8 * q + 4 * h] = y;
+                }
+                if constexpr (TWO && !P1) __builtin_amdgcn_sched_barrier(0);
+                if constexpr (!TWO || P1) {
+#pragma unroll
+                    for (int pq = 0; pq < 4; ++pq) {
+                        const f32x4 v = *(const f32x4 *)&tp[(trow + 8 * pq) * 36 + tc4];
+                        const int orow = m0 + 32 * wave + trow + 8 * pq;
+                        if (orow < M) *(f32x4 *)(pout + (size_t)orow * N + 32 * j + tc4) = v;
+                    }
+                }
+            }
+        }
+        if constexpr ((!TWO && !EMB) || (P1 && TAIL == 4))
+        if (score_w != nullptr) {
+            for (int c = 0; c < num_classes; ++c) {
+                __syncthreads();
+                for (int i = tid; i < N; i += 256) sw_s[i] = score_w[(size_t)c * N + i];
+                __syncthreads();
+                float dot = 0.f;
+#pragma unroll
+                for (int j = 0; j < NT; ++j) {
+                    float pj = 0.f;
+#pragma unroll
+                    for (int q = 0; q < 4; ++q) {
+                        const f32x4 wv = *(const f32x4 *)&sw_s[32 * j + 8 * q + 4 * h];
+#pragma unroll
+                        for (int e = 0; e < 4; ++e) pj += acc[j][4 * q + e] * wv[e];
+                    }
+                    dot += pj;
+                }
+                dot = pair_sum(dot);
+                if (h == 0 && row_ok) {
+                    float sc = dot + score_b[c];
+                    if (sigmoid) sc = 1.0f / (1.0f + expf(-sc));
+                    scores[(size_t)row * num_classes + c] = sc;
+                }
+            }
+        }
+        if constexpr (DIAG != 0) dsum[1] += stamp() - tq;
+        if constexpr (PT != 0) {
+            tail_stage(0);
+            int rowoff[4];
+            __amdgpu_buffer_rsrc_t crs;
+            if constexpr (PT == 1) {
+                crs = __builtin_amdgcn_make_buffer_rsrc(ptl.C2 + (size_t)m0 * PTN2, 0, (M - m0 < BM ? M - m0 : BM) * PTN2 * 4, 0x00020000);
+#pragma unroll
+                for (int p = 0; p < 4; ++p) rowoff[p] = ((32 * wave + trow + 8 * p) * PTN2 + tc4) * 4;
+            } else {
+                crs = __builtin_amdgcn_make_buffer_rsrc(ptl.C2, 0, 0, 0x00020000);
+#pragma unroll
+                for (int p = 0; p < 4; ++p) {
+                    const int orow = m0 + 32 * wave + trow + 8 * p;
+                    const int bb = orow / ptl.T, tt = orow - bb * ptl.T;
+                    rowoff[p] = orow < M ? (((bb * ptl.H * ptl.T + tt) << ptl.dhs) + tc4) * 4 : (int)0x80000000;
+                }
+            }
+            bias_mfma(0);
+            __syncthreads();
+            for (int c = 0; c < TNC; ++c) {
+                const int cn = c + 1 < TNC ? c + 1 : c;
+                static_for<8>([&](auto ktc) __attribute__((always_inline)) {
+                    constexpr int kt = decltype(ktc)::value;
+                    tail_step(ktc, kt < 7 ? tail_soff(c, kt + 1) : tail_soff(cn, 0));
+                });
+                if constexpr (PT == 2) {
+                    const int which = c >> 1;
+                    crs = __builtin_amdgcn_make_buffer_rsrc(ptl.C2 + (size_t)which * M * N, 0, M * N * 4, 0x00020000);
+                }
+#pragma unroll
+                for (int jj = 0; jj < 4; ++jj) {
+                    __builtin_amdgcn_sched_barrier(0);
+#pragma unroll
+                    for (int q = 0; q < 4; ++q) {
+                        f32x4 v;
+#pragma unroll
+                        for (int e = 0; e < 4; ++e) v[e] = PT == 1 ? relu1(U[jj][4 * q + e]) : U[jj][4 * q + e];
+                        *(f32x4 *)&tp[r * 36 + 8 * q + 4 * h] = v;
+                    }
+                    int soff;
+                    if constexpr (PT == 1) soff = (TCH * c + 32 * jj) * 4;
+                    else {
+                        const int cc = (TCH * c + 32 * jj) & (N - 1), head = cc >> ptl.dhs, e0 = cc - (head << ptl.dhs);
+                        soff = (((head * ptl.T) << ptl.dhs) + e0) * 4;
+                    }
+#pragma unroll
+                    for (int p = 0; p < 4; ++p) {
+                        const f32x4 v = *(const f32x4 *)&tp[(trow + 8 * p) * 36 + tc4];
+                        __builtin_amdgcn_raw_buffer_store_b128(__builtin_bit_cast(u32x4, v), crs, rowoff[p], soff, 0);
+                    }
+                }
+                __builtin_amdgcn_sched_barrier(0);
+                bias_mfma(cn);
+            }
+        }
+      });
+    }
+    if constexpr (DIAG != 0) {
+        if (diag != nullptr && lane == 0) {
+            unsigned long long *o = diag + ((size_t)blockIdx.x * 4 + wave) * 8;
+            o[0] = dsum[0]; o[1] = dsum[1]; o[2] = dsum[2]; o[3] = 0; o[4] = 0;
+            o[5] = stamp() - tbegin; o[6] = ktiles; o[7] = tbegin;
+        }
+    }
+}
diff --git a/video-summarization_amd/csrc/vs_scorer.cpp b/video-summarization_amd/csrc/vs_scorer.cpp
--- a/video-summarization_amd/csrc/vs_scorer.cpp
+++ b/video-summarization_amd/csrc/vs_scorer.cpp
@@ -67,6 +67,7 @@
     {"VS_ATTN_W64_CHECKED", &VskOptions::attn_w64_checked, 0}, {"VS_TRAIN_LP_MIN_ROWS", &VskOptions::train_lp_min_rows, 1024},
     {"VS_ATTN_W64", &VskOptions::attn_w64, 1},           {"VS_ATTN_W64_ABL", &VskOptions::attn_w64_abl, 0},
     {"VS_LAYER_TAIL_MIN_ROWS", &VskOptions::layer_tail_min_rows, 1024},
+    {"VS_EMBED_QKV_MIN_ROWS", &VskOptions::embed_qkv_min_rows, 65536},
 };
 int option_from_env(const OptionName &o) {
     const char *e = getenv(o.name);
@@ -161,6 +162,7 @@
     const bool f16x3 = plan.linear == VS_ARITH_F16X3;
     auto frag = [&](size_t f, size_t h) { return w->p(f16x3 ? h : f); };
     const float *pe_rows = pk ? pk->pe_rows : (w->has_pe ? w->p(w->pe) : nullptr);
+    const bool embed_qkv = vsk_embed_qkv_applies(in, plan, vsk_options());
     {
         StageScope ps(VS_STAGE_EMBED, st);
         switch (plan.embed) {
@@ -181,6 +183,12 @@
             VS_LAUNCH(vsk_sum_parts_pe(qkv, 8, w->p(w->embed_b), pe_rows, T, h0, M, d, st));
             break;
         case VS_EMBED_GEMM:
+            if (embed_qkv) {
+                const LayerOff &N = w->layers[0];
+                VS_LAUNCH(vsk_embed_qkv(x, w->p(w->embed_w), w->p(w->embed_b), pe_rows, h0, w->p(N.wqkv), w->p(N.bqkv), qkv, B, T, d, H,
+                                        D.in_features, st));
+                break;
+            }
             VS_LAUNCH(vsk_linear(x, w->p(w->embed_w), frag(w->f_embed_w, w->h_embed_w), w->p(w->embed_b), h0, M, d, D.in_features, 0,
                                  pe_rows, T, plan.mode_linear, st));
             break;
@@ -202,7 +210,7 @@
         if (plan.layer == VS_LAYER_RING) {
             StageScope ps(VS_STAGE_QKV, st);
             VS_LAUNCH(vsk_gemm16(h16, w->p(P.r_wqkv), w->p(P.bqkv), qkv, M, 3 * d, d, 3, 1, T, H, d / H, qs, st));
-        } else if (l == 0 ? plan.embed != VS_EMBED_BF16_QKV : !plan.tail_writes_qkv()) {
+        } else if (l == 0 ? plan.embed != VS_EMBED_BF16_QKV && !embed_qkv : !plan.tail_writes_qkv()) {
             StageScope ps(VS_STAGE_QKV, st);
             VS_LAUNCH(vsk_qkv(h0, w->p(P.wqkv), frag(P.f_wqkv, P.h_wqkv), w->p(P.bqkv), qkv, B, T, d, H, plan.mode_qkv, st,
                               plan.qkv16 ? qs : 1.0f));
```
